# mattiaskvist/yolo-v1

Hardware: AMD Instinct MI355X
Metric: images/sec at 448x448, forward (YOLOv1Backbone + FC head) (higher is better)
Workload: dtype bf16; 1 GPU; BASELINE.json configs[1]: batch=64/GPU 448x448 forward-only, YOLOv1Backbone + FC head, 1xMI355X per rank; global_batch=64, per_gpu_batch=64, weights=random init (torch default, seed 0), parallelism=single

## Files before the change

### include/yolo_hip.h

```cpp
#ifndef YOLO_HIP_H
#define YOLO_HIP_H

#include <stddef.h>
#include <stdint.h>

#ifdef __cplusplus
extern "C" {
#endif

#define YOLO_HIP_ABI_VERSION 2

#define YOLO_E_ARG (-1)
#define YOLO_E_UNSUPPORTED (-2)

typedef void *yolo_stream_t;

int yolo_hip_abi_version(void);
const char *yolo_hip_last_error(void);
int yolo_debug_stamps(void *buf, int k_iter);
int yolo_stream_create(int low, yolo_stream_t *out);


int yolo_decode(const float *pred, int N, int S, int B, int C, double conf_thr,
                double *rec, int32_t *counts, yolo_stream_t stream);

int yolo_decode_gt(const float *tgt, int N, int S, int B, int C,
                   double *rec, int32_t *counts, yolo_stream_t stream);

#define YOLO_NMS_INFERENCE 0
#define YOLO_NMS_METRICS 1

int yolo_nms(const double *rec, const int32_t *counts, int N, int max_per_img, double thr, int variant,
             int32_t *keep, int32_t *keep_counts, yolo_stream_t stream);

int yolo_pairwise_iou(const double *a, int na, const double *b, int nb, int variant,
                      double *out, yolo_stream_t stream);

int yolo_loss_fwd_bwd(const float *pred, const float *tgt, int N, int S, int B, int C,
                      float lambda_coord, float lambda_noobj,
                      float *out, float *dpred, double *work, yolo_stream_t stream);

int yolo_loss_iou(const float *boxes1, const float *boxes2, long n, float *out, yolo_stream_t stream);


typedef struct yolo_igemm_desc {
    int32_t N, Ho, Wo;
    int64_t in_img_stride;
    int32_t in_row_stride;
    int32_t in_px_stride;
    int32_t in_off;
    int32_t stride;
    int32_t KH, KW;
    int32_t tap_len;
    int32_t Cout;
    int64_t out_img_stride;
    int32_t out_row_stride, out_px_stride, out_off;
    int32_t epilogue;
    float slope;
    int32_t out_fp32;
    int32_t split_k;
    int64_t aux_img_stride;
    int32_t aux_row_stride, aux_px_stride, aux_off;
    int32_t pool2;
    int32_t w_blocked;
    int32_t tile_order;
    int32_t tile_hint;
    int64_t px_begin, px_end;
    int32_t skew_phases;
    int32_t skew_step;
    void *bn_stats;
    int32_t tile_px;
    int32_t split_slabs;
} yolo_igemm_desc;

#define YOLO_EPI_NONE 0
#define YOLO_EPI_BIAS 1
#define YOLO_EPI_BIAS_LRELU 2
#define YOLO_EPI_MUL_DLRELU 3

#define YOLO_EPI_BIAS_ADD_LRELU 4

int yolo_igemm(const yolo_igemm_desc *d, const void *in_bf16, const void *w_bf16 ,
               const float *bias, const void *aux_bf16, void *out, yolo_stream_t stream);
int yolo_igemm_finish(const yolo_igemm_desc *d, const float *acc, const float *bias, const void *aux_bf16,
                      void *out_bf16, yolo_stream_t stream);

typedef struct yolo_wgrad_desc {
    int64_t P;
    int32_t dy_px_stride, x_px_stride;
    int32_t Cout, Cin;
    int32_t KH, KW, pad;
    int64_t x_row_stride;
    int32_t split;
    int32_t accumulate;
    int32_t variant;
    int32_t geo_W, geo_H, geo_img_slots, geo_row_slots, geo_px_slots, geo_slot0;
    double *dw_sumsq;
    float *slabs;
    int64_t slab_floats;
} yolo_wgrad_desc;

int yolo_wgrad_slab_floats(const yolo_wgrad_desc *d, long *floats);
int yolo_wgrad(const yolo_wgrad_desc *d, const void *x_bf16, const void *dy_bf16,
               float *dw_packed, float *db, yolo_stream_t stream);

typedef struct yolo_pool_desc {
    int32_t N, H, W, C;
    int32_t in_halo, out_halo;
} yolo_pool_desc;
int yolo_maxpool3s2_fwd(const yolo_pool_desc *d, const void *x_bf16, void *y_bf16, yolo_stream_t stream);
int yolo_maxpool3s2_bwd(const yolo_pool_desc *d, const void *x_bf16, const void *dy_bf16, void *dx_bf16, int dx_halo,
                        yolo_stream_t stream);
int yolo_maxpool2_fwd(const yolo_pool_desc *d, const void *x_bf16, void *y_bf16, yolo_stream_t stream);
int yolo_maxpool2_bwd_lrelu(const yolo_pool_desc *d, const void *yfull_bf16, const void *dpool_bf16,
                            float slope, void *dz_bf16, yolo_stream_t stream);
int yolo_maxpool2_bwd_codes(const yolo_pool_desc *d, const void *ypool_bf16, const void *codes_u16, const void *dpool_bf16,
                            float slope, void *dz_bf16, yolo_stream_t stream);


int yolo_nchw_f32_to_nhwc_bf16(const float *x, int N, int C, int H, int W, void *y, int Cpad,
                               int halo_lo, int halo_hi, yolo_stream_t stream);
int yolo_nhwc_bf16_to_nchw_f32(const void *x, int N, int C, int H, int W, int halo, float *y, yolo_stream_t stream);
int yolo_nhwc_bf16_to_nchw_bf16(const void *x, int N, int C, int H, int W, int halo, void *y, yolo_stream_t stream);

int yolo_pack_conv_weight(const float *w_oihw, int Cout, int Cin, int KH, int KW, int Cinp, int KWp,
                          void *w_fwd_bf16, void *w_dgrad_bf16, yolo_stream_t stream);
int yolo_pack_fc_weight(const float *w, int O, int C, int HW, void *w_fwd_bf16, void *w_t_bf16, yolo_stream_t stream);
int yolo_pack_fc_weight_blocked(const float *w, int O, long K, void *w_panels_bf16, yolo_stream_t stream);
int yolo_pack_fc_weight_blocked_hwc(const float *w, int O, int C, int HW, void *w_panels_bf16, yolo_stream_t stream);
int yolo_unpack_conv_wgrad(const float *dw_packed, int Cout, int Cin, int KH, int KW, int Cinp, int KWp,
                           float *dw_oihw, int accumulate, yolo_stream_t stream);
int yolo_conv_stem7_fwd(const void *x_nhwc4_bf16, const void *w_packed_bf16, const float *bias, int N, int Ho, int Wo,
                        long x_img_stride, int x_row_stride, float slope, int pool2, void *out_bf16,
                        long out_img_stride, int out_row_stride, int out_off, void *out_full_bf16,
                        long full_img_stride, int full_row_stride, int full_off, yolo_stream_t stream);
int yolo_conv_stem7_fwd_f32(const float *x_nchw_f32, const void *w_packed_bf16, const float *bias, int N, int H, int W, float slope,
                            int pool2, void *out_bf16, long out_img_stride, int out_row_stride, int out_off, void *out_full_bf16,
                            long full_img_stride, int full_row_stride, int full_off, yolo_stream_t stream);
int yolo_wgrad_stem7(const void *x_nhwc4_bf16, const void *dy_bf16, int N, int Ho, int Wo, long x_img_stride,
                     int x_row_stride, long dy_img_stride, int dy_row_stride, int dy_off, float *dw_oihw,
                     float *db, float *scratch, long scratch_elems, yolo_stream_t stream);
int yolo_wgrad_stem7_pooled(const void *x_nhwc4_bf16, const void *y_full_bf16, int N, int Ho, int Wo, long x_img_stride,
                            int x_row_stride, long y_img_stride, int y_row_stride, int y_off, const void *dpool_bf16,
                            long dp_img_stride, int dp_row_stride, int dp_off, float slope, float *dw_oihw, float *db,
                            float *scratch, long scratch_elems, yolo_stream_t stream);
int yolo_wgrad_stem7_codes(const void *x_nhwc4_bf16, const void *y_pooled_bf16, const void *codes_u16, int N, int Ho, int Wo,
                           long x_img_stride, int x_row_stride, const void *dpool_bf16, long dp_img_stride, int dp_row_stride,
                           int dp_off, float slope, float *dw_oihw, float *db, float *scratch, long scratch_elems,
                           yolo_stream_t stream);
#define YOLO_PACK_MAX 32
typedef struct yolo_conv_pack_item {
    const float *w;
    void *w_fwd_bf16;
    void *w_dgrad_bf16;
    int Cout, Cin, KH, KW;
} yolo_conv_pack_item;
typedef struct yolo_conv_unpack_item {
    const float *dw_packed;
    float *dw_oihw;
    int Cout, Cin, KH, KW;
} yolo_conv_unpack_item;
int yolo_pack_conv_weights_multi(const yolo_conv_pack_item *items, int count, yolo_stream_t stream);
int yolo_unpack_conv_wgrads_multi(const yolo_conv_unpack_item *items, int count, yolo_stream_t stream);
int yolo_im2col_rows(const void *x_bf16, long x_img_stride, int x_row_stride, int x_px_stride, int stride,
                     int KH, int seg, int N, int Ho, int Wo, int out_halo, void *xcol_bf16, yolo_stream_t stream);
int yolo_transpose_f32_to_bf16(const float *x, int R, int Ccols, void *y_bf16, int ld, yolo_stream_t stream);
int yolo_transpose_bf16(const void *x_bf16, int R, int Ccols, int ldx, void *y_bf16, int ldy, yolo_stream_t stream);
int yolo_fc_dgrad_to_nhwc(const float *dxT, int N, int C, int H, int W, int halo, const void *y_act_bf16,
                          float slope, void *g_bf16, yolo_stream_t stream);
int yolo_cast_f32_to_bf16(const float *x, long n, void *y_bf16, yolo_stream_t stream);
int yolo_cast_bf16_to_f32(const void *x_bf16, long n, float *y, yolo_stream_t stream);
int yolo_bias_lrelu_rows(const float *x, const float *bias, int R, int Ccols, float slope,
                         void *y_bf16, float *y_f32, yolo_stream_t stream);
int yolo_bias_lrelu_rows_slabs(const float *x, int slabs, const float *bias, int R, int Ccols, float slope,
                               void *y_bf16, float *y_f32, yolo_stream_t stream);

int yolo_scale_rows_to_bf16(const float *x, const unsigned char *mask, float scale, const void *act_bf16, float slope,
                            int R, int Cc, int ld, void *y_bf16, yolo_stream_t stream);
int yolo_dropout_bf16(const void *x_bf16, const unsigned char *mask, float scale, long n, void *y_bf16, yolo_stream_t stream);

int yolo_sumsq_f32(const float *g, long n, double *acc, yolo_stream_t stream);
int yolo_adam_step(float *p, const float *g, float *exp_avg, float *exp_avg_sq, long n, float lr, float beta1,
                   float beta2, float eps, float weight_decay, long step, const double *norm_sq,
                   float max_norm, void *p_bf16, yolo_stream_t stream);
#define YOLO_MT_MAX 48
typedef struct yolo_adam_tensor {
    float *p;
    const float *g;
    float *m, *v;
    void *p_bf16;
    long n;
} yolo_adam_tensor;
int yolo_sumsq_f32_multi(const float *const *g, const long *n, int count, double *acc, yolo_stream_t stream);
int yolo_sumsq_fixed_slots(const long *n, int count, long *slots);
int yolo_sumsq_f32_fixed(const float *g, long n, double *scratch, long scratch_slots, double *acc, yolo_stream_t stream);
int yolo_sumsq_f32_multi_fixed(const float *const *g, const long *n, int count, double *scratch, long scratch_slots, double *acc,
                               yolo_stream_t stream);
int yolo_adam_step_multi(const yolo_adam_tensor *t, int count, float lr, float beta1, float beta2, float eps,
                         float weight_decay, long step, const double *norm_sq, float max_norm, const float *skip_flag,
                         yolo_stream_t stream);
int yolo_adam_step_multi_bg(const yolo_adam_tensor *t, int count, float lr, float beta1, float beta2, float eps,
                            float weight_decay, long step, const double *norm_sq, float max_norm, const float *skip_flag,
                            int workgroups, yolo_stream_t stream);

typedef struct yolo_sgd_tensor {
    float *p;
    const float *g;
    float *buf;
    void *p_bf16;
    long n;
} yolo_sgd_tensor;
int yolo_sgd_step(float *p, const float *g, float *buf, long n, float lr, float momentum, float dampening, float weight_decay,
                  int nesterov, int first_step, const double *norm_sq, float max_norm, void *p_bf16, const float *skip_flag,
                  yolo_stream_t stream);
int yolo_sgd_step_multi(const yolo_sgd_tensor *t, int count, float lr, float momentum, float dampening, float weight_decay,
                        int nesterov, int first_step, const double *norm_sq, float max_norm, const float *skip_flag,
                        yolo_stream_t stream);
int yolo_sgd_step_multi_bg(const yolo_sgd_tensor *t, int count, float lr, float momentum, float dampening, float weight_decay,
                           int nesterov, int first_step, const double *norm_sq, float max_norm, const float *skip_flag,
                           int workgroups, yolo_stream_t stream);

int yolo_clip_scale_f32(float *g, long n, const double *norm_sq, float max_norm, yolo_stream_t stream);

#define YOLO_BN_ACC_REPLICAS 16
int yolo_batchnorm_train_fwd(void *z_bf16, int N, int H, int W, int C, int halo, const float *gamma, const float *beta,
                             double eps, double momentum, float *running_mean, float *running_var,
                             const void *residual_bf16, int residual_halo, int relu, double *acc2c,
                             float *scale_shift, void *out_bf16, int out_halo, float *save_mean_invstd,
                             int stats_ready, yolo_stream_t stream);
int yolo_batchnorm_bwd(void *dy_bf16, int dy_halo, const void *y_bf16, int y_halo, const void *z_bf16, int z_halo,
                       int N, int H, int W, int C, const float *gamma, const float *mean_invstd, void *dz_bf16,
                       long dz_img_stride, long dz_row_stride, long dz_px_stride, long dz_off, int store_masked_dy,
                       int relu_from_z, float *dgamma, float *dbeta, double *acc2c, float *coef3c, yolo_stream_t stream);

int yolo_map_match(const double *rec, const int32_t *keep, const int32_t *keep_counts, int N, int max_per_img,
                   const double *gt_rec, const int32_t *gt_counts, int max_gt, const double *thresholds, int T,
                   double extra_threshold, double small_area, double medium_area, unsigned long long *tp_bits,
                   int32_t *gt_bucket, yolo_stream_t stream);

int yolo_preprocess_u8(const unsigned char *src_u8, int N, int Hs, int Ws, int Ho, int Wo, const int32_t *hbounds,
                       const int32_t *hcoef, int hk, const int32_t *vbounds, const int32_t *vcoef, int vk,
                       unsigned char *tmp_u8, const float *mean3, const float *std3, void *out_nhwc4_bf16, int halo,
                       float *out_nchw, yolo_stream_t stream);

typedef struct yolo_augment_desc {
    int64_t src_off;
    int64_t tmp_off;
    int32_t Hs, Ws;
    int32_t top, left, ch, cw;
    const int32_t *htab;
    const int32_t *vtab;
    int32_t hk, vk;
    int32_t n_ops;
    int32_t ops[3];
    float brightness;
    float saturation;
    int32_t hue_shift;
    int32_t reserved;
} yolo_augment_desc;
#define YOLO_AUG_BRIGHTNESS 0
#define YOLO_AUG_SATURATION 1
#define YOLO_AUG_HUE 2

int yolo_augment_u8(const unsigned char *src_u8, int64_t src_bytes, const yolo_augment_desc *descs_host,
                    const yolo_augment_desc *descs_dev, int N, int Ho, int Wo, unsigned char *tmp_u8, int64_t tmp_bytes,
                    const float *mean3, const float *std3, void *out_nhwc4_bf16, int halo, float *out_nchw,
                    unsigned char *out_u8, yolo_stream_t stream);

#ifdef __cplusplus
}
#endif
#endif
```

### yolo-v1_amd/csrc/igemm.hip

```cpp
#include "igemm_common.h"

namespace yolo {

template <int TCO, int TPX, int BK, int WCO, int WPX, int NST, int MF = MFMA_32x32x16>
struct IgemmCfg {
    static constexpr int NW = WCO * WPX;
    static constexpr int NTHR = NW * 64;
    static constexpr bool UNEVEN = MF == MFMA_16x16x32_STAGGER_U;
    static constexpr int A_BYTES = TCO * BK * 2;
    static constexpr int B_BYTES = (TPX * BK * 2 + 1024 * NW - 1) / (1024 * NW) * (1024 * NW);
    static constexpr int STAGE_BYTES = A_BYTES + B_BYTES;
    static constexpr int EP = TCO + 4;
    static constexpr int NTILES = TPX / 16;
    static constexpr int NT0 = (NTILES + 1) / 2, NT1 = NTILES / 2;
    static constexpr int PPX = UNEVEN ? NT0 * 16 : TPX / WPX;
    static constexpr int EPI_BYTES = PPX * EP * 4;
    static constexpr int TABLE_BYTES = TPX * 32;
    static constexpr int RED_BYTES = WCO * WPX * 64 * 16 * 4;
    static constexpr int MAIN_BYTES = (NST * STAGE_BYTES > EPI_BYTES + RED_BYTES) ? NST * STAGE_BYTES : EPI_BYTES + RED_BYTES;
    static constexpr int LDS_BYTES = TABLE_BYTES + MAIN_BYTES;
    static constexpr int A_INSTR = A_BYTES / 1024 / NW;
    static constexpr int B_INSTR = B_BYTES / 1024 / NW;
    static constexpr int LOADS = A_INSTR + B_INSTR;
    static constexpr int FR = MF != MFMA_32x32x16 ? 16 : 32;
    static constexpr int KS = MF != MFMA_32x32x16 ? 32 : 16;
    static constexpr int MT = TCO / WCO / FR, NT = UNEVEN ? NT0 : TPX / WPX / FR;
    static_assert(A_BYTES % (1024 * NW) == 0 && B_BYTES % (1024 * NW) == 0, "stage must split evenly over the waves");
    static_assert(!UNEVEN || (WPX == 2 && TPX % 16 == 0), "uneven split: two pixel groups of 16-pixel columns");
    static_assert(UNEVEN || TPX * BK * 2 == B_BYTES, "only the uneven configuration pads its B stage");
    static_assert(TPX <= NTHR, "one table entry per thread");
};

template <int TCO, int TPX, int BK, int WCO, int WPX, int NST, int MF, int VAR>
__global__ void __launch_bounds__(WCO * WPX * 64, (TCO == 64 && TPX == 128 && BK == 32 && VAR == 0 ? 5 : 2)) igemm_kernel(const IgemmParams p)
{
    using Cfg = IgemmCfg<TCO, TPX, BK, WCO, WPX, NST, MF>;
    constexpr bool STATS = VAR == 1, CODES = VAR == 2;
    constexpr bool M16 = MF != MFMA_32x32x16;
    constexpr bool UNEVEN = Cfg::UNEVEN;
    constexpr bool STG = MF == MFMA_16x16x32_STAGGER || UNEVEN;
    constexpr int FR = Cfg::FR;
    constexpr int MT = Cfg::MT, NT = Cfg::NT, NW = Cfg::NW, NTHR = Cfg::NTHR;
    extern __shared__ __attribute__((aligned(16))) char smem[];
    long *tab = reinterpret_cast<long *>(smem);
    char *stage_base = smem + Cfg::TABLE_BYTES;

    const int tid = threadIdx.x;
    const int lane = tid & 63;
    const int wave = __builtin_amdgcn_readfirstlane(tid >> 6);
    const int wco = UNEVEN ? wave % WCO : wave / WPX, wpx = UNEVEN ? wave / WCO : wave % WPX;
    const int px_lo = UNEVEN ? wpx * Cfg::NT0 * 16 : wpx * (TPX / WPX);

    if (NW == 8 && p.skew_phases > 1 && gridDim.x * gridDim.y > 256 && blockIdx.y == 0 && blockIdx.x < 256) {
        const int ph = (blockIdx.x >> 3) % p.skew_phases;
        if (ph) {
            const long t0 = __builtin_amdgcn_s_memtime(), wait = ph * p.skew_cycles;
            while ((long)__builtin_amdgcn_s_memtime() - t0 < wait) __builtin_amdgcn_s_sleep(16);
        }
    }

    const int nwg = p.n_co_tiles * p.n_px_tiles;
    int bid = blockIdx.x;
    {
        const int q = nwg >> 3, r = nwg & 7, xcd = bid & 7, k = bid >> 3;
        bid = (xcd < r ? xcd * (q + 1) : r * (q + 1) + (xcd - r) * q) + k;
    }
    const int co_tile = p.px_fastest ? bid / p.n_px_tiles : bid % p.n_co_tiles;
    const int px_tile = p.px_fastest ? bid % p.n_px_tiles : bid / p.n_co_tiles;
    const int co0 = co_tile * TCO;
    const int tpv = p.tpx_valid;
    const long px0 = p.px_begin + (long)px_tile * tpv;

    if (tid < TPX) {
        int n, oy, ox;
        bool valid;
        if (p.pool) {
            const int per_img = p.pool_tiles_x * p.pool_tiles_y;
            n = px_tile / per_img;
            const int t = px_tile - n * per_img;
            const int ty = t / p.pool_tiles_x, tx = t - ty * p.pool_tiles_x;
            oy = ty * (TPX / p.pool_tw) + tid / p.pool_tw;
            ox = tx * p.pool_tw + tid % p.pool_tw;
            valid = oy < p.HoWo / p.Wo && ox < p.Wo;
            if (!valid) { oy = 0; ox = 0; }
        } else {
            long m = px0 + tid;
            valid = m < p.M && tid < tpv;
            if (!valid) m = p.M - 1;
            n = (int)(m / p.HoWo);
            const int rem = (int)(m - (long)n * p.HoWo);
            oy = rem / p.Wo;
            ox = rem - oy * p.Wo;
        }
        tab[4 * tid] = (long)n * p.in_img_stride + (long)(oy * p.stride) * p.in_row_stride + (long)(ox * p.stride) * p.in_px_stride + p.in_off;
        const int qy = p.pool ? oy >> 1 : oy, qx = p.pool ? ox >> 1 : ox;
        tab[4 * tid + 1] = valid ? ((long)n * p.out_img_stride + (long)qy * p.out_row_stride + (long)qx * p.out_px_stride + p.out_off) : -1;
        tab[4 * tid + 2] = (long)n * p.aux_img_stride + (long)oy * p.aux_row_stride + (long)ox * p.aux_px_stride + p.aux_off;
    }
    __syncthreads();

    const bf16_t *a_src[Cfg::A_INSTR];
    const bf16_t *b_src[Cfg::B_INSTR];
    int a_dst[Cfg::A_INSTR], b_dst[Cfg::B_INSTR];
    {
        constexpr int CPR = BK / 8, RPB = 16 / CPR;
#pragma unroll
        for (int i = 0; i < Cfg::A_INSTR; ++i) {
            const int q = i * NW + wave;
            const int pos = q * 64 + lane;
            const int R = pos >> 4, s = (pos & 15) ^ swz_key<BK, M16>(R);
            const int r = R * RPB + s / CPR, chunk = s % CPR;
            int co = co0 + r;
            if (co >= p.Cout) co = p.Cout - 1;
            a_src[i] = p.w_blocked ? p.w + ((long)co_tile * p.nk * TCO + r) * BK + chunk * 8 : p.w + (long)co * p.Ktot + chunk * 8;
            a_dst[i] = q * 1024;
        }
#pragma unroll
        for (int i = 0; i < Cfg::B_INSTR; ++i) {
            const int q = i * NW + wave;
            const int pos = q * 64 + lane;
            const int R = pos >> 4, s = (pos & 15) ^ swz_key<BK, M16>(R);
            const int r = R * RPB + s / CPR, chunk = s % CPR;
            b_src[i] = r < TPX ? p.in + tab[4 * r] + chunk * 8 : p.in + tab[0];
            b_dst[i] = Cfg::A_BYTES + q * 1024;
        }
    }

    const bool interleave = gridDim.y > 1 && p.KH * p.KW == 1;
    const int kstep = interleave ? (int)gridDim.y : 1;
    int kbeg, kend;
    if (interleave) {
        const int mine = (p.nk - (int)blockIdx.y + kstep - 1) / kstep;
        kbeg = 0;
        kend = mine > 0 ? mine : 0;
    } else {
        kbeg = blockIdx.y * p.nk_per_split;
        kend = min(p.nk, kbeg + p.nk_per_split);
    }
    const int cpt = p.tap_len / BK;
    int tap = interleave ? 0 : kbeg / cpt;
    int c0 = interleave ? (int)blockIdx.y * BK : (kbeg - tap * cpt) * BK;
    int ky = tap / p.KW, kx = tap - ky * p.KW;

    auto stage = [&](int buf, int kiter_local) {
        char *sb = stage_base + buf * Cfg::STAGE_BYTES;
        const int kiter = interleave ? (int)blockIdx.y + kiter_local * kstep : kiter_local;
        const long a_off = (long)kiter * (p.w_blocked ? TCO * BK : BK);
        const long b_off = interleave ? (long)kiter * BK : (long)ky * p.in_row_stride + (long)kx * p.in_px_stride + c0;
        if (p.w_blocked) {
#pragma unroll
            for (int i = 0; i < Cfg::A_INSTR; ++i) GLDS16_NT(a_src[i] + a_off, sb + a_dst[i]);
        } else {
#pragma unroll
            for (int i = 0; i < Cfg::A_INSTR; ++i) GLDS16(a_src[i] + a_off, sb + a_dst[i]);
        }
#pragma unroll
        for (int i = 0; i < Cfg::B_INSTR; ++i) GLDS16(b_src[i] + b_off, sb + b_dst[i]);
        c0 += BK;
        if (c0 == p.tap_len) {
            c0 = 0;
            if (++kx == p.KW) { kx = 0; ++ky; }
        }
    };

    int a_rd[MT], b_rd[NT];
#pragma unroll
    for (int i = 0; i < MT; ++i) a_rd[i] = lds_off<BK, M16>(wco * (TCO / WCO) + i * FR + (lane & (FR - 1)), M16 ? (lane >> 4) : (lane >> 5));
#pragma unroll
    for (int i = 0; i < NT; ++i) {
        int row = px_lo + i * FR + (lane & (FR - 1));
        if (UNEVEN && row >= TPX) row = TPX - 1;
        b_rd[i] = Cfg::A_BYTES + lds_off<BK, M16>(row, M16 ? (lane >> 4) : (lane >> 5));
    }

    typedef typename std::conditional<M16, f32x4, f32x16>::type acc_t;
    acc_t acc[MT][NT];
#pragma unroll
    for (int i = 0; i < MT; ++i)
#pragma unroll
        for (int j = 0; j < NT; ++j)
#pragma unroll
            for (int r = 0; r < (M16 ? 4 : 16); ++r) acc[i][j][r] = 0.0f;

    constexpr int KSTEPS = BK / Cfg::KS;
    constexpr int KSH = M16 ? 6 : 5;
    auto read_frags = [&](int buf, bf16x8(&af)[KSTEPS][MT], bf16x8(&bfr)[KSTEPS][NT], auto ntc) {
        constexpr int NTG = decltype(ntc)::value;
        const char *sb = stage_base + buf * Cfg::STAGE_BYTES;
#pragma unroll
        for (int ks = 0; ks < KSTEPS; ++ks) {
#pragma unroll
            for (int i = 0; i < MT; ++i) af[ks][i] = *reinterpret_cast<const bf16x8 *>(sb + (a_rd[i] ^ (ks << KSH)));
#pragma unroll
            for (int j = 0; j < NTG; ++j) bfr[ks][j] = *reinterpret_cast<const bf16x8 *>(sb + (b_rd[j] ^ (ks << KSH)));
        }
    };
    auto mfmas = [&](bf16x8(&af)[KSTEPS][MT], bf16x8(&bfr)[KSTEPS][NT], auto ntc) {
        constexpr int NTG = decltype(ntc)::value;
#pragma unroll
        for (int ks = 0; ks < KSTEPS; ++ks)
#pragma unroll
            for (int i = 0; i < MT; ++i)
#pragma unroll
                for (int j = 0; j < NTG; ++j) {
                    if constexpr (M16) acc[i][j] = __builtin_amdgcn_mfma_f32_16x16x32_bf16(af[ks][i], bfr[ks][j], acc[i][j], 0, 0, 0);
                    else acc[i][j] = __builtin_amdgcn_mfma_f32_32x32x16_bf16(af[ks][i], bfr[ks][j], acc[i][j], 0, 0, 0);
                }
    };

    if constexpr (STG) {
        static_assert(!STG || (NST >= 3 && NW == 8), "stagger needs 8 waves and a ring of >= 3 stages");
        constexpr std::integral_constant<int, NT> ntA{};
        constexpr std::integral_constant<int, UNEVEN ? Cfg::NT1 : NT> ntB{};
        constexpr int D = NST - 1;
        const bool grpB = wave >= NW / 2;
        const int nkk = kend - kbeg;
#pragma unroll
        for (int s0 = 0; s0 < D; ++s0)
            if (s0 < nkk) stage(s0, kbeg + s0);
        auto wait_stage = [&](int newer) {
            if (newer >= D - 1) wait_vmcnt<(D - 1) * Cfg::LOADS>();
            else if (newer == 1 && D - 1 > 1) wait_vmcnt<Cfg::LOADS>();
            else wait_vmcnt<0>();
        };
        wait_stage(nkk - 1 < D - 1 ? nkk - 1 : D - 1);
        __builtin_amdgcn_s_barrier();
        __builtin_amdgcn_sched_barrier(0);
        bf16x8 af[KSTEPS][MT], bfr[KSTEPS][NT];
        int rd_buf = 0;
#ifdef IGEMM_STAMPS
        long stamp[8] = {0, 0, 0, 0, 0, 0, 0, 0};
#define STAMP(i) do { if (p.dbg && it == p.dbg_it) { __builtin_amdgcn_sched_barrier(0); stamp[i] = __builtin_amdgcn_s_memtime(); __builtin_amdgcn_sched_barrier(0); } } while (0)
#else
#define STAMP(i) do { } while (0)
#endif
        if (!grpB) {
            int ld_buf = D % NST;
            for (int it = 0; it < nkk; ++it) {
                STAMP(0);
                read_frags(rd_buf, af, bfr, ntA);
                STAMP(1);
                if (it + D < nkk) stage(ld_buf, kbeg + it + D);
                STAMP(2);
                asm volatile("s_waitcnt lgkmcnt(0)" ::: "memory");
                STAMP(3);
                __builtin_amdgcn_sched_barrier(0);
                __builtin_amdgcn_s_barrier();
                __builtin_amdgcn_sched_barrier(0);
                STAMP(4);
                __builtin_amdgcn_s_setprio(1);
                mfmas(af, bfr, ntA);
                __builtin_amdgcn_s_setprio(0);
                STAMP(5);
                { const int left = nkk - 2 - it; wait_stage(left < 0 ? 0 : left); }
                STAMP(6);
                __builtin_amdgcn_sched_barrier(0);
                __builtin_amdgcn_s_barrier();
                __builtin_amdgcn_sched_barrier(0);
                STAMP(7);
                rd_buf = rd_buf + 1 == NST ? 0 : rd_buf + 1;
                ld_buf = ld_buf + 1 == NST ? 0 : ld_buf + 1;
            }
            __builtin_amdgcn_s_barrier();
        } else {
            __builtin_amdgcn_s_barrier();
            __builtin_amdgcn_sched_barrier(0);
            int ld_buf = D % NST;
            for (int it = 0; it < nkk; ++it) {
                STAMP(0);
                read_frags(rd_buf, af, bfr, ntB);
                STAMP(1);
                if (it + D < nkk) stage(ld_buf, kbeg + it + D);
                STAMP(2);
                asm volatile("s_waitcnt lgkmcnt(0)" ::: "memory");
                { const int left = nkk - 2 - it; wait_stage(left < 0 ? 0 : left); }
                STAMP(3);
                __builtin_amdgcn_sched_barrier(0);
                __builtin_amdgcn_s_barrier();
                __builtin_amdgcn_sched_barrier(0);
                STAMP(4);
                STAMP(5);
                __builtin_amdgcn_s_setprio(1);
                mfmas(af, bfr, ntB);
                __builtin_amdgcn_s_setprio(0);
                STAMP(6);
                __builtin_amdgcn_sched_barrier(0);
                __builtin_amdgcn_s_barrier();
                __builtin_amdgcn_sched_barrier(0);
                STAMP(7);
                rd_buf = rd_buf + 1 == NST ? 0 : rd_buf + 1;
                ld_buf = ld_buf + 1 == NST ? 0 : ld_buf + 1;
            }
        }
#ifdef IGEMM_STAMPS
        if (p.dbg && lane == 0 && blockIdx.x < 512) {
#pragma unroll
            for (int i = 0; i < 8; ++i) p.dbg[((long)blockIdx.x * 8 + wave) * 8 + i] = stamp[i];
        }
#endif
#undef STAMP
    } else {
    constexpr int D = NST - 1;
#pragma unroll
    for (int s0 = 0; s0 < D; ++s0)
        if (kbeg + s0 < kend) stage(s0, kbeg + s0);
    int cur = 0, nxt = D % NST;
    for (int it = kbeg; it < kend; ++it) {
        if (D >= 2 && it + 1 < kend) wait_vmcnt<(D >= 2 ? (D - 1) * Cfg::LOADS : 0)>();
        else wait_vmcnt<0>();
        asm volatile("s_waitcnt lgkmcnt(0)" ::: "memory");
        __builtin_amdgcn_s_barrier();
        if (it + D < kend) stage(nxt, it + D);
        bf16x8 af[KSTEPS][MT], bfr[KSTEPS][NT];
        const char *sb = stage_base + cur * Cfg::STAGE_BYTES;
#pragma unroll
        for (int ks = 0; ks < KSTEPS; ++ks) {
#pragma unroll
            for (int i = 0; i < MT; ++i) af[0][i] = *reinterpret_cast<const bf16x8 *>(sb + (a_rd[i] ^ (ks << KSH)));
#pragma unroll
            for (int j = 0; j < NT; ++j) bfr[0][j] = *reinterpret_cast<const bf16x8 *>(sb + (b_rd[j] ^ (ks << KSH)));
#pragma unroll
            for (int i = 0; i < MT; ++i)
#pragma unroll
                for (int j = 0; j < NT; ++j) {
                    if constexpr (M16) acc[i][j] = __builtin_amdgcn_mfma_f32_16x16x32_bf16(af[0][i], bfr[0][j], acc[i][j], 0, 0, 0);
                    else acc[i][j] = __builtin_amdgcn_mfma_f32_32x32x16_bf16(af[0][i], bfr[0][j], acc[i][j], 0, 0, 0);
                }
        }
        cur = (cur + 1 == NST) ? 0 : cur + 1;
        nxt = (nxt + 1 == NST) ? 0 : nxt + 1;
    }
    }
    __syncthreads();

    float *ep = reinterpret_cast<float *>(stage_base);
    constexpr int PPX = Cfg::PPX;
    constexpr int CCH = TCO / 8;
    constexpr int PX_PER_STEP = NTHR / CCH;
    const int cc = tid % CCH;
    const int co = co0 + cc * 8;
    const bool has_bias = p.epilogue == YOLO_EPI_BIAS || p.epilogue == YOLO_EPI_BIAS_LRELU || p.epilogue == YOLO_EPI_BIAS_ADD_LRELU;
    float bias8[8];
#pragma unroll
    for (int k = 0; k < 8; ++k) bias8[k] = has_bias && (co + k < p.Cout) ? p.bias[co + k] : 0.0f;
    const bool split = gridDim.y > 1 && p.slab_stride == 0;
    void *const outp = p.slab_stride ? (void *)(reinterpret_cast<float *>(p.out) + (long)blockIdx.y * p.slab_stride) : p.out;
    float *red = reinterpret_cast<float *>(stage_base + Cfg::EPI_BYTES) + tid * 16;
    if constexpr (STATS) {
#pragma unroll
        for (int k = 0; k < 16; ++k) red[k] = 0.0f;
    }

    constexpr int E_CCH = TCO / 8, E_PXS = NTHR / E_CCH, E_PPX = Cfg::PPX;
    constexpr int NIT = (E_PPX + E_PXS - 1) / E_PXS;
    constexpr bool CAN_PREFETCH = NIT <= 4 && !UNEVEN && !STATS && TCO * TPX <= 128 * 128;
    const bool aux_fast = CAN_PREFETCH && (p.epilogue == YOLO_EPI_BIAS_ADD_LRELU || p.epilogue == YOLO_EPI_MUL_DLRELU) && gridDim.y == 1 && !p.pool &&
                          !p.out_fp32 && co0 + (tid % E_CCH) * 8 + 8 <= p.Cout;
    uint4 axv[CAN_PREFETCH ? NIT : 1];
    long axo[CAN_PREFETCH ? NIT : 1];
    auto aux_fetch = [&](int q) {
#pragma unroll
        for (int it = 0; it < NIT; ++it) {
            const int lp = tid / E_CCH + it * E_PXS;
            const int px = q * E_PPX + (lp < E_PPX ? lp : 0);
            axo[it] = lp < E_PPX ? tab[4 * px + 1] : -1;
            axv[it] = axo[it] >= 0 ? *reinterpret_cast<const uint4 *>(p.aux + tab[4 * px + 2] + co0 + (tid % E_CCH) * 8) : uint4{0u, 0u, 0u, 0u};
        }
    };

    for (int q = 0; q < WPX; ++q) {
        if (q > 0) __syncthreads();
        if constexpr (CAN_PREFETCH) {
            if (aux_fast) aux_fetch(q);
        }
        if (wpx == q) {
#pragma unroll
            for (int i = 0; i < MT; ++i)
#pragma unroll
                for (int j = 0; j < NT; ++j) {
                    if constexpr (M16) {
                        const int lp = j * 16 + (lane & 15);
                        const int cob = wco * (TCO / WCO) + i * 16 + 4 * (lane >> 4);
                        f32x4 v = {acc[i][j][0], acc[i][j][1], acc[i][j][2], acc[i][j][3]};
                        *reinterpret_cast<f32x4 *>(ep + lp * Cfg::EP + cob) = v;
                    } else {
                        const int lp = j * 32 + (lane & 31);
                        const int cob = wco * (TCO / WCO) + i * 32 + 4 * (lane >> 5);
#pragma unroll
                        for (int g = 0; g < 4; ++g) {
                            f32x4 v = {acc[i][j][4 * g], acc[i][j][4 * g + 1], acc[i][j][4 * g + 2], acc[i][j][4 * g + 3]};
                            *reinterpret_cast<f32x4 *>(ep + lp * Cfg::EP + cob + 8 * g) = v;
                        }
                    }
                }
        }
        __syncthreads();
        const int pbase = q * PPX;
        const int ppx_q = UNEVEN && q == 1 ? Cfg::NT1 * 16 : PPX;

        if (split) {
            float *o = reinterpret_cast<float *>(p.out);
            for (int e = tid; e < ppx_q * TCO; e += NTHR) {
                const int lp = e / TCO, c = e - lp * TCO;
                const long ob = tab[4 * (pbase + lp) + 1];
                if (ob >= 0 && co0 + c < p.Cout) atomicAdd(o + ob + co0 + c, ep[lp * Cfg::EP + c]);
            }
            continue;
        }
        if (p.pool) {
            const int tw = p.pool_tw, hw = tw >> 1;
            for (int w = tid / CCH; w < PPX / 4; w += PX_PER_STEP) {
                const int l00 = (w / hw) * 2 * tw + (w % hw) * 2;
                const long ob = tab[4 * (pbase + l00) + 1];
                if (ob < 0 || co >= p.Cout) continue;
                float v[8];
                if (CODES && p.pool == 3) {
                    unsigned code = 0;
#pragma unroll
                    for (int k = 0; k < 8; ++k) {
                        const float *zp = ep + l00 * Cfg::EP + cc * 8 + k;
                        float m = 0.0f;
                        unsigned am = 0;
#pragma unroll
                        for (int w4 = 0; w4 < 4; ++w4) {
                            float t = zp[((w4 >> 1) * tw + (w4 & 1)) * Cfg::EP] + bias8[k];
                            t = (p.epilogue == YOLO_EPI_BIAS_LRELU && t < 0.0f) ? t * p.slope : t;
                            t = __uint_as_float((unsigned)f32_to_bf16(t) << 16);
                            if (w4 == 0 || t > m) { m = t; am = w4; }
                        }
                        v[k] = m;
                        code |= am << (2 * k);
                        __builtin_amdgcn_sched_barrier(0);
                    }
                    reinterpret_cast<unsigned short *>(const_cast<bf16_t *>(p.aux))[(ob + co) >> 3] = (unsigned short)code;
                } else {
#pragma unroll
                    for (int k = 0; k < 8; ++k) {
                        const float a = ep[l00 * Cfg::EP + cc * 8 + k], b = ep[(l00 + 1) * Cfg::EP + cc * 8 + k];
                        const float c = ep[(l00 + tw) * Cfg::EP + cc * 8 + k], d = ep[(l00 + tw + 1) * Cfg::EP + cc * 8 + k];
                        float m = fmaxf(fmaxf(a, b), fmaxf(c, d)) + bias8[k];
                        v[k] = (p.epilogue == YOLO_EPI_BIAS_LRELU && m < 0.0f) ? m * p.slope : m;
                    }
                }
                uint4 pk;
                pk.x = (unsigned)f32_to_bf16(v[0]) | ((unsigned)f32_to_bf16(v[1]) << 16);
                pk.y = (unsigned)f32_to_bf16(v[2]) | ((unsigned)f32_to_bf16(v[3]) << 16);
                pk.z = (unsigned)f32_to_bf16(v[4]) | ((unsigned)f32_to_bf16(v[5]) << 16);
                pk.w = (unsigned)f32_to_bf16(v[6]) | ((unsigned)f32_to_bf16(v[7]) << 16);
                *reinterpret_cast<uint4 *>(reinterpret_cast<bf16_t *>(p.out) + ob + co) = pk;
            }
            if (p.pool == 2) {
                bf16_t *full = const_cast<bf16_t *>(p.aux);
                for (int lp = tid / CCH; lp < PPX; lp += PX_PER_STEP) {
                    const int px = pbase + lp;
                    if (tab[4 * px + 1] < 0) continue;
                    if (co >= p.Cout) continue;
                    float v[8];
#pragma unroll
                    for (int k = 0; k < 8; ++k) {
                        const float m = ep[lp * Cfg::EP + cc * 8 + k] + bias8[k];
                        v[k] = (p.epilogue == YOLO_EPI_BIAS_LRELU && m < 0.0f) ? m * p.slope : m;
                    }
                    uint4 pk;
                    pk.x = (unsigned)f32_to_bf16(v[0]) | ((unsigned)f32_to_bf16(v[1]) << 16);
                    pk.y = (unsigned)f32_to_bf16(v[2]) | ((unsigned)f32_to_bf16(v[3]) << 16);
                    pk.z = (unsigned)f32_to_bf16(v[4]) | ((unsigned)f32_to_bf16(v[5]) << 16);
                    pk.w = (unsigned)f32_to_bf16(v[6]) | ((unsigned)f32_to_bf16(v[7]) << 16);
                    *reinterpret_cast<uint4 *>(full + tab[4 * px + 2] + co) = pk;
                }
            }
            continue;
        }
        if constexpr (CAN_PREFETCH) {
            if (aux_fast) {
#pragma unroll
                for (int it0 = 0; it0 < NIT; ++it0) {
                    const uint4 av = axv[it0];
                    const long ao = axo[it0];
                    if (ao < 0) continue;
                    const int lp = tid / CCH + it0 * PX_PER_STEP;
                    const f32x4 lo = *reinterpret_cast<const f32x4 *>(ep + lp * Cfg::EP + cc * 8);
                    const f32x4 hi = *reinterpret_cast<const f32x4 *>(ep + lp * Cfg::EP + cc * 8 + 4);
                    float v[8] = {lo[0], lo[1], lo[2], lo[3], hi[0], hi[1], hi[2], hi[3]};
                    const unsigned yy[4] = {av.x, av.y, av.z, av.w};
#pragma unroll
                    for (int k = 0; k < 8; ++k) {
                        const float a = __uint_as_float((k & 1) ? (yy[k >> 1] & 0xffff0000u) : (yy[k >> 1] << 16));
                        if (p.epilogue == YOLO_EPI_BIAS_ADD_LRELU) {
                            v[k] += bias8[k] + a;
                            v[k] = v[k] > 0.0f ? v[k] : v[k] * p.slope;
                        } else {
                            v[k] = a > 0.0f ? v[k] : v[k] * p.slope;
                        }
                    }
                    uint4 pk;
                    pk.x = (unsigned)f32_to_bf16(v[0]) | ((unsigned)f32_to_bf16(v[1]) << 16);
                    pk.y = (unsigned)f32_to_bf16(v[2]) | ((unsigned)f32_to_bf16(v[3]) << 16);
                    pk.z = (unsigned)f32_to_bf16(v[4]) | ((unsigned)f32_to_bf16(v[5]) << 16);
                    pk.w = (unsigned)f32_to_bf16(v[6]) | ((unsigned)f32_to_bf16(v[7]) << 16);
                    *reinterpret_cast<uint4 *>(reinterpret_cast<bf16_t *>(p.out) + ao + co) = pk;
                }
                continue;
            }
        }
#pragma unroll 2
        for (int lp = tid / CCH; lp < ppx_q; lp += PX_PER_STEP) {
            const int px = pbase + lp;
            const long ob = tab[4 * px + 1];
            if (ob < 0 || co >= p.Cout) continue;
            float v[8];
            const f32x4 lo = *reinterpret_cast<const f32x4 *>(ep + lp * Cfg::EP + cc * 8);
            const f32x4 hi = *reinterpret_cast<const f32x4 *>(ep + lp * Cfg::EP + cc * 8 + 4);
            v[0] = lo[0]; v[1] = lo[1]; v[2] = lo[2]; v[3] = lo[3];
            v[4] = hi[0]; v[5] = hi[1]; v[6] = hi[2]; v[7] = hi[3];
            if (has_bias) {
#pragma unroll
                for (int k = 0; k < 8; ++k) v[k] += bias8[k];
            }
            if (p.epilogue == YOLO_EPI_BIAS_ADD_LRELU) {
                const uint4 y = *reinterpret_cast<const uint4 *>(p.aux + tab[4 * px + 2] + co);
                const unsigned yy[4] = {y.x, y.y, y.z, y.w};
#pragma unroll
                for (int k = 0; k < 8; ++k) {
                    v[k] += __uint_as_float((k & 1) ? (yy[k >> 1] & 0xffff0000u) : (yy[k >> 1] << 16));
                    v[k] = v[k] > 0.0f ? v[k] : v[k] * p.slope;
                }
            } else if (p.epilogue == YOLO_EPI_BIAS_LRELU) {
#pragma unroll
                for (int k = 0; k < 8; ++k) v[k] = v[k] > 0.0f ? v[k] : v[k] * p.slope;
            } else if (p.epilogue == YOLO_EPI_MUL_DLRELU) {
                const uint4 y = *reinterpret_cast<const uint4 *>(p.aux + tab[4 * px + 2] + co);
                const unsigned yy[4] = {y.x, y.y, y.z, y.w};
#pragma unroll
                for (int k = 0; k < 8; ++k) {
                    const float a = __uint_as_float((k & 1) ? (yy[k >> 1] & 0xffff0000u) : (yy[k >> 1] << 16));
                    v[k] = a > 0.0f ? v[k] : v[k] * p.slope;
                }
            }
            if (p.out_fp32) {
                float *o = reinterpret_cast<float *>(outp) + ob + co;
                if (co + 8 <= p.Cout && ((ob + co) & 3) == 0) {
                    *reinterpret_cast<f32x4 *>(o) = f32x4{v[0], v[1], v[2], v[3]};
                    *reinterpret_cast<f32x4 *>(o + 4) = f32x4{v[4], v[5], v[6], v[7]};
                } else {
#pragma unroll
                    for (int k = 0; k < 8; ++k)
                        if (co + k < p.Cout) o[k] = v[k];
                }
            } else {
                bf16_t *o = reinterpret_cast<bf16_t *>(p.out) + ob + co;
                uint4 pk;
                pk.x = (unsigned)f32_to_bf16(v[0]) | ((unsigned)f32_to_bf16(v[1]) << 16);
                pk.y = (unsigned)f32_to_bf16(v[2]) | ((unsigned)f32_to_bf16(v[3]) << 16);
                pk.z = (unsigned)f32_to_bf16(v[4]) | ((unsigned)f32_to_bf16(v[5]) << 16);
                pk.w = (unsigned)f32_to_bf16(v[6]) | ((unsigned)f32_to_bf16(v[7]) << 16);
                *reinterpret_cast<uint4 *>(o) = pk;
                if constexpr (STATS) {
                    const unsigned w4[4] = {pk.x, pk.y, pk.z, pk.w};
#pragma unroll
                    for (int k = 0; k < 8; ++k) {
                        const float r = __uint_as_float((k & 1) ? (w4[k >> 1] & 0xffff0000u) : (w4[k >> 1] << 16));
                        red[k] += r;
                        red[8 + k] += r * r;
                    }
                }
            }
        }
    }
    if constexpr (STATS) {
        __syncthreads();
        const float *all = reinterpret_cast<const float *>(stage_base + Cfg::EPI_BYTES);
        for (int c = tid; c < TCO; c += NTHR) {
            const int c8 = c >> 3, k = c & 7;
            float a = 0.0f, b = 0.0f;
            for (int j = 0; j < NTHR / CCH; ++j) { a += all[(j * CCH + c8) * 16 + k]; b += all[(j * CCH + c8) * 16 + 8 + k]; }
            if (co0 + c < p.Cout) {
                double *rep = p.stats + (size_t)(blockIdx.x % YOLO_BN_ACC_REPLICAS) * 2 * p.Cout;
                atomicAdd(rep + co0 + c, (double)a);
                atomicAdd(rep + p.Cout + co0 + c, (double)b);
            }
        }
    }
}

template <int TCO, int TPX, int BK, int WCO, int WPX, int NST, int MF, int VAR>
static int launch_impl(const IgemmParams &p, int splits, hipStream_t s)
{
    using Cfg = IgemmCfg<TCO, TPX, BK, WCO, WPX, NST, MF>;
    static bool attr_done[64] = {};
    int dev = 0;
    if (hipGetDevice(&dev) != hipSuccess || dev < 0 || dev >= 64) dev = 0;
    if (!attr_done[dev]) {
        hipError_t e = hipFuncSetAttribute(reinterpret_cast<const void *>(&igemm_kernel<TCO, TPX, BK, WCO, WPX, NST, MF, VAR>), hipFuncAttributeMaxDynamicSharedMemorySize, Cfg::LDS_BYTES);
        if (e != hipSuccess) return fail((int)e, "yolo_igemm: hipFuncSetAttribute(%d B LDS): %s", Cfg::LDS_BYTES, hipGetErrorString(e));
        attr_done[dev] = true;
    }
    IgemmParams q = p;
    q.n_co_tiles = (p.Cout + TCO - 1) / TCO;
    if (p.pool) {
        q.tpx_valid = TPX;
        q.pool_tiles_x = (p.Wo + p.pool_tw - 1) / p.pool_tw;
        q.pool_tiles_y = (p.HoWo / p.Wo + TPX / p.pool_tw - 1) / (TPX / p.pool_tw);
        q.n_px_tiles = (int)(p.M / p.HoWo) * q.pool_tiles_x * q.pool_tiles_y;
    } else {
        if (q.tpx_valid <= 0 || q.tpx_valid > TPX) q.tpx_valid = TPX;
        q.n_px_tiles = (int)((p.M - p.px_begin + q.tpx_valid - 1) / q.tpx_valid);
    }
    q.nk = (int)(p.Ktot / BK);
    if (p.px_fastest < 0) q.px_fastest = 0;
    q.nk_per_split = (q.nk + splits - 1) / splits;
    const int real_splits = p.slab_stride ? splits : (q.nk + q.nk_per_split - 1) / q.nk_per_split;
    hipLaunchKernelGGL((igemm_kernel<TCO, TPX, BK, WCO, WPX, NST, MF, VAR>), dim3(q.n_co_tiles * q.n_px_tiles, real_splits), dim3(Cfg::NTHR), Cfg::LDS_BYTES, s, q);
    return check_launch("yolo_igemm");
}

template <int TCO, int TPX, int BK, int WCO, int WPX, int NST, int MF = MFMA_32x32x16>
static int launch(const IgemmParams &p, int splits, hipStream_t s)
{
    return p.stats ? launch_impl<TCO, TPX, BK, WCO, WPX, NST, MF, 1>(p, splits, s) : launch_impl<TCO, TPX, BK, WCO, WPX, NST, MF, 0>(p, splits, s);
}

__global__ void __launch_bounds__(256) igemm_finish_kernel(const float *__restrict__ acc, const float *__restrict__ bias, const bf16_t *__restrict__ aux,
                                                           bf16_t *__restrict__ out, long M, int slabs, int HoWo, int Wo, int Cout, int epilogue, float slope,
                                                           long out_img, int out_row, int out_px, int out_off, long aux_img, int aux_row, int aux_px, int aux_off)
{
    const int C8 = Cout >> 3;
    const long idx = (long)blockIdx.x * blockDim.x + threadIdx.x;
    if (idx >= M * C8) return;
    const int c = (int)(idx % C8) * 8;
    const long m = idx / C8;
    const int n = (int)(m / HoWo);
    const int rem = (int)(m - (long)n * HoWo);
    const int oy = rem / Wo, ox = rem - oy * Wo;
    const float4 a = *reinterpret_cast<const float4 *>(acc + m * Cout + c), b = *reinterpret_cast<const float4 *>(acc + m * Cout + c + 4);
    float v[8] = {a.x, a.y, a.z, a.w, b.x, b.y, b.z, b.w};
    for (int sl = 1; sl < slabs; ++sl) {
        const float *as = acc + (long)sl * M * Cout + m * Cout + c;
        const float4 a2 = *reinterpret_cast<const float4 *>(as), b2 = *reinterpret_cast<const float4 *>(as + 4);
        v[0] += a2.x; v[1] += a2.y; v[2] += a2.z; v[3] += a2.w;
        v[4] += b2.x; v[5] += b2.y; v[6] += b2.z; v[7] += b2.w;
    }
    if (epilogue == YOLO_EPI_BIAS || epilogue == YOLO_EPI_BIAS_LRELU) {
#pragma unroll
        for (int k = 0; k < 8; ++k) v[k] += bias[c + k];
    }
    if (epilogue == YOLO_EPI_BIAS_LRELU) {
#pragma unroll
        for (int k = 0; k < 8; ++k) v[k] = v[k] > 0.0f ? v[k] : v[k] * slope;
    } else if (epilogue == YOLO_EPI_MUL_DLRELU) {
        const uint4 y = *reinterpret_cast<const uint4 *>(aux + (long)n * aux_img + (long)oy * aux_row + (long)ox * aux_px + aux_off + c);
        const unsigned yy[4] = {y.x, y.y, y.z, y.w};
#pragma unroll
        for (int k = 0; k < 8; ++k) {
            const float t = __uint_as_float((k & 1) ? (yy[k >> 1] & 0xffff0000u) : (yy[k >> 1] << 16));
            v[k] = t > 0.0f ? v[k] : v[k] * slope;
        }
    }
    uint4 o;
    o.x = (unsigned)f32_to_bf16(v[0]) | ((unsigned)f32_to_bf16(v[1]) << 16);
    o.y = (unsigned)f32_to_bf16(v[2]) | ((unsigned)f32_to_bf16(v[3]) << 16);
    o.z = (unsigned)f32_to_bf16(v[4]) | ((unsigned)f32_to_bf16(v[5]) << 16);
    o.w = (unsigned)f32_to_bf16(v[6]) | ((unsigned)f32_to_bf16(v[7]) << 16);
    *reinterpret_cast<uint4 *>(out + (long)n * out_img + (long)oy * out_row + (long)ox * out_px + out_off + c) = o;
}

}

using namespace yolo;

static long *g_dbg = nullptr;
static int g_dbg_it = 0;

namespace yolo {
void debug_stamp_target(long **buf, int *it)
{
    *buf = g_dbg;
    *it = g_dbg_it;
}
}

YOLO_API int yolo_debug_stamps(void *buf, int k_iter)
{
    g_dbg = (long *)buf;
    g_dbg_it = k_iter;
#ifdef IGEMM_STAMPS
    return 0;
#else
    return buf ? fail(YOLO_E_UNSUPPORTED, "yolo_debug_stamps: this library was built without -DIGEMM_STAMPS (make diag)") : 0;
#endif
}

YOLO_API int yolo_igemm(const yolo_igemm_desc *d, const void *in, const void *w, const float *bias, const void *aux, void *out, yolo_stream_t stream)
{
    if (!d || !in || !w || !out) return fail(YOLO_E_ARG, "yolo_igemm: null pointer");
    if (d->N <= 0 || d->Ho <= 0 || d->Wo <= 0 || d->KH <= 0 || d->KW <= 0 || d->tap_len <= 0 || d->Cout <= 0 || d->stride <= 0)
        return fail(YOLO_E_ARG, "yolo_igemm: bad descriptor");
    if ((d->epilogue == YOLO_EPI_BIAS || d->epilogue == YOLO_EPI_BIAS_LRELU || d->epilogue == YOLO_EPI_BIAS_ADD_LRELU) && !bias) return fail(YOLO_E_ARG, "yolo_igemm: epilogue needs bias");
    if ((d->epilogue == YOLO_EPI_MUL_DLRELU || d->epilogue == YOLO_EPI_BIAS_ADD_LRELU) && !aux) return fail(YOLO_E_ARG, "yolo_igemm: epilogue needs aux");
    if (d->epilogue < 0 || d->epilogue > YOLO_EPI_BIAS_ADD_LRELU) return fail(YOLO_E_ARG, "yolo_igemm: epilogue %d", d->epilogue);
    const int splits = d->split_k > 1 ? d->split_k : 1;
    if (splits > 1 && (!d->out_fp32 || d->epilogue != YOLO_EPI_NONE)) return fail(YOLO_E_ARG, "yolo_igemm: split_k needs fp32 output and EPI_NONE");
    if (d->split_slabs && splits > 1 && (d->out_off != 0 || (d->Wo > 1 && d->out_px_stride != d->Cout) || (d->Ho > 1 && d->out_row_stride != d->Wo * d->Cout)
                                         || (d->N > 1 && d->out_img_stride != (int64_t)d->Ho * d->Wo * d->Cout)))
        return fail(YOLO_E_ARG, "yolo_igemm: split_slabs needs the dense [N*Ho*Wo][Cout] output addressing");
    if (d->tile_px < 0) return fail(YOLO_E_ARG, "yolo_igemm: tile_px %d", d->tile_px);
    if (!d->out_fp32 && ((d->Cout & 7) || (d->out_off & 7) || (d->out_px_stride & 7) || (d->out_row_stride & 7) || (d->out_img_stride & 7)))
        return fail(YOLO_E_UNSUPPORTED, "yolo_igemm: bf16 output needs Cout and output strides in multiples of 8");
    if ((d->tap_len & 31) || (d->in_off & 7) || (d->in_px_stride & 3) || (d->in_row_stride & 7) || (d->in_img_stride & 7))
        return fail(YOLO_E_UNSUPPORTED, "yolo_igemm: tap_len=%d must be a multiple of 32 and input strides 16-B aligned", d->tap_len);

    IgemmParams p{};
    p.in = (const bf16_t *)in; p.w = (const bf16_t *)w; p.bias = bias; p.aux = (const bf16_t *)aux; p.out = out;
    p.M = (long)d->N * d->Ho * d->Wo; p.HoWo = d->Ho * d->Wo; p.Wo = d->Wo;
    if (d->px_begin < 0 || d->px_end < 0 || d->px_begin > p.M || d->px_end > p.M || (d->px_end && d->px_end <= d->px_begin))
        return fail(YOLO_E_ARG, "yolo_igemm: bad pixel range [%ld, %ld) of %ld", (long)d->px_begin, (long)d->px_end, (long)p.M);
    if ((d->px_begin || d->px_end) && d->pool2) return fail(YOLO_E_UNSUPPORTED, "yolo_igemm: pixel ranges are not available with pool2");
    p.px_begin = d->px_begin;
    p.tpx_valid = d->tile_px;
    p.slab_stride = (d->split_slabs && splits > 1) ? (long)d->N * d->Ho * d->Wo * d->Cout : 0;
    if (d->px_end) p.M = d->px_end;
    p.in_img_stride = d->in_img_stride; p.in_row_stride = d->in_row_stride; p.in_px_stride = d->in_px_stride; p.in_off = d->in_off; p.stride = d->stride;
    p.KH = d->KH; p.KW = d->KW; p.tap_len = d->tap_len; p.Cout = d->Cout;
    p.Ktot = (long)d->KH * d->KW * d->tap_len;
    p.out_img_stride = d->out_img_stride; p.out_row_stride = d->out_row_stride; p.out_px_stride = d->out_px_stride; p.out_off = d->out_off;
    p.aux_img_stride = d->aux_img_stride; p.aux_row_stride = d->aux_row_stride; p.aux_px_stride = d->aux_px_stride; p.aux_off = d->aux_off;
    p.epilogue = d->epilogue; p.slope = d->slope; p.out_fp32 = d->out_fp32;
    hipStream_t s = STRM(stream);

    const bool bk64 = (d->tap_len % 64) == 0;
    const bool small_co = d->Cout <= 64 || (d->Cout % 128 != 0 && d->Cout % 64 == 0 && d->Cout < 512);
    const long npx = p.M - p.px_begin;
    const long tiles128 = ((npx + 127) / 128) * ((d->Cout + 127) / 128);
    const int force = d->tile_hint;
    p.w_blocked = d->w_blocked;
    p.px_fastest = d->tile_order == 1 ? 0 : (d->tile_order == 2 ? 1 : -1);
    if (d->skew_phases < 0 || d->skew_phases > 64 || d->skew_step < 0 || d->skew_step > (1 << 22)) return fail(YOLO_E_ARG, "yolo_igemm: skew_phases %d / skew_step %d", d->skew_phases, d->skew_step);
    p.skew_phases = d->skew_phases;
    p.skew_cycles = d->skew_step;
    p.stats = (double *)d->bn_stats;
    p.dbg = g_dbg;
    p.dbg_it = g_dbg_it;
    if (p.stats && (d->out_fp32 || splits > 1 || d->pool2 || d->px_begin || d->px_end))
        return fail(YOLO_E_UNSUPPORTED, "yolo_igemm: bn_stats needs a plain bf16 launch (no split_k, pool2, pixel range)");
    p.pool = (d->pool2 == 2 || d->pool2 == 3) ? d->pool2 : (d->pool2 ? 1 : 0);
    if (p.pool == 2 && !aux) return fail(YOLO_E_ARG, "yolo_igemm: pool2 = 2 writes the un-pooled activation through aux (pointer + aux_* strides)");
    if (p.pool == 3 && (!aux || (d->Cout & 7) || (d->out_img_stride & 7) || (d->out_row_stride & 7) || (d->out_px_stride & 7) || (d->out_off & 7)))
        return fail(YOLO_E_ARG, "yolo_igemm: pool2 = 3 writes the arg-max codes through aux (one uint16 per 8 channels at (pooled element address) / 8): "
                                "Cout and the out_* strides must be multiples of 8");
    p.pool_tw = 16;
    if (p.pool && d->tile_px) return fail(YOLO_E_UNSUPPORTED, "yolo_igemm: tile_px is not available with pool2");
    if (p.pool && (splits > 1 || d->out_fp32 || (d->Ho & 1) || (d->Wo & 1) || (d->epilogue != YOLO_EPI_BIAS && d->epilogue != YOLO_EPI_BIAS_LRELU)))
        return fail(YOLO_E_UNSUPPORTED, "yolo_igemm: pool2 needs even Ho/Wo, bf16 output, a bias epilogue and no split-K");
    if (force == 20 || force == 21) return igemm_persist_launch(p, force, splits, s);
    if (p.pool == 3 && !(force >= 15 && force <= 18)) {
        if (!bk64 || d->w_blocked || p.stats) return fail(YOLO_E_UNSUPPORTED, "yolo_igemm: pool2 = 3 needs tap_len %% 64 == 0 (or tile_hint 16 / 18), plain weights, no bn_stats");
        if (small_co) return launch_impl<64, 128, 64, 2, 2, 2, MFMA_16x16x32, 2>(p, splits, s);
        return launch_impl<128, 128, 64, 2, 2, 2, MFMA_16x16x32, 2>(p, splits, s);
    }
    if (d->w_blocked) {
        if (!bk64) return fail(YOLO_E_UNSUPPORTED, "yolo_igemm: blocked weights need tap_len %% 64 == 0");
        return npx <= 64 ? launch<128, 64, 64, 2, 2, 3, MFMA_16x16x32>(p, splits, s) : launch<128, 128, 64, 2, 2, 2, MFMA_16x16x32>(p, splits, s);
    }
    if (force == 12) return launch<256, 256, 32, 2, 4, 4, MFMA_16x16x32_STAGGER>(p, splits, s);
    if (force == 14) {
        if (d->pool2) return fail(YOLO_E_UNSUPPORTED, "yolo_igemm: tile_hint 14 has no pooled epilogue");
        return launch<256, 208, 32, 4, 2, 4, MFMA_16x16x32_STAGGER_U>(p, splits, s);
    }
    if (force >= 15 && force <= 18) return igemm_pipe_launch(p, force, splits, s);
    if (force == 22) return conv_c64_launch(p, s);
    if (force == 19) return igemm_stream_launch(p, splits, s);
    if (force == 13) return launch<256, 128, 32, 4, 2, 4, MFMA_16x16x32_STAGGER>(p, splits, s);
    if (force == 10) return launch<64, 128, 32, 2, 2, 2>(p, splits, s);
    if (!bk64) {
        if (force == 7) return launch<64, 128, 32, 2, 2, 3>(p, splits, s);
        if (force == 9) return launch<64, 128, 32, 2, 2, 4>(p, splits, s);
        if (force == 10) return launch<64, 128, 32, 2, 2, 2>(p, splits, s);
        if (small_co) return launch<64, 128, 32, 2, 2, 3>(p, splits, s);
        return launch<128, 128, 32, 2, 2, 2>(p, splits, s);
    }
    if (force == 8) return launch<64, 128, 64, 2, 2, 3, MFMA_16x16x32>(p, splits, s);
    if (p.pool) {
        if (small_co) return launch<64, 128, 64, 2, 2, 2, MFMA_16x16x32>(p, splits, s);
        return launch<128, 128, 64, 2, 2, 2, MFMA_16x16x32>(p, splits, s);
    }
    if (force == 1) return launch<128, 128, 64, 2, 2, 2>(p, splits, s);
    if (force == 2) return launch<256, 128, 64, 4, 2, 3>(p, splits, s);
    if (force == 3) return launch<128, 64, 64, 2, 2, 2>(p, splits, s);
    if (force == 4) return launch<64, 128, 64, 2, 2, 2>(p, splits, s);
    if (force == 5) return launch<128, 128, 64, 2, 2, 2, MFMA_16x16x32>(p, splits, s);
    if (force == 6) return launch<256, 128, 64, 4, 2, 3, MFMA_16x16x32>(p, splits, s);
    if (force == 11) return launch<256, 128, 64, 4, 2, 3, MFMA_16x16x32_STAGGER>(p, splits, s);
    if (npx <= 64) {
        if (small_co) return launch<64, 64, 64, 2, 2, 2, MFMA_16x16x32>(p, splits, s);
        return splits > 1 ? launch<128, 64, 64, 2, 2, 3, MFMA_16x16x32>(p, splits, s) : launch<128, 64, 64, 2, 2, 2, MFMA_16x16x32>(p, splits, s);
    }
    if (small_co) return launch<64, 128, 64, 2, 2, 2, MFMA_16x16x32>(p, splits, s);
    if (tiles128 * splits < 320 && d->Cout >= 128) return launch<128, 64, 64, 2, 2, 2, MFMA_16x16x32>(p, splits, s);
    return launch<128, 128, 64, 2, 2, 2, MFMA_16x16x32>(p, splits, s);
}

YOLO_API int yolo_igemm_finish(const yolo_igemm_desc *d, const float *acc, const float *bias, const void *aux, void *out, yolo_stream_t stream)
{
    if (!d || !acc || !out) return fail(YOLO_E_ARG, "yolo_igemm_finish: null pointer");
    if (d->epilogue != YOLO_EPI_NONE && d->epilogue != YOLO_EPI_BIAS && d->epilogue != YOLO_EPI_BIAS_LRELU && d->epilogue != YOLO_EPI_MUL_DLRELU)
        return fail(YOLO_E_UNSUPPORTED, "yolo_igemm_finish: epilogue %d", d->epilogue);
    if ((d->epilogue == YOLO_EPI_BIAS || d->epilogue == YOLO_EPI_BIAS_LRELU) && !bias) return fail(YOLO_E_ARG, "yolo_igemm_finish: epilogue needs bias");
    if (d->epilogue == YOLO_EPI_MUL_DLRELU && !aux) return fail(YOLO_E_ARG, "yolo_igemm_finish: epilogue needs aux");
    if (d->out_fp32 || d->pool2 || (d->Cout & 7) || (d->out_off & 7) || (d->out_px_stride & 7) || (d->out_row_stride & 7) || (d->out_img_stride & 7))
        return fail(YOLO_E_UNSUPPORTED, "yolo_igemm_finish: bf16 output with Cout and strides in multiples of 8, no pool2");
    const long M = (long)d->N * d->Ho * d->Wo;
    const long total = M * (d->Cout / 8);
    hipLaunchKernelGGL(igemm_finish_kernel, dim3((unsigned)((total + 255) / 256)), dim3(256), 0, STRM(stream), acc, bias, (const bf16_t *)aux, (bf16_t *)out, M,
                       (d->split_slabs && d->split_k > 1) ? d->split_k : 1, d->Ho * d->Wo, d->Wo, d->Cout, d->epilogue, d->slope, (long)d->out_img_stride, d->out_row_stride, d->out_px_stride, d->out_off,
                       (long)d->aux_img_stride, d->aux_row_stride, d->aux_px_stride, d->aux_off);
    return check_launch("yolo_igemm_finish");
}
```

### yolo-v1_amd/csrc/igemm_common.h

```cpp
#pragma once
#include "common.h"
#include <type_traits>

namespace yolo {

typedef __attribute__((ext_vector_type(8))) __bf16 bf16x8;
typedef __attribute__((ext_vector_type(16))) float f32x16;
typedef __attribute__((ext_vector_type(4))) float f32x4;

enum { MFMA_32x32x16 = 0, MFMA_16x16x32 = 1, MFMA_16x16x32_STAGGER = 2, MFMA_16x16x32_STAGGER_U = 3 };

struct IgemmParams {
    const bf16_t *in;
    const bf16_t *w;
    const float *bias;
    const bf16_t *aux;
    void *out;
    long M;
    int HoWo, Wo;
    long in_img_stride;
    int in_row_stride, in_px_stride, in_off, stride;
    int KH, KW, tap_len, Cout;
    long Ktot;
    long out_img_stride;
    int out_row_stride, out_px_stride, out_off;
    long aux_img_stride;
    int aux_row_stride, aux_px_stride, aux_off;
    int epilogue;
    float slope;
    int out_fp32;
    int pool, pool_tw, pool_tiles_x, pool_tiles_y;
    int w_blocked;
    int nk;
    int nk_per_split;
    int n_co_tiles, n_px_tiles;
    long px_begin;
    int tpx_valid;
    long slab_stride;
    int px_fastest;
    int skew_phases;
    long skew_cycles;
    long *dbg;
    int dbg_it;
    double *stats;
    unsigned div_hw_magic, div_hw_shift, div_w_magic, div_w_shift, div_hw2_magic, div_hw2_shift;
    unsigned *tile_ctr;
};

#define GLDS16(gptr, lptr) \
    __builtin_amdgcn_global_load_lds((const __attribute__((address_space(1))) void *)(gptr), (__attribute__((address_space(3))) void *)(lptr), 16, 0, 0)

#define GLDS16_NT(gptr, lptr) \
    __builtin_amdgcn_global_load_lds((const __attribute__((address_space(1))) void *)(gptr), (__attribute__((address_space(3))) void *)(lptr), 16, 0, 2)

template <int BK, bool M16>
__device__ __forceinline__ int swz_key(int R)
{
    if constexpr (BK == 32 && M16) return (-R) & 3;
    else return R & 15;
}

template <int BK, bool M16>
__device__ __forceinline__ int lds_off(int r, int chunk)
{
    constexpr int CPR = BK / 8;
    constexpr int RPB = 16 / CPR;
    const int R = r / RPB;
    const int s = (r % RPB) * CPR + chunk;
    return R * 256 + ((s ^ swz_key<BK, M16>(R)) << 4);
}

template <int N>
__device__ __forceinline__ void wait_vmcnt()
{
    asm volatile("s_waitcnt vmcnt(%0)" ::"n"(N) : "memory");
}

int igemm_pipe_launch(const IgemmParams &p, int hint, int splits, hipStream_t s);
int igemm_persist_launch(const IgemmParams &p, int hint, int splits, hipStream_t s);
int igemm_stream_launch(const IgemmParams &p, int splits, hipStream_t s);
int conv_c64_launch(const IgemmParams &p, hipStream_t s);

}
```

### yolo-v1_amd/csrc/igemm_persist.hip

```cpp
#include "igemm_common.h"
#include <atomic>
#include <mutex>

namespace yolo {

template <int NTILES_>
struct PersistCfg {
    static constexpr int TCO = 256, NTILES = NTILES_, NST = 4, BK = 32;
    static constexpr int TPX = 16 * NTILES;
    static constexpr int WCO = 4, NW = 8, NTHR = 512;
    static constexpr int NT0 = 7, NT1 = NTILES - 7;
    static constexpr int A_BYTES = TCO * BK * 2;
    static constexpr int B_BYTES = 256 * BK * 2;
    static constexpr int STAGE_BYTES = A_BYTES + B_BYTES;
    static constexpr int A_PIECES = A_BYTES / 1024 / NW, B_PIECES = B_BYTES / 1024 / NW;
    static constexpr int LOADS = A_PIECES + B_PIECES;
    static constexpr int TABLE_BYTES = 256 * 16;
    static constexpr int STASH_BYTES = NW * 64 * 4;
    static constexpr int MAIL_BYTES = 64;
    static constexpr int LDS_BYTES = 2 * TABLE_BYTES + STASH_BYTES + MAIL_BYTES + NST * STAGE_BYTES;
    static constexpr int D = NST - 1;
    static_assert(NT1 >= 1 && NT1 <= NT0, "pixel group B holds 1 .. 7 columns");
};

__device__ __forceinline__ unsigned fast_div(unsigned n, unsigned magic, unsigned shift)
{
    return magic ? (__umulhi(n, magic) >> shift) : n;
}

__device__ __forceinline__ int fresh_lane()
{
    int l;
    asm volatile("v_mbcnt_lo_u32_b32 %0, -1, 0\n\tv_mbcnt_hi_u32_b32 %0, -1, %0" : "=v"(l));
    return l;
}

__device__ __forceinline__ f32x4 quad_max4(f32x4 v)
{
    float a0, a1, a2, a3;
    asm volatile("s_nop 1\n\t"
                 "v_max_f32_dpp %0, %4, %4 quad_perm:[1,0,3,2] row_mask:0xf bank_mask:0xf\n\t"
                 "v_max_f32_dpp %1, %5, %5 quad_perm:[1,0,3,2] row_mask:0xf bank_mask:0xf\n\t"
                 "v_max_f32_dpp %2, %6, %6 quad_perm:[1,0,3,2] row_mask:0xf bank_mask:0xf\n\t"
                 "v_max_f32_dpp %3, %7, %7 quad_perm:[1,0,3,2] row_mask:0xf bank_mask:0xf\n\t"
                 "v_max_f32_dpp %0, %0, %0 quad_perm:[2,3,0,1] row_mask:0xf bank_mask:0xf\n\t"
                 "v_max_f32_dpp %1, %1, %1 quad_perm:[2,3,0,1] row_mask:0xf bank_mask:0xf\n\t"
                 "v_max_f32_dpp %2, %2, %2 quad_perm:[2,3,0,1] row_mask:0xf bank_mask:0xf\n\t"
                 "v_max_f32_dpp %3, %3, %3 quad_perm:[2,3,0,1] row_mask:0xf bank_mask:0xf"
                 : "=&v"(a0), "=&v"(a1), "=&v"(a2), "=&v"(a3)
                 : "v"(v[0]), "v"(v[1]), "v"(v[2]), "v"(v[3]));
    return f32x4{a0, a1, a2, a3};
}

__device__ __forceinline__ void quad_min4(unsigned (&k)[4])
{
    asm volatile("s_nop 1\n\t"
                 "v_min_u32_dpp %0, %0, %0 quad_perm:[1,0,3,2] row_mask:0xf bank_mask:0xf\n\t"
                 "v_min_u32_dpp %1, %1, %1 quad_perm:[1,0,3,2] row_mask:0xf bank_mask:0xf\n\t"
                 "v_min_u32_dpp %2, %2, %2 quad_perm:[1,0,3,2] row_mask:0xf bank_mask:0xf\n\t"
                 "v_min_u32_dpp %3, %3, %3 quad_perm:[1,0,3,2] row_mask:0xf bank_mask:0xf\n\t"
                 "v_min_u32_dpp %0, %0, %0 quad_perm:[2,3,0,1] row_mask:0xf bank_mask:0xf\n\t"
                 "v_min_u32_dpp %1, %1, %1 quad_perm:[2,3,0,1] row_mask:0xf bank_mask:0xf\n\t"
                 "v_min_u32_dpp %2, %2, %2 quad_perm:[2,3,0,1] row_mask:0xf bank_mask:0xf\n\t"
                 "v_min_u32_dpp %3, %3, %3 quad_perm:[2,3,0,1] row_mask:0xf bank_mask:0xf"
                 : "+v"(k[0]), "+v"(k[1]), "+v"(k[2]), "+v"(k[3]));
}

__device__ __forceinline__ void store1(const void *base, unsigned voff, unsigned byte)
{
    asm volatile("global_store_byte %0, %1, %2\n\ts_nop 1" ::"v"(voff), "v"(byte), "s"(base) : "memory");
}

__device__ __forceinline__ unsigned pack_bf16x2(float lo, float hi)
{
    unsigned r;
    asm("v_cvt_pk_bf16_f32 %0, %1, %2" : "=v"(r) : "v"(lo), "v"(hi));
    return r;
}

template <int IMM>
__device__ __forceinline__ void store8(const void *base, unsigned voff, unsigned lo, unsigned hi)
{
    typedef __attribute__((ext_vector_type(2))) unsigned u32x2;
    const u32x2 d = {lo, hi};
    asm volatile("global_store_dwordx2 %0, %1, %2 offset:%3\n\ts_nop 1" ::"v"(voff), "v"(d), "s"(base), "n"(IMM) : "memory");
}

template <int IMM>
__device__ __forceinline__ void store16(const void *base, unsigned voff, unsigned a, unsigned b, unsigned c, unsigned d)
{
    typedef __attribute__((ext_vector_type(4))) unsigned u32x4;
    const u32x4 v = {a, b, c, d};
    asm volatile("global_store_dwordx4 %0, %1, %2 offset:%3\n\ts_nop 1" ::"v"(voff), "v"(v), "s"(base), "n"(IMM) : "memory");
}

__device__ __forceinline__ void row_swap4(f32x4 &x, f32x4 &y)
{
    float x0 = x[0], x1 = x[1], x2 = x[2], x3 = x[3], y0 = y[0], y1 = y[1], y2 = y[2], y3 = y[3];
    asm volatile("s_nop 1\n\t"
                 "v_permlane16_swap_b32 %0, %4\n\t"
                 "v_permlane16_swap_b32 %1, %5\n\t"
                 "v_permlane16_swap_b32 %2, %6\n\t"
                 "v_permlane16_swap_b32 %3, %7\n\t"
                 "s_nop 1"
                 : "+v"(x0), "+v"(x1), "+v"(x2), "+v"(x3), "+v"(y0), "+v"(y1), "+v"(y2), "+v"(y3));
    x = f32x4{x0, x1, x2, x3};
    y = f32x4{y0, y1, y2, y3};
}

template <int NTILES, bool POOL, int DGRAD, bool CODES = false, bool SLAB = false, int MT = 4>
__global__ void __launch_bounds__(512, 2) igemm_persist_kernel(const IgemmParams p)
{
    using C = PersistCfg<NTILES>;
    constexpr int TPX = C::TPX, BK = C::BK, NW = C::NW, WCO = C::WCO, NT0 = C::NT0, NT1 = C::NT1, NST = C::NST;
    constexpr int A_BYTES = C::A_BYTES, STAGE_BYTES = C::STAGE_BYTES, LOADS = C::LOADS, D = C::D;
    constexpr int WCH = MT * 16;
    constexpr int TCO = WCO * WCH;
    extern __shared__ __attribute__((aligned(16))) char smem[];
    unsigned *tab = reinterpret_cast<unsigned *>(smem);
    float *stash = reinterpret_cast<float *>(smem + 2 * C::TABLE_BYTES);
    int *mail = reinterpret_cast<int *>(smem + 2 * C::TABLE_BYTES + C::STASH_BYTES);
    char *stage_base = smem + 2 * C::TABLE_BYTES + C::STASH_BYTES + C::MAIL_BYTES;

    const int tid = threadIdx.x;
    const int lane = tid & 63;
    const int wave = __builtin_amdgcn_readfirstlane(tid >> 6);
    const int wco = wave % WCO, grp = wave / WCO;
    const int px_lo = grp * NT0 * 16;

#ifdef IGEMM_STAMPS
    long tstamp[8] = {0, 0, 0, 0, 0, 0, 0, 0};
    tstamp[0] = __builtin_amdgcn_s_memtime();
#define PSTAMP(i) do { __builtin_amdgcn_sched_barrier(0); tstamp[i] = __builtin_amdgcn_s_memtime(); __builtin_amdgcn_sched_barrier(0); } while (0)
#else
#define PSTAMP(i) do { } while (0)
#endif
    const int S = SLAB ? p.pool_tiles_x : 1;
    const int T = p.n_co_tiles * p.n_px_tiles * S;
    const int G = gridDim.x;
    const int tpv = p.tpx_valid;
    const int xl = (int)blockIdx.x & 7;
    const int cnt_x = (T >> 3) + (xl < (T & 7) ? 1 : 0);
    const int nwg_x = (G - xl + 7) >> 3;
    unsigned *const tile_ctr = p.tile_ctr + xl;

    auto tile_of = [&](int j, int &co0, unsigned &px0, int &ks) {
        const int q = T >> 3, r = T & 7;
        int bid = (xl < r ? xl * (q + 1) : r * (q + 1) + (xl - r) * q) + j;
        ks = 0;
        if constexpr (SLAB) {
            ks = bid % S;
            bid /= S;
        }
        const int co_tile = p.px_fastest ? bid / p.n_px_tiles : bid % p.n_co_tiles;
        const int px_tile = p.px_fastest ? bid % p.n_px_tiles : bid / p.n_co_tiles;
        co0 = co_tile * TCO;
        px0 = (unsigned)px_tile * (unsigned)tpv;
    };

    auto build_table = [&](int buf, unsigned px0) {
        const int tid = wave * 64 + fresh_lane();
        if (tid < TPX) {
            unsigned m;
            if constexpr (POOL) {
                const unsigned W = (unsigned)(tid >> 4) * 4 + (unsigned)((tid >> 2) & 3), e = (unsigned)tid & 3;
                const unsigned hw = (unsigned)p.Wo >> 1;
                const unsigned wy = fast_div(W, p.div_hw2_magic, p.div_hw2_shift), wx = W - wy * hw;
                m = px0 + (2 * wy + (e >> 1)) * (unsigned)p.Wo + 2 * wx + (e & 1);
            } else {
                m = px0 + (unsigned)tid;
            }
            if (m >= (unsigned)p.M) m = (unsigned)p.M - 1;
            const unsigned n = fast_div(m, p.div_hw_magic, p.div_hw_shift);
            const unsigned rem = m - n * (unsigned)p.HoWo;
            const unsigned oy = fast_div(rem, p.div_w_magic, p.div_w_shift), ox = rem - oy * (unsigned)p.Wo;
            const long in_e = (long)n * p.in_img_stride + (long)(oy * p.stride) * p.in_row_stride + (long)(ox * p.stride) * p.in_px_stride + p.in_off;
            const unsigned qy = POOL ? oy >> 1 : oy, qx = POOL ? ox >> 1 : ox;
            const long out_e = (long)n * p.out_img_stride + (long)qy * p.out_row_stride + (long)qx * p.out_px_stride + p.out_off;
            const long aux_e = (long)n * p.aux_img_stride + (long)oy * p.aux_row_stride + (long)ox * p.aux_px_stride + p.aux_off;
            uint4 ent;
            ent.x = (unsigned)(in_e * 2);
            ent.y = (unsigned)(out_e * (SLAB ? 4 : 2));
            ent.z = (unsigned)(aux_e * 2);
            ent.w = 0;
            *reinterpret_cast<uint4 *>(tab + (buf * 256 + tid) * 4) = ent;
        }
    };

    unsigned a_voff[C::A_PIECES], b_voff[C::B_PIECES];
#pragma unroll
    for (int i = 0; i < C::A_PIECES; ++i) {
        const int pos = (i * NW + wave) * 64 + lane;
        const int R = pos >> 4, s = (pos & 15) ^ swz_key<BK, true>(R);
        int r = R * 4 + s / 4;
        const int chunk = s % 4;
        if (r >= p.Cout) r = p.Cout - 1;
        a_voff[i] = (unsigned)(((long)r * p.Ktot + chunk * 8) * 2);
    }
    auto load_b_voff = [&](int buf) {
        const int lane = fresh_lane();
#pragma unroll
        for (int i = 0; i < C::B_PIECES; ++i) {
            const int pos = (i * NW + wave) * 64 + lane;
            const int R = pos >> 4, s = (pos & 15) ^ swz_key<BK, true>(R);
            const int r = R * 4 + s / 4;
            b_voff[i] = tab[(buf * 256 + (r < TPX ? r : 0)) * 4] + (unsigned)((s % 4) * 16);
        }
    };

    const int nk = SLAB ? p.nk_per_split : p.nk;
    const int cpt = p.tap_len / BK;
    unsigned a_soff = 0;
    int c0 = 0, ky = 0, kx = 0;

    auto stage = [&](int buf) {
        char *sb = stage_base + buf * STAGE_BYTES + wave * 1024;
        const unsigned b_soff = (unsigned)((ky * p.in_row_stride + kx * p.in_px_stride + c0) * 2);
        const char *wb = reinterpret_cast<const char *>(p.w) + a_soff;
        const char *xb = reinterpret_cast<const char *>(p.in) + b_soff;
#pragma unroll
        for (int i = 0; i < C::A_PIECES; ++i)
            __builtin_amdgcn_global_load_lds((const __attribute__((address_space(1))) void *)(wb + (unsigned long)a_voff[i]),
                                             (__attribute__((address_space(3))) void *)(sb + i * NW * 1024), 16, 0, 0);
#ifdef PERSIST_NO_B
        constexpr int NB = 0;
        (void)xb;
#elif defined(PERSIST_HALF_B)
        const int NB = (kx == 1) ? C::B_PIECES : 0;
#else
        constexpr int NB = C::B_PIECES;
#endif
#pragma unroll
        for (int i = 0; i < NB; ++i)
            __builtin_amdgcn_global_load_lds((const __attribute__((address_space(1))) void *)(xb + (unsigned long)b_voff[i]),
                                             (__attribute__((address_space(3))) void *)(sb + A_BYTES + i * NW * 1024), 16, 0, 0);
        a_soff += BK * 2;
        c0 += BK;
        const int w0 = c0 == p.tap_len;
        c0 = w0 ? 0 : c0;
        kx += w0;
        const int w1 = kx == p.KW;
        kx = w1 ? 0 : kx;
        ky += w1;
    };
    auto stage_reset = [&](int co0, int ks) {
        const int kbeg = ks * nk;
        a_soff = (unsigned)((long)co0 * p.Ktot * 2) + (unsigned)kbeg * (BK * 2);
        const int tap = kbeg / cpt;
        c0 = (kbeg - tap * cpt) * BK;
        ky = tap / p.KW;
        kx = tap - ky * p.KW;
    };

    const int a_rd0 = lds_off<BK, true>(wco * WCH + (lane & 15), lane >> 4);
    const int b_rd0 = A_BYTES + lds_off<BK, true>(px_lo + (lane & 15), lane >> 4);

    f32x4 acc[MT][NT0];

    unsigned drawn = 0;
    auto draw = [&]() {
        if (wave == 0) {
            const unsigned l = fresh_lane();
            if (l == 0) {
                unsigned d = 1u;
                asm volatile("s_nop 4\n\tglobal_atomic_add %0, %1, %0, %2 sc0" : "+v"(d) : "v"(l), "s"(tile_ctr) : "memory");
                drawn = d;
            }
        }
    };
    auto publish = [&](int slot) {
        if (wave == 0) {
            if (fresh_lane() == 0) mail[slot] = nwg_x + (int)drawn;
            asm volatile("s_waitcnt lgkmcnt(0)" ::: "memory");
        }
    };

    int j_cur = (int)blockIdx.x >> 3;
    draw();
    int co0_cur, ks_cur;
    unsigned px0_cur;
    tile_of(j_cur, co0_cur, px0_cur, ks_cur);
    build_table(0, px0_cur);
    const bool has_bias = p.epilogue == YOLO_EPI_BIAS || p.epilogue == YOLO_EPI_BIAS_LRELU || p.epilogue == YOLO_EPI_BIAS_ADD_LRELU;
    auto load_stash = [&](int co0) {
        const int lane = fresh_lane();
        const int ch = co0 + wco * WCH + lane;
        stash[wave * 64 + lane] = (has_bias && lane < WCH && ch < p.Cout) ? p.bias[ch] : 0.0f;
    };
    load_stash(co0_cur);
    __syncthreads();
    load_b_voff(0);
    stage_reset(co0_cur, ks_cur);
#pragma unroll
    for (int s0 = 0; s0 < D; ++s0) stage(s0);
    wait_vmcnt<(D - 1) * LOADS>();
    publish(0);
    __builtin_amdgcn_s_barrier();
    __builtin_amdgcn_sched_barrier(0);
    int j_next = __builtin_amdgcn_readfirstlane(mail[0]);
    PSTAMP(1);

    auto run = [&](auto ntc) {
        constexpr int NTG = decltype(ntc)::value;
        bf16x8 a0[MT], b0[NT0], a1[MT], b1[NT0];
        auto rd = [&](int buf, bf16x8(&af)[MT], bf16x8(&bfr)[NT0]) {
            const char *sb = stage_base + buf * STAGE_BYTES;
#pragma unroll
            for (int i = 0; i < MT; ++i) af[i] = *reinterpret_cast<const bf16x8 *>(sb + a_rd0 + i * 1024);
#pragma unroll
            for (int j = 0; j < NTG; ++j) bfr[j] = *reinterpret_cast<const bf16x8 *>(sb + b_rd0 + j * 1024);
        };
        auto mm = [&](auto zc, bf16x8(&af)[MT], bf16x8(&bfr)[NT0]) {
            constexpr bool Z = decltype(zc)::value;
#pragma unroll
            for (int i = 0; i < MT; ++i)
#pragma unroll
                for (int j = 0; j < NTG; ++j)
                    acc[i][j] = __builtin_amdgcn_mfma_f32_16x16x32_bf16(af[i], bfr[j], Z ? f32x4{0.0f, 0.0f, 0.0f, 0.0f} : acc[i][j], 0, 0, 0);
        };
        using ZeroC = std::integral_constant<bool, true>;
        using AccC = std::integral_constant<bool, false>;
        constexpr int NRD = MT + NTG, NMF = MT * NTG;
        auto body = [&](auto zc, int rbuf, int lbuf, bf16x8(&ca)[MT], bf16x8(&cb)[NT0], bf16x8(&na)[MT], bf16x8(&nb)[NT0]) {
            __builtin_amdgcn_s_barrier();
            __builtin_amdgcn_sched_barrier(0);
            rd(rbuf, na, nb);
            stage(lbuf);
            mm(zc, ca, cb);
#pragma unroll
            for (int k = 0; k < NRD; ++k) {
                __builtin_amdgcn_sched_group_barrier(0x008, 1, 0);
                __builtin_amdgcn_sched_group_barrier(0x100, 1, 0);
            }
            constexpr int PER = (NMF - NRD) / (LOADS + 1);
#pragma unroll
            for (int k = 0; k < LOADS; ++k) {
                __builtin_amdgcn_sched_group_barrier(0x008, PER, 0);
                __builtin_amdgcn_sched_group_barrier(0x020, 1, 0);
            }
            __builtin_amdgcn_sched_group_barrier(0x008, NMF - NRD - LOADS * PER, 0);
            __builtin_amdgcn_sched_barrier(0);
        };
        auto last_step = [&](int lbuf, bf16x8(&ca)[MT], bf16x8(&cb)[NT0]) {
            wait_vmcnt<(D - 2) * LOADS>();
            __builtin_amdgcn_s_barrier();
            __builtin_amdgcn_sched_barrier(0);
            stage(lbuf);
            mm(AccC{}, ca, cb);
            constexpr int PER = NMF / (LOADS + 1);
#pragma unroll
            for (int k = 0; k < LOADS; ++k) {
                __builtin_amdgcn_sched_group_barrier(0x008, PER, 0);
                __builtin_amdgcn_sched_group_barrier(0x020, 1, 0);
            }
            __builtin_amdgcn_sched_group_barrier(0x008, NMF - LOADS * PER, 0);
            __builtin_amdgcn_sched_barrier(0);
        };
        auto step = [&](int rbuf, int lbuf, bf16x8(&ca)[MT], bf16x8(&cb)[NT0], bf16x8(&na)[MT], bf16x8(&nb)[NT0]) {
            wait_vmcnt<(D - 2) * LOADS>();
            body(AccC{}, rbuf, lbuf, ca, cb, na, nb);
        };
        auto step_x = [&](auto zc, int nst, int rbuf, int lbuf, bf16x8(&ca)[MT], bf16x8(&cb)[NT0], bf16x8(&na)[MT], bf16x8(&nb)[NT0]) {
            if (nst == 0) wait_vmcnt<(D - 2) * LOADS>();
            else if (SLAB) wait_vmcnt<(D - 2) * LOADS + MT * NTG>();
            else if (POOL ? !CODES : nst <= 2) wait_vmcnt<(D - 2) * LOADS + NTG>();
            else wait_vmcnt<(D - 2) * LOADS + 2 * NTG>();
            body(zc, rbuf, lbuf, ca, cb, na, nb);
        };
        auto epilogue = [&](int tb, int co0, int nvi, int ks) {
            asm volatile("s_nop 15\n\ts_nop 15" ::: "memory");
            const int lane = fresh_lane();
            const int g4 = (lane >> 4) * 4;
            const unsigned *tb_ = tab + tb * 1024;
            const float *st = stash + wave * 64;
            const float slope = p.slope;
            if constexpr (SLAB) {
                const float *slab = reinterpret_cast<const float *>(p.out) + (long)ks * p.slab_stride;
                const unsigned chb = (unsigned)((co0 + wco * WCH + g4) * 4);
#pragma unroll
                for (int j = 0; j < NTG; ++j) {
                    const unsigned ob = tb_[(px_lo + j * 16 + (lane & 15)) * 4 + 1] + chb;
#pragma unroll
                    for (int i = 0; i < MT; ++i) {
                        const unsigned w0 = __float_as_uint(acc[i][j][0]), w1 = __float_as_uint(acc[i][j][1]), w2 = __float_as_uint(acc[i][j][2]), w3 = __float_as_uint(acc[i][j][3]);
                        if (i == 0) store16<0>(slab, ob, w0, w1, w2, w3);
                        else if (i == 1) store16<64>(slab, ob, w0, w1, w2, w3);
                        else if (i == 2) store16<128>(slab, ob, w0, w1, w2, w3);
                        else store16<192>(slab, ob, w0, w1, w2, w3);
                    }
                }
                (void)nvi; (void)st; (void)slope;
            } else if constexpr (POOL) {
                const int e = lane & 3;
                if constexpr (CODES) {
                    f32x4 bsa[MT];
#pragma unroll
                    for (int i = 0; i < MT; ++i) bsa[i] = *reinterpret_cast<const f32x4 *>(st + i * 16 + g4);
                    const unsigned chb = (unsigned)((co0 + wco * WCH + e * 16 + g4) * 2);
                    const unsigned cdb = (unsigned)((co0 + wco * WCH + e * 16) >> 2) + (unsigned)(lane >> 4);
                    const bool lrelu = p.epilogue == YOLO_EPI_BIAS_LRELU;
#pragma unroll
                    for (int j = 0; j < NTG; ++j) {
                        const unsigned obp = tb_[(px_lo + j * 16 + (lane & 15)) * 4 + 1];
                        f32x4 sel = f32x4{0.0f, 0.0f, 0.0f, 0.0f};
                        unsigned code = 0;
#pragma unroll
                        for (int i = 0; i < MT; ++i) {
                            f32x4 t;
#pragma unroll
                            for (int r = 0; r < 4; r += 2) {
                                float t0 = acc[i][j][r] + bsa[i][r], t1 = acc[i][j][r + 1] + bsa[i][r + 1];
                                t0 = (lrelu && t0 < 0.0f) ? t0 * slope : t0;
                                t1 = (lrelu && t1 < 0.0f) ? t1 * slope : t1;
                                const unsigned pk = pack_bf16x2(t0, t1);
                                t[r] = __uint_as_float(pk << 16);
                                t[r + 1] = __uint_as_float(pk & 0xffff0000u);
                            }
                            const f32x4 m = quad_max4(t);
                            unsigned key[4];
#pragma unroll
                            for (int r = 0; r < 4; ++r) key[r] = (t[r] == m[r]) ? (unsigned)e : 4u;
                            quad_min4(key);
                            const unsigned c4 = key[0] | (key[1] << 2) | (key[2] << 4) | (key[3] << 6);
                            code = (e == i) ? c4 : code;
#pragma unroll
                            for (int r = 0; r < 4; ++r) sel[r] = (e == i) ? m[r] : sel[r];
                        }
                        const unsigned lo = pack_bf16x2(sel[0], sel[1]), hi = pack_bf16x2(sel[2], sel[3]);
                        if (e < nvi) {
                            store8<0>(p.out, obp + chb, lo, hi);
                            store1(p.aux, (obp >> 3) + cdb, code);
                        }
                    }
                } else {
                const f32x4 bs = *reinterpret_cast<const f32x4 *>(st + e * 16 + g4);
                const unsigned chb = (unsigned)((co0 + wco * WCH + e * 16 + g4) * 2);
#pragma unroll
                for (int j = 0; j < NTG; ++j) {
                    const unsigned ob = tb_[(px_lo + j * 16 + (lane & 15)) * 4 + 1] + chb;
                    f32x4 sel = f32x4{0.0f, 0.0f, 0.0f, 0.0f};
#pragma unroll
                    for (int i = 0; i < MT; ++i) {
                        const f32x4 m = quad_max4(acc[i][j]);
#pragma unroll
                        for (int r = 0; r < 4; ++r) sel[r] = (e == i) ? m[r] : sel[r];
                    }
                    float v[4];
#pragma unroll
                    for (int r = 0; r < 4; ++r) {
                        const float t = sel[r] + bs[r];
                        v[r] = (p.epilogue == YOLO_EPI_BIAS_LRELU && t < 0.0f) ? t * slope : t;
                    }
                    const unsigned lo = pack_bf16x2(v[0], v[1]), hi = pack_bf16x2(v[2], v[3]);
                    if (e < nvi) store8<0>(p.out, ob, lo, hi);
                }
                }
            } else {
                const int g = lane >> 4;
                const int cl = (g & 1) * 16 + (g >> 1) * 8;
                f32x4 bs[2][2];
#pragma unroll
                for (int pr = 0; pr < 2; ++pr) {
                    bs[pr][0] = *reinterpret_cast<const f32x4 *>(st + pr * 32 + cl);
                    bs[pr][1] = *reinterpret_cast<const f32x4 *>(st + pr * 32 + cl + 4);
                }
                const unsigned chb = (unsigned)((co0 + wco * WCH + cl) * 2);
                const int my_tile = g & 1;
                const bool lrelu = p.epilogue == YOLO_EPI_BIAS_LRELU;
#pragma unroll
                for (int j = 0; j < NTG; ++j) {
                    const unsigned slot4 = (unsigned)(px_lo + j * 16 + (lane & 15)) * 4;
                    const unsigned ob = tb_[slot4 + 1] + chb;
                    uint4 ax[2];
                    if constexpr (DGRAD) {
                        const char *ap = reinterpret_cast<const char *>(p.aux) + (unsigned long)(tb_[slot4 + 2] + chb);
                        ax[0] = *reinterpret_cast<const uint4 *>(ap);
                        ax[1] = *reinterpret_cast<const uint4 *>(ap + 64);
                    }
#pragma unroll
                    for (int pr = 0; pr < 2; ++pr) {
                        f32x4 x = acc[2 * pr][j], y = acc[2 * pr + 1][j];
                        row_swap4(x, y);
                        float v[8] = {x[0], x[1], x[2], x[3], y[0], y[1], y[2], y[3]};
                        if constexpr (DGRAD == 1) {
                            const unsigned yy[4] = {ax[pr].x, ax[pr].y, ax[pr].z, ax[pr].w};
#pragma unroll
                            for (int k = 0; k < 8; ++k) {
                                const float a = __uint_as_float((k & 1) ? (yy[k >> 1] & 0xffff0000u) : (yy[k >> 1] << 16));
                                v[k] = a > 0.0f ? v[k] : v[k] * slope;
                            }
                        } else if constexpr (DGRAD == 2) {
                            const unsigned yy[4] = {ax[pr].x, ax[pr].y, ax[pr].z, ax[pr].w};
#pragma unroll
                            for (int k = 0; k < 8; ++k) {
                                float t = v[k] + bs[pr][k >> 2][k & 3];
                                t += __uint_as_float((k & 1) ? (yy[k >> 1] & 0xffff0000u) : (yy[k >> 1] << 16));
                                v[k] = t > 0.0f ? t : t * slope;
                            }
                        } else {
#pragma unroll
                            for (int k = 0; k < 8; ++k) {
                                const float t = v[k] + bs[pr][k >> 2][k & 3];
                                v[k] = lrelu ? fmaxf(t, t * slope) : t;
                            }
                        }
                        const unsigned w0 = pack_bf16x2(v[0], v[1]), w1 = pack_bf16x2(v[2], v[3]), w2 = pack_bf16x2(v[4], v[5]), w3 = pack_bf16x2(v[6], v[7]);
                        if (2 * pr + my_tile < nvi) {
                            if (pr == 0) store16<0>(p.out, ob, w0, w1, w2, w3);
                            else store16<64>(p.out, ob, w0, w1, w2, w3);
                        }
                    }
                }
            }
            __builtin_amdgcn_sched_barrier(0);
        };

        rd(0, a0, b0);
        int rbuf = 1, lbuf = D;
        auto adv = [&]() {
            rbuf = rbuf + 1 == NST ? 0 : rbuf + 1;
            lbuf = lbuf + 1 == NST ? 0 : lbuf + 1;
        };
        int nst = 0;
        bool has_next;
        int n_lim = cnt_x;
        for (int ti = 0; ti < n_lim;) {
            has_next = (unsigned)j_next < (unsigned)cnt_x;
            int co0_next, ks_next;
            unsigned px0_next;
            tile_of(has_next ? j_next : j_cur, co0_next, px0_next, ks_next);
            step_x(ZeroC{}, nst, rbuf, lbuf, a0, b0, a1, b1);
            adv();
            draw();
            build_table((ti + 1) & 1, px0_next);
            asm volatile("s_waitcnt lgkmcnt(0)" ::: "memory");
            step_x(AccC{}, nst, rbuf, lbuf, a1, b1, a0, b0);
            adv();
            for (int it = 2; it + 4 < nk; it += 2) {
                step(rbuf, lbuf, a0, b0, a1, b1);
                adv();
                step(rbuf, lbuf, a1, b1, a0, b0);
                adv();
            }
            step(rbuf, lbuf, a0, b0, a1, b1);
            adv();
            publish((ti + 1) & 1);
            load_b_voff((ti + 1) & 1);
            stage_reset(co0_next, ks_next);
            step(rbuf, lbuf, a1, b1, a0, b0);
            adv();
            step(rbuf, lbuf, a0, b0, a1, b1);
            adv();
            last_step(lbuf, a1, b1);
            adv();
#ifdef IGEMM_STAMPS
            if (ti == 0) PSTAMP(2);
            if (ti == 1) PSTAMP(4);
            if (!has_next) PSTAMP(6);
#endif
            nst = __builtin_amdgcn_readfirstlane(min(MT, max(0, (p.Cout - co0_cur - wco * WCH) >> 4)));
            epilogue(ti & 1, co0_cur, nst, ks_cur);
            ks_cur = ks_next;
#ifdef IGEMM_STAMPS
            if (ti == 0) PSTAMP(3);
            if (ti == 1) PSTAMP(5);
#endif
            rd(rbuf == 0 ? NST - 1 : rbuf - 1, a0, b0);
            if (co0_next != co0_cur) load_stash(co0_next);
            co0_cur = co0_next;
            j_cur = j_next;
            j_next = __builtin_amdgcn_readfirstlane(mail[(ti + 1) & 1]);
            ++ti;
            if (!has_next) n_lim = ti;
        }
        wait_vmcnt<0>();
        if (threadIdx.x == 0) {
            const unsigned gone = atomicAdd(p.tile_ctr + 8 + xl, 1u);
            if (gone == (unsigned)nwg_x - 1u) {
                atomicExch(p.tile_ctr + xl, 0u);
                atomicExch(p.tile_ctr + 8 + xl, 0u);
            }
        }
    };
    if (grp == 0) run(std::integral_constant<int, NT0>{});
    else run(std::integral_constant<int, NT1>{});
#ifdef IGEMM_STAMPS
    if (p.dbg && lane == 0 && blockIdx.x < 512) {
        tstamp[7] = __builtin_amdgcn_s_memtime();
#pragma unroll
        for (int i = 0; i < 8; ++i) p.dbg[((long)blockIdx.x * 8 + wave) * 8 + i] = tstamp[i];
    }
#endif
#undef PSTAMP
}

static void magic_u31(unsigned d, unsigned &magic, unsigned &shift)
{
    if (d <= 1) { magic = 0; shift = 0; return; }
    unsigned l = 0;
    while ((1ull << l) < d) ++l;
    const unsigned long long num = 1ull << (31 + l);
    magic = (unsigned)((num + d - 1) / d);
    shift = l - 1;
}

static unsigned *persist_counters(int dev)
{
    constexpr unsigned RING = 1024;
    static unsigned *ring[64] = {};
    static std::atomic<unsigned> next[64];
    static std::mutex mu;
    if (!ring[dev]) {
        std::lock_guard<std::mutex> g(mu);
        if (!ring[dev]) {
            unsigned *r = nullptr;
            if (hipMalloc(&r, RING * 16 * sizeof(unsigned)) != hipSuccess) return nullptr;
            if (hipMemset(r, 0, RING * 16 * sizeof(unsigned)) != hipSuccess || hipDeviceSynchronize() != hipSuccess) return nullptr;
            ring[dev] = r;
        }
    }
    return ring[dev] + 16u * (next[dev].fetch_add(1u, std::memory_order_relaxed) % RING);
}

template <int NTILES, bool POOL, int DGRAD, bool CODES = false, bool SLAB = false, int MT = 4>
static int persist_launch(const IgemmParams &p, int splits, hipStream_t s)
{
    using C = PersistCfg<NTILES>;
    static bool attr_done[64] = {};
    static int cus[64] = {};
    int dev = 0;
    if (hipGetDevice(&dev) != hipSuccess || dev < 0 || dev >= 64) dev = 0;
    if (!attr_done[dev]) {
        hipError_t e = hipFuncSetAttribute(reinterpret_cast<const void *>(&igemm_persist_kernel<NTILES, POOL, DGRAD, CODES, SLAB, MT>), hipFuncAttributeMaxDynamicSharedMemorySize, C::LDS_BYTES);
        if (e != hipSuccess) return fail((int)e, "yolo_igemm: hipFuncSetAttribute(%d B LDS): %s", C::LDS_BYTES, hipGetErrorString(e));
        int n = 0;
        if (hipDeviceGetAttribute(&n, hipDeviceAttributeMultiprocessorCount, dev) != hipSuccess || n <= 0) n = 256;
        cus[dev] = n;
        attr_done[dev] = true;
    }
    IgemmParams q = p;
    q.n_co_tiles = (p.Cout + 64 * MT - 1) / (64 * MT);
    if (POOL) q.tpx_valid = C::TPX;
    if (q.tpx_valid <= 0 || q.tpx_valid > C::TPX) q.tpx_valid = C::TPX;
    q.n_px_tiles = (int)((p.M + q.tpx_valid - 1) / q.tpx_valid);
    q.nk = (int)(p.Ktot / C::BK);
    if (p.px_fastest < 0) q.px_fastest = 0;
    magic_u31((unsigned)p.HoWo, q.div_hw_magic, q.div_hw_shift);
    magic_u31((unsigned)p.Wo, q.div_w_magic, q.div_w_shift);
    magic_u31((unsigned)p.Wo / 2, q.div_hw2_magic, q.div_hw2_shift);
    q.nk_per_split = q.nk / (SLAB ? splits : 1);
    const long tiles = (long)q.n_co_tiles * q.n_px_tiles * (SLAB ? splits : 1);
    const int G = (int)std::min<long>(tiles, cus[dev]);
    q.pool_tiles_x = SLAB ? splits : 1;
    q.tile_ctr = persist_counters(dev);
    if (!q.tile_ctr) return fail(2, "yolo_igemm: cannot allocate the tile counters");
    hipLaunchKernelGGL((igemm_persist_kernel<NTILES, POOL, DGRAD, CODES, SLAB, MT>), dim3(G), dim3(C::NTHR), C::LDS_BYTES, s, q);
    return check_launch("yolo_igemm (persistent)");
}

int igemm_persist_launch(const IgemmParams &p, int hint, int splits, hipStream_t s)
{
    const bool slab = splits > 1;
    if (p.stats || p.w_blocked || p.px_begin || (slab ? (!p.slab_stride || !p.out_fp32 || p.epilogue != YOLO_EPI_NONE || p.pool) : (p.slab_stride || p.out_fp32)))
        return fail(YOLO_E_UNSUPPORTED, "yolo_igemm: tile_hint %d is a bf16 launch, or split-K into fp32 slabs (split_slabs = 1, epilogue NONE); no bn_stats, blocked weights, pixel range", hint);
    if (p.tap_len % 32) return fail(YOLO_E_UNSUPPORTED, "yolo_igemm: tile_hint %d needs tap_len %% 32 == 0", hint);
    const long nk_all = p.Ktot / 32;
    if (nk_all % splits) return fail(YOLO_E_UNSUPPORTED, "yolo_igemm: tile_hint %d splits K into equal ranges", hint);
    const long nk = nk_all / splits;
    if (nk % 2 || nk < 6) return fail(YOLO_E_UNSUPPORTED, "yolo_igemm: tile_hint %d needs an even number (>= 6) of 32-deep K steps per range", hint);
    if (p.epilogue < YOLO_EPI_NONE || p.epilogue > YOLO_EPI_BIAS_ADD_LRELU) return fail(YOLO_E_UNSUPPORTED, "yolo_igemm: tile_hint %d has no epilogue %d", hint, p.epilogue);
    if (!(p.slope >= 0.0f && p.slope <= 1.0f)) return fail(YOLO_E_UNSUPPORTED, "yolo_igemm: tile_hint %d needs 0 <= slope <= 1", hint);
    if (p.Cout > 256 && p.Cout % 256) return fail(YOLO_E_UNSUPPORTED, "yolo_igemm: tile_hint %d needs Cout <= 256 or Cout %% 256 == 0", hint);
    if (p.Cout % 16) return fail(YOLO_E_UNSUPPORTED, "yolo_igemm: tile_hint %d needs Cout %% 16 == 0", hint);
    if (p.M >= (1L << 31)) return fail(YOLO_E_UNSUPPORTED, "yolo_igemm: tile_hint %d indexes fewer than 2^31 output pixels", hint);
    const long n_img = p.M / p.HoWo + 1;
    const long in_bytes = (n_img * p.in_img_stride + (long)p.KH * p.in_row_stride) * 2, w_bytes = (long)p.Cout * p.Ktot * 2;
    const long out_bytes = (n_img * p.out_img_stride + p.out_off) * (slab ? 4 : 2), aux_bytes = p.aux ? (n_img * p.aux_img_stride + p.aux_off) * 2 : 0;
    if (in_bytes >= (1L << 32) || w_bytes >= (1L << 32) || out_bytes >= (1L << 32) || aux_bytes >= (1L << 32))
        return fail(YOLO_E_UNSUPPORTED, "yolo_igemm: tile_hint %d addresses operands below 4 GB", hint);
    if ((p.out_off | p.out_px_stride | p.out_row_stride) & 3 || (p.out_img_stride & 3))
        return fail(YOLO_E_UNSUPPORTED, "yolo_igemm: tile_hint %d stores 8-byte pieces: output strides in multiples of 4 elements", hint);
    if ((p.epilogue == YOLO_EPI_MUL_DLRELU || p.epilogue == YOLO_EPI_BIAS_ADD_LRELU) && ((p.aux_off | p.aux_px_stride | p.aux_row_stride) & 3 || (p.aux_img_stride & 3)))
        return fail(YOLO_E_UNSUPPORTED, "yolo_igemm: tile_hint %d reads aux in 8-byte pieces", hint);
    if (p.pool) {
        if (hint != 21 || (p.pool != 1 && p.pool != 3) || !(p.Wo == 112 || p.Wo == 56 || p.Wo == 28) || (p.HoWo / p.Wo) % 2 || p.M % 224
            || (p.epilogue != YOLO_EPI_BIAS && p.epilogue != YOLO_EPI_BIAS_LRELU))
            return fail(YOLO_E_UNSUPPORTED, "yolo_igemm: the pooled epilogue of tile_hint 21 needs pool2 = 1 or 3, rows of 112, 56 or 28 pixels and whole 224-pixel tiles");
        if (p.pool == 3 && ((p.out_off | p.out_px_stride | p.out_row_stride) & 7 || (p.out_img_stride & 7) || (p.Cout & 7)))
            return fail(YOLO_E_UNSUPPORTED, "yolo_igemm: pool2 = 3 needs Cout and the output strides in multiples of 8");
        if (p.Cout > 128 && p.Cout <= 192)
            return p.pool == 3 ? persist_launch<14, true, 0, true, false, 3>(p, 1, s) : persist_launch<14, true, 0, false, false, 3>(p, 1, s);
        return p.pool == 3 ? persist_launch<14, true, 0, true>(p, 1, s) : persist_launch<14, true, 0>(p, 1, s);
    }
    if (slab && p.Cout % 256) return fail(YOLO_E_UNSUPPORTED, "yolo_igemm: tile_hint %d splits K only for Cout %% 256 == 0", hint);
    if (slab) return hint == 20 ? persist_launch<13, false, 0, false, true>(p, splits, s) : persist_launch<14, false, 0, false, true>(p, splits, s);
    const int dg = p.epilogue == YOLO_EPI_MUL_DLRELU ? 1 : (p.epilogue == YOLO_EPI_BIAS_ADD_LRELU ? 2 : 0);
    switch (hint) {
    case 20: return dg == 1 ? persist_launch<13, false, 1>(p, 1, s) : (dg == 2 ? persist_launch<13, false, 2>(p, 1, s) : persist_launch<13, false, 0>(p, 1, s));
    case 21: return dg == 1 ? persist_launch<14, false, 1>(p, 1, s) : (dg == 2 ? persist_launch<14, false, 2>(p, 1, s) : persist_launch<14, false, 0>(p, 1, s));
    }
    return fail(YOLO_E_ARG, "yolo_igemm: tile_hint %d is not a persistent configuration", hint);
}

}
```

### yolo-v1_amd/yolo/_hip.py

```python

from __future__ import annotations

import ctypes
import os

import torch

_HERE = os.path.dirname(os.path.abspath(__file__))
LIB_PATH = os.environ.get("YOLO_HIP_LIB") or os.path.join(_HERE, "libyolo_hip.so")
_LIB = None

ABI_VERSION = 2
BN_ACC_REPLICAS = 16
c_int, c_long, c_float, c_double, c_void_p = ctypes.c_int, ctypes.c_long, ctypes.c_float, ctypes.c_double, ctypes.c_void_p


class IgemmDesc(ctypes.Structure):

    _fields_ = [
        ("N", ctypes.c_int32), ("Ho", ctypes.c_int32), ("Wo", ctypes.c_int32),
        ("in_img_stride", ctypes.c_int64),
        ("in_row_stride", ctypes.c_int32), ("in_px_stride", ctypes.c_int32), ("in_off", ctypes.c_int32),
        ("stride", ctypes.c_int32), ("KH", ctypes.c_int32), ("KW", ctypes.c_int32),
        ("tap_len", ctypes.c_int32), ("Cout", ctypes.c_int32),
        ("out_img_stride", ctypes.c_int64),
        ("out_row_stride", ctypes.c_int32), ("out_px_stride", ctypes.c_int32), ("out_off", ctypes.c_int32),
        ("epilogue", ctypes.c_int32), ("slope", ctypes.c_float), ("out_fp32", ctypes.c_int32), ("split_k", ctypes.c_int32),
        ("aux_img_stride", ctypes.c_int64),
        ("aux_row_stride", ctypes.c_int32), ("aux_px_stride", ctypes.c_int32), ("aux_off", ctypes.c_int32),
        ("pool2", ctypes.c_int32),
        ("w_blocked", ctypes.c_int32),
        ("tile_order", ctypes.c_int32),
        ("tile_hint", ctypes.c_int32),
        ("px_begin", ctypes.c_int64), ("px_end", ctypes.c_int64),
        ("skew_phases", ctypes.c_int32), ("skew_step", ctypes.c_int32),
        ("bn_stats", ctypes.c_void_p),
        ("tile_px", ctypes.c_int32), ("split_slabs", ctypes.c_int32),
    ]


class WgradDesc(ctypes.Structure):

    _fields_ = [
        ("P", ctypes.c_int64),
        ("dy_px_stride", ctypes.c_int32), ("x_px_stride", ctypes.c_int32),
        ("Cout", ctypes.c_int32), ("Cin", ctypes.c_int32),
        ("KH", ctypes.c_int32), ("KW", ctypes.c_int32), ("pad", ctypes.c_int32),
        ("x_row_stride", ctypes.c_int64),
        ("split", ctypes.c_int32), ("accumulate", ctypes.c_int32), ("variant", ctypes.c_int32),
        ("geo_W", ctypes.c_int32), ("geo_H", ctypes.c_int32), ("geo_img_slots", ctypes.c_int32), ("geo_row_slots", ctypes.c_int32),
        ("geo_px_slots", ctypes.c_int32), ("geo_slot0", ctypes.c_int32),
        ("dw_sumsq", ctypes.c_void_p),
        ("slabs", ctypes.c_void_p), ("slab_floats", ctypes.c_int64),
    ]


class PoolDesc(ctypes.Structure):

    _fields_ = [("N", ctypes.c_int32), ("H", ctypes.c_int32), ("W", ctypes.c_int32), ("C", ctypes.c_int32),
                ("in_halo", ctypes.c_int32), ("out_halo", ctypes.c_int32)]


class AdamTensor(ctypes.Structure):

    _fields_ = [("p", c_void_p), ("g", c_void_p), ("m", c_void_p), ("v", c_void_p), ("p_bf16", c_void_p), ("n", ctypes.c_long)]


class SgdTensor(ctypes.Structure):

    _fields_ = [("p", c_void_p), ("g", c_void_p), ("buf", c_void_p), ("p_bf16", c_void_p), ("n", ctypes.c_long)]


class ConvPackItem(ctypes.Structure):

    _fields_ = [("w", c_void_p), ("wf", c_void_p), ("wd", c_void_p), ("Cout", c_int), ("Cin", c_int), ("KH", c_int), ("KW", c_int)]


class ConvUnpackItem(ctypes.Structure):

    _fields_ = [("dwp", c_void_p), ("dw", c_void_p), ("Cout", c_int), ("Cin", c_int), ("KH", c_int), ("KW", c_int)]


class AugmentDesc(ctypes.Structure):

    _fields_ = [("src_off", ctypes.c_int64), ("tmp_off", ctypes.c_int64),
                ("Hs", ctypes.c_int32), ("Ws", ctypes.c_int32),
                ("top", ctypes.c_int32), ("left", ctypes.c_int32), ("ch", ctypes.c_int32), ("cw", ctypes.c_int32),
                ("htab", c_void_p), ("vtab", c_void_p),
                ("hk", ctypes.c_int32), ("vk", ctypes.c_int32),
                ("n_ops", ctypes.c_int32), ("ops", ctypes.c_int32 * 3),
                ("brightness", ctypes.c_float), ("saturation", ctypes.c_float), ("hue_shift", ctypes.c_int32), ("reserved", ctypes.c_int32)]


AUG_BRIGHTNESS, AUG_SATURATION, AUG_HUE = 0, 1, 2
EPI_NONE, EPI_BIAS, EPI_BIAS_LRELU, EPI_MUL_DLRELU, EPI_BIAS_ADD_LRELU = 0, 1, 2, 3, 4
NMS_INFERENCE, NMS_METRICS = 0, 1

_SIGS = {
    "yolo_hip_abi_version": [],
    "yolo_debug_stamps": [c_void_p, c_int],
    "yolo_stream_create": [c_int, ctypes.POINTER(c_void_p)],
    "yolo_decode": [c_void_p, c_int, c_int, c_int, c_int, c_double, c_void_p, c_void_p, c_void_p],
    "yolo_decode_gt": [c_void_p, c_int, c_int, c_int, c_int, c_void_p, c_void_p, c_void_p],
    "yolo_nms": [c_void_p, c_void_p, c_int, c_int, c_double, c_int, c_void_p, c_void_p, c_void_p],
    "yolo_batchnorm_train_fwd": [c_void_p, c_int, c_int, c_int, c_int, c_int, c_void_p, c_void_p, c_double, c_double, c_void_p, c_void_p, c_void_p, c_int,
                                 c_int, c_void_p, c_void_p, c_void_p, c_int, c_void_p, c_int, c_void_p],
    "yolo_batchnorm_bwd": [c_void_p, c_int, c_void_p, c_int, c_void_p, c_int, c_int, c_int, c_int, c_int, c_void_p, c_void_p, c_void_p, ctypes.c_long, ctypes.c_long,
                           ctypes.c_long, ctypes.c_long, c_int, c_int, c_void_p, c_void_p, c_void_p, c_void_p, c_void_p],
    "yolo_map_match": [c_void_p, c_void_p, c_void_p, c_int, c_int, c_void_p, c_void_p, c_int, ctypes.POINTER(c_double), c_int, c_double, c_double, c_double,
                       c_void_p, c_void_p, c_void_p],
    "yolo_pairwise_iou": [c_void_p, c_int, c_void_p, c_int, c_int, c_void_p, c_void_p],
    "yolo_loss_fwd_bwd": [c_void_p, c_void_p, c_int, c_int, c_int, c_int, c_float, c_float, c_void_p, c_void_p, c_void_p, c_void_p],
    "yolo_loss_iou": [c_void_p, c_void_p, c_long, c_void_p, c_void_p],
    "yolo_igemm": [ctypes.POINTER(IgemmDesc), c_void_p, c_void_p, c_void_p, c_void_p, c_void_p, c_void_p],
    "yolo_igemm_finish": [ctypes.POINTER(IgemmDesc), c_void_p, c_void_p, c_void_p, c_void_p, c_void_p],
    "yolo_wgrad": [ctypes.POINTER(WgradDesc), c_void_p, c_void_p, c_void_p, c_void_p, c_void_p],
    "yolo_wgrad_slab_floats": [ctypes.POINTER(WgradDesc), ctypes.POINTER(ctypes.c_long)],
    "yolo_conv_stem7_fwd": [c_void_p, c_void_p, c_void_p, c_int, c_int, c_int, c_long, c_int, c_float, c_int, c_void_p, c_long, c_int, c_int, c_void_p, c_long,
                            c_int, c_int, c_void_p],
    "yolo_conv_stem7_fwd_f32": [c_void_p, c_void_p, c_void_p, c_int, c_int, c_int, c_float, c_int, c_void_p, c_long, c_int, c_int, c_void_p, c_long, c_int, c_int,
                                c_void_p],
    "yolo_wgrad_stem7": [c_void_p, c_void_p, c_int, c_int, c_int, c_long, c_int, c_long, c_int, c_int, c_void_p, c_void_p, c_void_p, c_long, c_void_p],
    "yolo_wgrad_stem7_pooled": [c_void_p, c_void_p, c_int, c_int, c_int, c_long, c_int, c_long, c_int, c_int, c_void_p, c_long, c_int, c_int, c_float, c_void_p,
                                c_void_p, c_void_p, c_long, c_void_p],
    "yolo_wgrad_stem7_codes": [c_void_p, c_void_p, c_void_p, c_int, c_int, c_int, c_long, c_int, c_void_p, c_long, c_int, c_int, c_float, c_void_p, c_void_p, c_void_p,
                               c_long, c_void_p],
    "yolo_maxpool3s2_fwd": [ctypes.POINTER(PoolDesc), c_void_p, c_void_p, c_void_p],
    "yolo_maxpool3s2_bwd": [ctypes.POINTER(PoolDesc), c_void_p, c_void_p, c_void_p, c_int, c_void_p],
    "yolo_maxpool2_fwd": [ctypes.POINTER(PoolDesc), c_void_p, c_void_p, c_void_p],
    "yolo_maxpool2_bwd_lrelu": [ctypes.POINTER(PoolDesc), c_void_p, c_void_p, c_float, c_void_p, c_void_p],
    "yolo_maxpool2_bwd_codes": [ctypes.POINTER(PoolDesc), c_void_p, c_void_p, c_void_p, c_float, c_void_p, c_void_p],
    "yolo_nchw_f32_to_nhwc_bf16": [c_void_p, c_int, c_int, c_int, c_int, c_void_p, c_int, c_int, c_int, c_void_p],
    "yolo_nhwc_bf16_to_nchw_f32": [c_void_p, c_int, c_int, c_int, c_int, c_int, c_void_p, c_void_p],
    "yolo_nhwc_bf16_to_nchw_bf16": [c_void_p, c_int, c_int, c_int, c_int, c_int, c_void_p, c_void_p],
    "yolo_scale_rows_to_bf16": [c_void_p, c_void_p, c_float, c_void_p, c_float, c_int, c_int, c_int, c_void_p, c_void_p],
    "yolo_dropout_bf16": [c_void_p, c_void_p, c_float, c_long, c_void_p, c_void_p],
    "yolo_pack_conv_weight": [c_void_p, c_int, c_int, c_int, c_int, c_int, c_int, c_void_p, c_void_p, c_void_p],
    "yolo_pack_fc_weight": [c_void_p, c_int, c_int, c_int, c_void_p, c_void_p, c_void_p],
    "yolo_pack_fc_weight_blocked": [c_void_p, c_int, c_long, c_void_p, c_void_p],
    "yolo_pack_fc_weight_blocked_hwc": [c_void_p, c_int, c_int, c_int, c_void_p, c_void_p],
    "yolo_unpack_conv_wgrad": [c_void_p, c_int, c_int, c_int, c_int, c_int, c_int, c_void_p, c_int, c_void_p],
    "yolo_im2col_rows": [c_void_p, c_long, c_int, c_int, c_int, c_int, c_int, c_int, c_int, c_int, c_int, c_void_p, c_void_p],
    "yolo_transpose_f32_to_bf16": [c_void_p, c_int, c_int, c_void_p, c_int, c_void_p],
    "yolo_transpose_bf16": [c_void_p, c_int, c_int, c_int, c_void_p, c_int, c_void_p],
    "yolo_fc_dgrad_to_nhwc": [c_void_p, c_int, c_int, c_int, c_int, c_int, c_void_p, c_float, c_void_p, c_void_p],
    "yolo_cast_f32_to_bf16": [c_void_p, c_long, c_void_p, c_void_p],
    "yolo_cast_bf16_to_f32": [c_void_p, c_long, c_void_p, c_void_p],
    "yolo_preprocess_u8": [c_void_p, c_int, c_int, c_int, c_int, c_int, c_void_p, c_void_p, c_int, c_void_p, c_void_p, c_int, c_void_p,
                           ctypes.POINTER(c_float), ctypes.POINTER(c_float), c_void_p, c_int, c_void_p, c_void_p],
    "yolo_augment_u8": [c_void_p, ctypes.c_int64, ctypes.POINTER(AugmentDesc), c_void_p, c_int, c_int, c_int, c_void_p, ctypes.c_int64,
                        ctypes.POINTER(c_float), ctypes.POINTER(c_float), c_void_p, c_int, c_void_p, c_void_p, c_void_p],
    "yolo_sumsq_f32": [c_void_p, c_long, c_void_p, c_void_p],
    "yolo_adam_step": [c_void_p, c_void_p, c_void_p, c_void_p, c_long, c_float, c_float, c_float, c_float, c_float, c_long, c_void_p, c_float, c_void_p, c_void_p],
    "yolo_clip_scale_f32": [c_void_p, c_long, c_void_p, c_float, c_void_p],
    "yolo_pack_conv_weights_multi": [ctypes.POINTER(ConvPackItem), c_int, c_void_p],
    "yolo_unpack_conv_wgrads_multi": [ctypes.POINTER(ConvUnpackItem), c_int, c_void_p],
    "yolo_sumsq_f32_multi": [c_void_p, c_void_p, c_int, c_void_p, c_void_p],
    "yolo_sumsq_fixed_slots": [ctypes.POINTER(c_long), c_int, ctypes.POINTER(c_long)],
    "yolo_sumsq_f32_fixed": [c_void_p, c_long, c_void_p, c_long, c_void_p, c_void_p],
    "yolo_sumsq_f32_multi_fixed": [c_void_p, c_void_p, c_int, c_void_p, c_long, c_void_p, c_void_p],
    "yolo_adam_step_multi": [ctypes.POINTER(AdamTensor), c_int, c_float, c_float, c_float, c_float, c_float, c_long, c_void_p, c_float, c_void_p, c_void_p],
    "yolo_adam_step_multi_bg": [ctypes.POINTER(AdamTensor), c_int, c_float, c_float, c_float, c_float, c_float, c_long, c_void_p, c_float, c_void_p, c_int, c_void_p],
    "yolo_sgd_step": [c_void_p, c_void_p, c_void_p, c_long, c_float, c_float, c_float, c_float, c_int, c_int, c_void_p, c_float, c_void_p, c_void_p, c_void_p],
    "yolo_sgd_step_multi": [ctypes.POINTER(SgdTensor), c_int, c_float, c_float, c_float, c_float, c_int, c_int, c_void_p, c_float, c_void_p, c_void_p],
    "yolo_sgd_step_multi_bg": [ctypes.POINTER(SgdTensor), c_int, c_float, c_float, c_float, c_float, c_int, c_int, c_void_p, c_float, c_void_p, c_int, c_void_p],
    "yolo_bias_lrelu_rows": [c_void_p, c_void_p, c_int, c_int, c_float, c_void_p, c_void_p, c_void_p],
    "yolo_bias_lrelu_rows_slabs": [c_void_p, c_int, c_void_p, c_int, c_int, c_float, c_void_p, c_void_p, c_void_p],
}


def available() -> bool:
    return os.path.exists(LIB_PATH)


def lib():
    global _LIB
    if _LIB is None:
        if not os.path.exists(LIB_PATH):
            raise RuntimeError(
                f"{LIB_PATH} not found: the gfx950 HIP library is not built (run `make -C yolo-v1_amd/csrc` or "
                "`python -c 'import __graft_entry__ as g; g.build()'`).  This package has no CPU/eager fallback for GPU tensors.")
        L = ctypes.CDLL(LIB_PATH)
        L.yolo_hip_abi_version.argtypes, L.yolo_hip_abi_version.restype = [], c_int
        if L.yolo_hip_abi_version() != ABI_VERSION:
            raise RuntimeError(f"{LIB_PATH} has ABI version {L.yolo_hip_abi_version()}, this package binds version {ABI_VERSION}: rebuild it "
                               "(`make -C yolo-v1_amd/csrc`)")
        for name, args in _SIGS.items():
            fn = getattr(L, name)
            fn.argtypes = args
            fn.restype = c_int
        L.yolo_hip_last_error.argtypes = []
        L.yolo_hip_last_error.restype = ctypes.c_char_p
        _LIB = L
    return _LIB


E_ARG, E_UNSUPPORTED = -1, -2


class HipUnsupported(RuntimeError):
    """the library refused a shape / configuration (YOLO_E_UNSUPPORTED) -- nothing was launched"""


def check(rc: int, what: str = "") -> None:
    if rc != 0:
        msg = lib().yolo_hip_last_error().decode(errors="replace")
        raise (HipUnsupported if rc == E_UNSUPPORTED else RuntimeError)(f"libyolo_hip {what} failed (code {rc}): {msg}")


def ptr(t) -> c_void_p:
    return c_void_p(None) if t is None else c_void_p(t.data_ptr())


def stream() -> c_void_p:
    return c_void_p(torch.cuda.current_stream().cuda_stream)


def side_stream(device, low: bool = True) -> "torch.cuda.Stream":
    with torch.cuda.device(device):
        h = c_void_p()
        check(lib().yolo_stream_create(1 if low else 0, ctypes.byref(h)), "yolo_stream_create")
        return torch.cuda.ExternalStream(h.value, device=device)


def require_cuda(*tensors) -> None:
    dev = None
    for t in tensors:
        if t is None:
            continue
        if not t.is_cuda:
            raise RuntimeError("libyolo_hip kernels need device tensors (got a CPU tensor)")
        if dev is None:
            dev = t.device
        elif t.device != dev:
            raise RuntimeError(f"libyolo_hip kernels need all tensors on one device (got {dev} and {t.device})")


def device_guard(fn):
    import functools

    @functools.wraps(fn)
    def wrapper(*args, **kw):
        dev = None
        for a in (*args, *kw.values()):
            if isinstance(a, torch.Tensor) and a.is_cuda:
                if dev is None:
                    dev = a.device
                elif a.device != dev:
                    raise RuntimeError(f"{fn.__name__}: tensors on different devices ({dev} and {a.device})")
        if dev is None or dev.index == torch.cuda.current_device():
            return fn(*args, **kw)
        with torch.cuda.device(dev):
            return fn(*args, **kw)

    return wrapper
```

### yolo-v1_amd/yolo/config.py

```python

from __future__ import annotations

from dataclasses import dataclass, fields


@dataclass
class EngineConfig:
    TIMERS: list | None = None
    IGEMM_LAUNCHES: int = 0
    TUNE_LOG: list | None = None
    AUTOTUNE: bool = False
    TILE_HINT: int = 0
    TILE_PX: int = 0
    PLAN_TABLE: bool = True
    BORROW_PLANS: bool = True
    SMALL_SPLIT: bool = True
    PERSIST: bool = True
    BN_STATS_IN_CONV: bool = True
    STEM_KERNEL: bool = True
    STEM_POOL_BWD_FUSED: bool = True
    STRIDE2_CLASSES: bool = True
    STEM_F32_INPUT: bool = True
    FLATTEN_FREE: bool = True
    POOL_CODES: bool = True
    FUSE_POOL: bool = True
    FC_NORM_IN_WGRAD: int = 1 << 26
    WGRAD_STREAM: bool = True
    SIDE_LOW: bool = True
    WGRAD_SLABS: bool = False
    WGRAD_PIPE: bool = True
    WGRAD_CHOICE: object = None
    PLAN_TIMES: object = None
    TUNE_REPS: int = 1
    FC_WGRAD_SIDE: bool = True
    DETERMINISTIC: bool = False
    WGRAD_WIDE: bool = True


def _from_env(cfg: EngineConfig) -> EngineConfig:
    import os
    for f in fields(EngineConfig):
        v = os.environ.get("YOLO_AMD_" + f.name)
        if v is None:
            continue
        if f.type not in ("bool", "int"):
            raise ValueError(f"YOLO_AMD_{f.name}: only the bool / int switches can be set from the environment")
        setattr(cfg, f.name, bool(int(v)) if f.type == "bool" else int(v))
    return cfg


CONFIG = _from_env(EngineConfig())
SWITCHES = frozenset(f.name for f in fields(EngineConfig))
```

### yolo-v1_amd/yolo/executor.py

```python

from __future__ import annotations

import ctypes
from dataclasses import dataclass

import torch
import torch.nn as nn

from . import _hip
from ._hip import (EPI_BIAS, EPI_BIAS_LRELU, EPI_MUL_DLRELU, EPI_NONE, ConvPackItem, ConvUnpackItem, IgemmDesc, PoolDesc, WgradDesc, check, ptr)
from .config import CONFIG as CFG
from .plans import igemm_call
from .runtime import RT, Act, _attach_wgrad_slabs, _EventSlot, _igemm, _on_side_stream, _round_up, _timed

@dataclass
class Layer:
    kind: str
    name: str = ""
    Cout: int = 0
    Cin: int = 0
    K: int = 1
    stride: int = 1
    pad: int = 0
    lrelu: bool = False
    dropout: float = 0.0
    drop_mod: object = None
    weight: nn.Parameter | None = None
    bias: nn.Parameter | None = None
    first: bool = False
    Hin: int = 0
    Win: int = 0
    Hout: int = 0
    Wout: int = 0


class Plan:

    SLOPE = 0.1

    def __init__(self, layers: list[Layer], in_channels: int, input_is_image: bool, S: int | None = None):
        self.layers = layers
        self.in_channels = in_channels
        self.input_is_image = input_is_image
        self.params: list[nn.Parameter] = []
        for L in layers:
            if L.kind in ("conv", "fc"):
                self.params += [L.weight, L.bias]
        self._pf: dict[int, tuple] = {}
        self._pd: dict[int, tuple] = {}
        self._pfb: dict[int, tuple] = {}
        self._pd2: dict[int, tuple] = {}
        self._ws: dict[tuple, list] = {}
        self.grad_norm_sq: dict = {}
        self.debug_keep = False
        self.last = None
        self.arena = None
        self.arena_views: dict[int, tuple] = {}
        self.on_grad_ready = None
        self.on_backward_done = None
        self.on_stream_wait = None
        self.cfg = None
        self.params_ready = _EventSlot()
        self.owner = None

    @property
    def c(self):
        return self.cfg if self.cfg is not None else CFG

    def attach_grad_arena(self, device) -> torch.Tensor:
        order = [li for li in reversed(range(len(self.layers))) if self.layers[li].kind in ("conv", "fc")]
        off = 0
        wv, bv = {}, {}
        for li in order:
            n = self.layers[li].weight.numel()
            wv[li] = (off, off + n, _round_up(off + n, 64))
            off = _round_up(off + n, 64)
        self._arena_w_end = off
        for li in order:
            n = self.layers[li].bias.numel()
            bv[li] = (off, off + n)
            off = _round_up(off + n, 64)
        self.arena = torch.zeros(off, dtype=torch.float32, device=device)
        self.arena_views = {li: (self.arena[wv[li][0]:wv[li][1]].view_as(self.layers[li].weight),
                                 self.arena[bv[li][0]:bv[li][1]].view_as(self.layers[li].bias), wv[li][0], wv[li][2])
                            for li in order}
        return self.arena

    @staticmethod
    def _side_stream(dev) -> "torch.cuda.Stream":
        key = torch.device(dev).index
        if key not in RT._SIDE_STREAMS:
            RT._SIDE_STREAMS[key] = RT.STREAMS.side(dev, CFG.SIDE_LOW)
        return RT._SIDE_STREAMS[key]

    def _layer_done(self, li: int):
        if self.arena is not None and self.on_grad_ready is not None:
            _, _, a, b = self.arena_views[li]
            self.on_grad_ready(a, b)

    @staticmethod
    def from_modules(mods, in_channels: int, input_is_image: bool) -> "Plan":
        layers: list[Layer] = []
        i = 0
        mods = list(mods)
        while i < len(mods):
            m = mods[i]
            nxt = mods[i + 1] if i + 1 < len(mods) else None
            if isinstance(m, nn.Conv2d):
                k, s, p = m.kernel_size[0], m.stride[0], m.padding[0]
                if m.kernel_size[0] != m.kernel_size[1] or m.groups != 1 or m.dilation != (1, 1) or m.bias is None:
                    raise ValueError(f"unsupported conv {m}")
                act = isinstance(nxt, nn.LeakyReLU)
                if act and abs(nxt.negative_slope - Plan.SLOPE) > 1e-12:
                    raise ValueError("only LeakyReLU(0.1) is fused")
                first = (m.in_channels == 3 and k == 7 and s == 2 and p == 3)
                if not first and not ((k == 3 and p == 1) or (k == 1 and p == 0)) or (not first and s not in (1, 2)):
                    raise ValueError(f"unsupported conv geometry {m}")
                if not first and (m.in_channels % 32 or m.out_channels % 8):
                    raise ValueError(f"unsupported channel counts {m}")
                layers.append(Layer("conv", Cout=m.out_channels, Cin=m.in_channels, K=k, stride=s, pad=p, lrelu=act,
                                    weight=m.weight, bias=m.bias, first=first))
                i += 2 if act else 1
            elif isinstance(m, nn.MaxPool2d):
                ks = m.kernel_size if isinstance(m.kernel_size, int) else m.kernel_size[0]
                st = m.stride if isinstance(m.stride, int) else m.stride[0]
                if ks != 2 or st != 2:
                    raise ValueError("only MaxPool2d(2,2)")
                layers.append(Layer("pool"))
                i += 1
            elif isinstance(m, nn.Flatten):
                layers.append(Layer("flatten"))
                i += 1
            elif isinstance(m, nn.Linear):
                if m.in_features % 64 or m.bias is None:
                    raise ValueError(f"unsupported Linear {m}: in_features must be a multiple of 64")
                act = isinstance(nxt, nn.LeakyReLU)
                j = i + (2 if act else 1)
                drop, drop_mod = 0.0, None
                if j < len(mods) and isinstance(mods[j], nn.Dropout):
                    drop, drop_mod = mods[j].p, mods[j]
                    j += 1
                layers.append(Layer("fc", Cout=m.out_features, Cin=m.in_features, lrelu=act, dropout=drop, drop_mod=drop_mod, weight=m.weight, bias=m.bias))
                i = j
            else:
                raise ValueError(f"unsupported module in plan: {m}")
        return Plan(layers, in_channels, input_is_image)

    @staticmethod
    def _wkey(w):
        return (w._version, w.data_ptr())

    def _multi_ok(self, L: Layer) -> bool:
        return L.kind == "conv" and not L.first and L.Cout % 64 == 0 and L.Cin % 64 == 0 and L.K * L.K <= 9

    def _src(self, L: Layer):
        wsrc = L.weight.detach()
        if wsrc.dtype != torch.float32 or not wsrc.is_contiguous():
            wsrc = wsrc.float().contiguous()
        return wsrc

    def _pack_all(self, need_dgrad: bool):
        items, keep, done = [], [], []
        for li, L in enumerate(self.layers):
            if not self._multi_ok(L):
                continue
            key = self._wkey(L.weight)
            f, d = self._pf.get(li), self._pd.get(li)
            want_f = f is None or f[0] != key
            want_d = need_dgrad and li > 0 and (d is None or d[0] != key)
            if not (want_f or want_d):
                continue
            dev = L.weight.device
            wsrc = self._src(L)
            keep.append(wsrc)
            wf = wd = None
            if want_f:
                wf = f[1] if f is not None else torch.empty((L.Cout, L.K, L.K, L.Cin), dtype=torch.bfloat16, device=dev)
            if want_d:
                wd = d[1] if d is not None else torch.empty((L.Cin, L.K, L.K, L.Cout), dtype=torch.bfloat16, device=dev)
            items.append(ConvPackItem(wsrc.data_ptr(), wf.data_ptr() if wf is not None else None, wd.data_ptr() if wd is not None else None,
                                      L.Cout, L.Cin, L.K, L.K))
            done.append((li, key, wf, wd))
        if items:
            tab = (ConvPackItem * len(items))(*items)
            check(RT.lib().yolo_pack_conv_weights_multi(tab, len(items), RT.stream()), "pack_conv_weights_multi")
            for li, key, wf, wd in done:
                if wf is not None:
                    self._pf[li] = (key, wf)
                if wd is not None:
                    self._pd[li] = (key, wd)

    def _pack(self, li: int, need_dgrad: bool):
        L = self.layers[li]
        key = self._wkey(L.weight)
        f, d = self._pf.get(li), self._pd.get(li)
        ok_f = f is not None and f[0] == key
        ok_d = d is not None and d[0] == key
        if ok_f and (ok_d or not need_dgrad):
            return f[1], (d[1] if ok_d else None)
        dev = L.weight.device
        wsrc = self._src(L)
        wf = f[1] if f is not None else None
        wd = d[1] if d is not None else None
        if L.kind == "conv":
            if L.first:
                if wf is None:
                    wf = torch.empty((L.Cout, 7, 8, 4), dtype=torch.bfloat16, device=dev)
                check(RT.lib().yolo_pack_conv_weight(ptr(wsrc), L.Cout, 3, 7, 7, 4, 8, ptr(wf), None, RT.stream()), "pack_conv_weight")
                self._pf[li] = (key, wf)
                return wf, None
            if wf is None:
                wf = torch.empty((L.Cout, L.K, L.K, L.Cin), dtype=torch.bfloat16, device=dev)
            if need_dgrad and wd is None:
                wd = torch.empty((L.Cin, L.K, L.K, L.Cout), dtype=torch.bfloat16, device=dev)
            check(RT.lib().yolo_pack_conv_weight(ptr(wsrc), L.Cout, L.Cin, L.K, L.K, L.Cin, L.K, None if ok_f else ptr(wf),
                                              ptr(wd) if (need_dgrad and not ok_d) else None, RT.stream()), "pack_conv_weight")
        else:
            if not ok_f:
                if wf is None:
                    wf = torch.empty((L.Cout, L.Cin), dtype=torch.bfloat16, device=dev)
                check(RT.lib().yolo_cast_f32_to_bf16(ptr(wsrc), wsrc.numel(), ptr(wf), RT.stream()), "cast fc weight")
            if need_dgrad and not ok_d:
                ld = _round_up(L.Cout, 32)
                if wd is None:
                    wd = torch.zeros((L.Cin, ld), dtype=torch.bfloat16, device=dev)
                check(RT.lib().yolo_transpose_f32_to_bf16(ptr(wsrc), L.Cout, L.Cin, ptr(wd), ld, RT.stream()), "transpose")
        self._pf[li] = (key, wf)
        if need_dgrad:
            self._pd[li] = (key, wd)
            return wf, wd
        return wf, (wd if ok_d else None)

    def _stride2_panels(self, li: int, wdg: torch.Tensor) -> dict:
        L = self.layers[li]
        key = self._wkey(L.weight)
        hit = self._pd2.get(li)
        if hit is not None and hit[0] == key:
            return hit[1]
        sel = {0: slice(1, 2), 1: slice(0, 3, 2)}
        panels = {}
        for py in (0, 1):
            for px in (0, 1):
                panels[(py, px)] = wdg[:, sel[py], sel[px], :].contiguous()
        self._pd2[li] = (key, panels)
        return panels

    def _pack_fc_blocked(self, li: int, hwc=None):
        L = self.layers[li]
        key = (self._wkey(L.weight), hwc)
        hit = self._pfb.get(li)
        if hit is not None and hit[0] == key:
            return hit[1]
        wsrc = self._src(L)
        wb = hit[1] if hit is not None else torch.empty((_round_up(L.Cout, 128) * L.Cin,), dtype=torch.bfloat16, device=L.weight.device)
        if hwc is not None:
            check(RT.lib().yolo_pack_fc_weight_blocked_hwc(ptr(wsrc), L.Cout, hwc[0], hwc[1], ptr(wb), RT.stream()), "pack_fc_blocked_hwc")
        else:
            check(RT.lib().yolo_pack_fc_weight_blocked(ptr(wsrc), L.Cout, L.Cin, ptr(wb), RT.stream()), "pack_fc_blocked")
        self._pfb[li] = (key, wb)
        return wb

    def fc_biases(self):
        return [L.bias for L in self.layers if L.kind == "fc" and L.bias is not None and L.bias.is_cuda]

    def bf16_shadows(self):
        out = []
        for li, L in enumerate(self.layers):
            if L.kind != "fc" or not L.weight.is_cuda:
                continue
            wf, _ = self._pack(li, False)

            def fresh(p, li=li, wf=wf):
                self._pf[li] = (self._wkey(p), wf)
            out.append((L.weight, wf, fresh))
        return out

    def _workspace(self, N: int, x_shape, device, train: bool):
        key = (N, tuple(x_shape[1:]), str(device), train)
        pool = self._ws.setdefault(key, [])
        if pool:
            ws = pool.pop()
            self._apply_geom(ws)
            return key, ws
        ws = {"acts": [], "grads": {}, "misc": {}, "geom": {}}
        C, H, W = x_shape[1], x_shape[2], x_shape[3]
        if self.layers and self.layers[0].kind == "conv" and self.layers[0].first:
            a = Act(N, H, W, 4, 3, device)
        else:
            a = Act(N, H, W, C, 1, device)
        ws["in"] = a
        cur = a
        flat = None
        for li, L in enumerate(self.layers):
            if L.kind == "conv":
                L.Hin, L.Win = cur.H, cur.W
                L.Hout = (cur.H + 2 * L.pad - L.K) // L.stride + 1
                L.Wout = (cur.W + 2 * L.pad - L.K) // L.stride + 1
                dense = (not train and self.c.FLATTEN_FREE and li + 2 < len(self.layers) and self.layers[li + 1].kind == "flatten"
                         and self.layers[li + 2].kind == "fc" and L.Cout % 8 == 0 and (L.Cout * L.Hout * L.Wout) % 64 == 0)
                cur = Act(N, L.Hout, L.Wout, L.Cout, 0 if dense else 1, device)
            elif L.kind == "pool":
                L.Hin, L.Win = cur.H, cur.W
                cur = Act(N, cur.H // 2, cur.W // 2, cur.C, 1, device)
            elif L.kind == "flatten":
                flat = torch.empty((N, cur.C * cur.H * cur.W), dtype=torch.bfloat16, device=device)
                cur = flat
            elif L.kind == "fc":
                feat = flat.shape[1] if (flat is not None and cur is flat) else None
                if feat is not None and feat != L.Cin:
                    raise RuntimeError(f"mat1 and mat2 shapes cannot be multiplied ({N}x{feat} and {L.Cin}x{L.Cout}): input of "
                                       f"{tuple(x_shape[2:])} pixels does not match the Linear layer behind nn.Flatten")
                cur = None
            ws["acts"].append(cur)
            ws["geom"][li] = (L.Hin, L.Win, L.Hout, L.Wout)
        return key, ws

    def _apply_geom(self, ws):
        for li, g in ws["geom"].items():
            L = self.layers[li]
            L.Hin, L.Win, L.Hout, L.Wout = g

    def _release(self, key, ws):
        self._ws.setdefault(key, []).append(ws)

    def _conv_desc(self, L: Layer, a_in: Act, a_out: Act) -> IgemmDesc:
        d = IgemmDesc()
        d.N, d.Ho, d.Wo = a_in.N, L.Hout, L.Wout
        d.in_img_stride, d.in_row_stride, d.in_px_stride = a_in.img_stride, a_in.row_stride, a_in.px_stride
        d.stride = L.stride
        if L.first:
            d.in_off = 0
            d.KH, d.KW, d.tap_len = 7, 1, 32
        else:
            d.in_off = a_in.interior_off(L.pad)
            d.KH, d.KW, d.tap_len = L.K, L.K, L.Cin
        d.Cout = L.Cout
        d.out_img_stride, d.out_row_stride, d.out_px_stride = a_out.img_stride, a_out.row_stride, a_out.px_stride
        d.out_off = a_out.interior_off()
        d.epilogue = EPI_BIAS_LRELU if L.lrelu else EPI_BIAS
        d.slope = self.SLOPE
        d.out_fp32 = 0
        d.split_k = 1
        d.tile_hint, d.tile_px = self.c.TILE_HINT, self.c.TILE_PX
        return d

    @staticmethod
    def _pool_fusable(L: Layer) -> bool:
        if L.Cout % 8:
            return False
        if L.Hout % 8 == 0 and L.Wout % 16 == 0:
            return True
        nk = L.K * L.K * L.Cin // 32
        return (not L.first and L.Cin % 32 == 0 and nk % 2 == 0 and nk >= 4 and L.Wout in (112, 56, 28) and L.Hout % 2 == 0
                and (L.Hout * L.Wout) % 112 == 0)

    def _few_tiles(self, L: Layer, N: int) -> bool:
        tiles = ((N * L.Hout * L.Wout + 223) // 224) * ((L.Cout + 255) // 256)
        return bool(self.c.SMALL_SPLIT and not L.first and tiles < 64 and L.K * L.K * L.Cin >= 2304 and L.Cin % 64 == 0)

    @_hip.device_guard
    def forward(self, x: torch.Tensor, train: bool, drop_training: bool, u8_size=None):
        from .augment import U8Batch
        L_ = RT.lib()
        st = RT.stream()
        N = x.shape[0]
        dev = x.device
        stem_f32 = False
        if isinstance(x, U8Batch):
            key, ws = self._workspace(N, x.shape, dev, train)
            self._pack_all(train)
            a = ws["in"]
            if not (a.C == 4 and a.halo == 3):
                raise ValueError("uint8 input needs a plan that starts with the 7x7/s2 stem")
            x.into_act(a)
        elif u8_size is not None:
            x = x.detach()
            from . import preprocess as _pp
            key, ws = self._workspace(N, (N, 3, u8_size[0], u8_size[1]), dev, train)
            self._pack_all(train)
            a = ws["in"]
            if not (a.C == 4 and a.halo == 3):
                raise ValueError("uint8 input needs a plan that starts with the 7x7/s2 stem")
            _pp.preprocess_u8_into(x, u8_size, a)
        else:
            x = x.detach()
            if x.dim() != 4 or x.shape[1] != self.in_channels:
                raise RuntimeError(f"expected input of shape (N, {self.in_channels}, H, W), got {tuple(x.shape)}")
            if x.dtype != torch.float32 or not x.is_contiguous():
                x = x.float().contiguous()
            key, ws = self._workspace(N, x.shape, dev, train)
            self._pack_all(train)
            a = ws["in"]
            L0 = self.layers[0]
            stem_f32 = (not train and self.c.STEM_F32_INPUT and self.c.STEM_KERNEL and a.C == 4 and a.halo == 3 and L0.kind == "conv" and L0.first and L0.Cout == 64
                        and L0.Hout % 8 == 0 and L0.Wout % 16 == 0 and 2 * L0.Hout == x.shape[2] and 2 * L0.Wout == x.shape[3]
                        and ws["acts"][0].C == 64 and L0.bias.dtype == torch.float32)
            if stem_f32:
                pass
            elif a.C == 4 and a.halo == 3:
                check(L_.yolo_nchw_f32_to_nhwc_bf16(ptr(x), N, x.shape[1], x.shape[2], x.shape[3], a.p, 4, 3, 3, st), "nchw->nhwc4")
            else:
                check(L_.yolo_nchw_f32_to_nhwc_bf16(ptr(x), N, x.shape[1], x.shape[2], x.shape[3], a.p, a.C, 1, 1, st), "nchw->nhwc")
        cur = a
        fc_saved = {}
        out = None
        skip_pool = False
        self.grad_norm_sq.clear()
        hwc = None
        codes_mode = train and self.c.POOL_CODES and self.debug_keep is not True
        ws["codes"] = set()
        for li, L in enumerate(self.layers):
            nxt = ws["acts"][li]
            if L.kind == "conv":
                wf, _ = self._pack(li, train)
                fuse = (not train and self.c.FUSE_POOL and li + 1 < len(self.layers) and self.layers[li + 1].kind == "pool"
                        and self._pool_fusable(L) and not self._few_tiles(L, N))
                if fuse:
                    nxt = ws["acts"][li + 1]
                d = self._conv_desc(L, cur, nxt)
                d.pool2 = 1 if fuse else 0
                b = L.bias.detach()
                if L.first and self.c.STEM_KERNEL and L.Cout == 64 and L.Hout % 8 == 0 and L.Wout % 16 == 0 and nxt.C == 64 and b.dtype == torch.float32:
                    dual = (train and self.c.FUSE_POOL and li + 1 < len(self.layers) and self.layers[li + 1].kind == "pool")
                    full = nxt if dual else None
                    dst = ws["acts"][li + 1] if dual else nxt
                    codes = self._codes(ws, li, dst) if (dual and codes_mode) else None
                    with _timed(f"conv{li}" + ("+pool" if (fuse or dual) else ""), "stem", 2.0 * N * L.Hout * L.Wout * L.Cout * L.Cin * L.K * L.K):
                        if stem_f32 and li == 0:
                            check(L_.yolo_conv_stem7_fwd_f32(ptr(x), ptr(wf), ptr(b), N, x.shape[2], x.shape[3], self.SLOPE if L.lrelu else 1.0,
                                                             1 if fuse else 0, dst.p, dst.img_stride, dst.row_stride, dst.interior_off(), None, 0, 0, 0, st),
                                  "conv_stem7_fwd_f32")
                        elif codes is not None:
                            check(L_.yolo_conv_stem7_fwd(cur.p, ptr(wf), ptr(b), N, L.Hout, L.Wout, cur.img_stride, cur.row_stride,
                                                         self.SLOPE if L.lrelu else 1.0, 3, dst.p, dst.img_stride, dst.row_stride,
                                                         dst.interior_off(), ptr(codes), 0, 0, 0, st), "conv_stem7_fwd")
                        else:
                            check(L_.yolo_conv_stem7_fwd(cur.p, ptr(wf), ptr(b), N, L.Hout, L.Wout, cur.img_stride, cur.row_stride,
                                                         self.SLOPE if L.lrelu else 1.0, 1 if (fuse or dual) else 0, dst.p, dst.img_stride, dst.row_stride,
                                                         dst.interior_off(), full.p if dual else None, full.img_stride if dual else 0,
                                                         full.row_stride if dual else 0, full.interior_off() if dual else 0, st), "conv_stem7_fwd")
                    cur = dst
                    skip_pool = fuse or dual
                    continue
                dual = (train and self.c.FUSE_POOL and not fuse and li + 1 < len(self.layers) and self.layers[li + 1].kind == "pool"
                        and self._pool_fusable(L) and not L.first)
                if dual:
                    full, pooled = nxt, ws["acts"][li + 1]
                    d = self._conv_desc(L, cur, pooled)
                    codes = self._codes(ws, li, pooled) if codes_mode else None
                    if codes is not None:
                        d.pool2 = 3
                        auxp = ptr(codes)
                    else:
                        d.pool2 = 2
                        d.aux_img_stride, d.aux_row_stride, d.aux_px_stride, d.aux_off = full.img_stride, full.row_stride, full.px_stride, full.interior_off()
                        auxp = full.p
                    with _timed(f"conv{li}+pool", "igemm", 2.0 * N * L.Hout * L.Wout * L.Cout * L.Cin * L.K * L.K):
                        igemm_call(d, cur.p, ptr(wf), ptr(b), auxp, pooled.p, st, f"igemm conv{li}")
                    cur = pooled
                    skip_pool = True
                    continue
                with _timed(f"conv{li}" + ("+pool" if fuse else ""), "igemm", 2.0 * N * L.Hout * L.Wout * L.Cout * L.Cin * L.K * L.K):
                    igemm_call(d, cur.p, ptr(wf), ptr(b), None, nxt.p, st, f"igemm conv{li}")
                cur = nxt
                skip_pool = fuse
            elif L.kind == "pool" and skip_pool:
                skip_pool = False
            elif L.kind == "pool":
                pd = PoolDesc(N, cur.H, cur.W, cur.C, cur.halo, nxt.halo)
                with _timed(f"pool{li}", "maxpool2_fwd"):
                    check(L_.yolo_maxpool2_fwd(ctypes.byref(pd), cur.p, nxt.p, st), "maxpool")
                cur = nxt
            elif L.kind == "flatten":
                if not train and isinstance(cur, Act) and cur.halo == 0 and cur.halo_hi == 0 and self.c.FLATTEN_FREE:
                    hwc = (cur.C, cur.H * cur.W)
                    cur = cur.t.view(N, -1)
                    continue
                check(L_.yolo_nhwc_bf16_to_nchw_bf16(cur.p, N, cur.C, cur.H, cur.W, cur.halo, ptr(nxt), st), "flatten")
                cur = nxt
            elif L.kind == "fc":
                self.params_ready.wait(dev)
                if train:
                    wf, _ = self._pack(li, False)
                else:
                    wf = self._pack_fc_blocked(li, hwc)
                    hwc = None
                xin = cur
                K = L.Cin
                d = IgemmDesc()
                d.N, d.Ho, d.Wo = N, 1, 1
                d.in_img_stride, d.in_row_stride, d.in_px_stride, d.in_off = xin.shape[1], 0, xin.shape[1], 0
                d.stride, d.KH, d.KW, d.tap_len, d.Cout = 1, 1, 1, K, L.Cout
                d.out_img_stride, d.out_row_stride, d.out_px_stride, d.out_off = L.Cout, 0, L.Cout, 0
                d.slope = self.SLOPE
                d.out_fp32 = 1
                d.w_blocked = 0 if train else 1
                last = (li == len(self.layers) - 1)
                nk = K // 64
                splits = max(1, min(32 if d.w_blocked else 48, nk // 16)) if K >= 4096 else 1
                b = L.bias.detach()
                if splits > 1:
                    acc = RT._splitk_scratch(splits * N * L.Cout, zero=False)
                    d.epilogue, d.split_k, d.split_slabs = EPI_NONE, splits, 1
                    with _timed(f"fc{li}", "igemm", 2.0 * N * L.Cout * L.Cin):
                        _igemm(L_, d, ptr(xin), ptr(wf), None, None, ptr(acc), st, f"igemm fc{li}")
                    yb = torch.empty((N, L.Cout), dtype=torch.bfloat16, device=dev) if not last else None
                    yf = torch.empty((N, L.Cout), dtype=torch.float32, device=dev) if last else None
                    check(L_.yolo_bias_lrelu_rows_slabs(ptr(acc), splits, ptr(b), N, L.Cout, self.SLOPE if L.lrelu else 1.0, ptr(yb), ptr(yf), st),
                          "bias_lrelu_rows")
                else:
                    yf = torch.empty((N, L.Cout), dtype=torch.float32, device=dev)
                    d.epilogue, d.split_k = (EPI_BIAS_LRELU if L.lrelu else EPI_BIAS), 1
                    with _timed(f"fc{li}", "igemm", 2.0 * N * L.Cout * L.Cin):
                        _igemm(L_, d, ptr(xin), ptr(wf), ptr(b), None, ptr(yf), st, f"igemm fc{li}")
                    yb = None
                    if not last:
                        yb = torch.empty((N, L.Cout), dtype=torch.bfloat16, device=dev)
                        check(L_.yolo_cast_f32_to_bf16(ptr(yf), yf.numel(), ptr(yb), st), "cast")
                mask = None
                y_act = yb
                if L.drop_mod is not None:
                    L.dropout = float(L.drop_mod.p)
                if not last and L.dropout > 0 and drop_training:
                    mask = (torch.rand((N, L.Cout), device=dev) >= L.dropout).to(torch.uint8)
                    yd = torch.empty_like(yb)
                    check(L_.yolo_dropout_bf16(ptr(yb), ptr(mask), 1.0 / max(1.0 - L.dropout, 1e-12) if L.dropout < 1.0 else 0.0, yb.numel(), ptr(yd), st), "dropout")
                    cur = yd
                else:
                    cur = yb
                fc_saved[li] = (xin, y_act, mask)
                if last:
                    out = yf
        if out is None:
            out = torch.empty((N, cur.C, cur.H, cur.W), dtype=torch.float32, device=dev)
            check(L_.yolo_nhwc_bf16_to_nchw_f32(cur.p, N, cur.C, cur.H, cur.W, cur.halo, ptr(out), st), "nhwc->nchw")
        saved = (key, ws, fc_saved, N, dev) if train else None
        if not train:
            self._release(key, ws)
        return out, saved

    @staticmethod
    def _codes(ws, li: int, pooled: Act) -> torch.Tensor:
        c = ws["misc"].get(("codes", li))
        if c is None:
            c = torch.empty(pooled.t.numel() // 8, dtype=torch.int16, device=pooled.t.device)
            ws["misc"][("codes", li)] = c
        ws["codes"].add(li)
        return c

    def _grad_buf(self, ws, li: int, N, dev) -> Act:
        g = ws["grads"].get(li)
        if g is None:
            L = self.layers[li]
            if L.stride == 1 or L.first:
                g = Act(N, L.Hout, L.Wout, L.Cout, 1, dev)
            else:
                g = Act(N, L.Hin, L.Win, L.Cout, 1, dev)
            ws["grads"][li] = g
        return g

    def _grad_out_strides(self, L: Layer, g: Act):
        if L.stride == 1 or L.first:
            return g.img_stride, g.row_stride, g.px_stride, g.interior_off()
        return g.img_stride, 2 * g.row_stride, 2 * g.px_stride, g.interior_off()

    @staticmethod
    def _wgrad_desc(L: Layer, g: Act, xin: Act, N: int) -> WgradDesc:
        px = N * L.Hout * L.Wout
        deep = (L.Cout >= 512 and L.Cin >= 256 and px >= 40000) or (L.Cout >= 1024 and L.Cin >= 1024 and px >= 12000)
        variant = 5 if (CFG.WGRAD_PIPE and L.K == 3 and L.stride == 1 and deep) else 0
        flat = False
        if CFG.WGRAD_PIPE and CFG.WGRAD_WIDE and L.K == 3 and L.stride == 1:
            if (deep and L.Cin < 1024) or (L.Cin == 64 and L.Cout >= 192 and px >= 500000):
                variant = 6
                flat = L.Hout >= 56 and L.Wout >= 56
        geo_ok = L.Hout >= 2 and L.Wout >= 2
        geo = variant >= 5 or (geo_ok and (L.stride > 1 or g.Hp * g.Wp >= 1.12 * L.Hout * L.Wout))
        choice = CFG.WGRAD_CHOICE.get((N, L.Hout, L.Wout, L.Cout, L.Cin, L.K, L.stride)) if CFG.WGRAD_CHOICE else None
        if choice is not None and L.K == 3 and L.stride == 1 and CFG.WGRAD_PIPE and (int(choice[0]) != 6 or CFG.WGRAD_WIDE):
            variant, flat = int(choice[0]), bool(choice[1])
            geo = geo_ok and not flat
        if not flat and geo:
            return WgradDesc(N * L.Hout * L.Wout, g.px_stride, xin.px_stride, L.Cout, L.Cin, L.K, L.K, L.pad, xin.row_stride, 0, 0, variant,
                             L.Wout, L.Hout, g.Hp * g.Wp, g.Wp * L.stride, L.stride, g.halo * g.Wp + g.halo)
        return WgradDesc(N * g.Hp * g.Wp, g.px_stride, xin.px_stride, L.Cout, L.Cin, L.K, L.K, L.pad, xin.row_stride, 0, 0, variant)

    def backward(self, saved, gout: torch.Tensor, need_gx: bool):
        L_ = RT.lib()
        st = RT.stream()
        key, ws, fc_saved, N, dev = saved
        self._apply_geom(ws)
        if self.arena is not None:
            self.arena[self._arena_w_end:].zero_()
        grads: dict[int, tuple] = {}
        nl = len(self.layers)
        offs, tot = {}, 0
        for i, L in enumerate(self.layers):
            if L.kind == "conv":
                offs[("w", i)] = tot
                tot += _round_up(L.Cout * 7 * 8 * 4 if L.first else L.Cout * L.K * L.K * L.Cin, 64)
        btot = 0
        if self.arena is None:
            for i, L in enumerate(self.layers):
                if L.kind in ("conv", "fc"):
                    offs[("b", i)] = btot
                    btot += _round_up(L.Cout, 64)
        scratch = ws["misc"].get("wgrad_scratch")
        if scratch is None or scratch.numel() < tot:
            scratch = ws["misc"]["wgrad_scratch"] = torch.empty(max(tot, 1), dtype=torch.float32, device=dev)
        bscratch = torch.zeros(max(btot, 1), dtype=torch.float32, device=dev)

        def grad_tensors(i):
            L = self.layers[i]
            if self.arena is not None:
                dw, db, _, _ = self.arena_views[i]
                return dw, db
            o = offs[("b", i)]
            return torch.empty_like(L.weight, dtype=torch.float32), bscratch[o: o + L.Cout]

        pending: list[tuple] = []
        stem_dpool = None

        def flush():
            items = [ConvUnpackItem(dwp.data_ptr(), dw.data_ptr(), L.Cout, L.Cin, L.K, L.K) for (i, L, dwp, dw) in pending if self._multi_ok(L)]
            if items:
                check(L_.yolo_unpack_conv_wgrads_multi((ConvUnpackItem * len(items))(*items), len(items), RT.stream()), "unpack_conv_wgrads_multi")
            for (i, L, dwp, dw) in pending:
                if not self._multi_ok(L):
                    if L.first:
                        check(L_.yolo_unpack_conv_wgrad(ptr(dwp), L.Cout, 3, 7, 7, 4, 8, ptr(dw), 0, RT.stream()), "unpack")
                    else:
                        check(L_.yolo_unpack_conv_wgrad(ptr(dwp), L.Cout, L.Cin, L.K, L.K, L.Cin, L.K, ptr(dw), 0, RT.stream()), "unpack")
                self._layer_done(i)
            pending.clear()

        gout = gout.detach()
        if gout.dtype != torch.float32 or not gout.is_contiguous():
            gout = gout.float().contiguous()

        main_t = RT.STREAMS.current(dev)
        side_t = self._side_stream(dev) if self.c.WGRAD_STREAM else None
        det = bool(self.c.DETERMINISTIC)

        def _on_side():
            return _on_side_stream(main_t, side_t, self.on_stream_wait if self.arena is not None else None)

        with _on_side():
            scratch.zero_()
        fc_keep: list = []

        def input_of(li):
            return ws["in"] if li == 0 else ws["acts"][li - 1]

        g_flat = None
        g_act: Act | None = None
        li = nl - 1
        if self.layers[li].kind == "fc":
            g_flat = gout.reshape(N, -1)
        else:
            L = self.layers[li]
            y = ws["acts"][li]
            graw = Act(N, y.H, y.W, y.C, 1, dev)
            check(L_.yolo_nchw_f32_to_nhwc_bf16(ptr(gout), N, y.C, y.H, y.W, graw.p, y.C, 1, 1, st), "gout->nhwc")
            if L.kind == "conv":
                g = self._grad_buf(ws, li, N, dev)
                self._apply_dlrelu_into(graw, y, L, g, st)
                g_act = g
            else:
                assert L.kind == "pool", "plans end with fc, conv or pool"
                g_act = graw

        while li >= 0:
            L = self.layers[li]
            if L.kind == "fc":
                xin, y_act, mask = fc_saved[li]
                last = (li == nl - 1)
                ldg = _round_up(L.Cout, 32)
                gb = torch.empty((N, ldg), dtype=torch.bfloat16, device=dev)
                check(L_.yolo_scale_rows_to_bf16(ptr(g_flat), ptr(mask), ((1.0 / (1.0 - L.dropout)) if L.dropout < 1.0 else 0.0) if mask is not None else 1.0,
                                                 ptr(y_act) if (L.lrelu and not last) else None, self.SLOPE, N, L.Cout, ldg, ptr(gb), st), "scale_rows")
                dw, db = grad_tensors(li)
                wd = WgradDesc(N, ldg, L.Cin, L.Cout, L.Cin, 1, 1, 0, 0, 1, 0)
                nsq = None
                if det:
                    pass
                elif L.Cout * L.Cin >= self.c.FC_NORM_IN_WGRAD and L.Cin % 4 == 0:
                    nsq = torch.zeros((), dtype=torch.float64, device=dev)
                    wd.dw_sumsq = nsq.data_ptr()
                if self.c.FC_WGRAD_SIDE and side_t is not None:
                    fc_keep.append(gb)
                    with _on_side() as wst:
                        if det:
                            _attach_wgrad_slabs(L_, wd, dev, wst)
                        with _timed(f"fc{li}.wgrad", "wgrad", 2.0 * N * L.Cout * L.Cin):
                            check(L_.yolo_wgrad(ctypes.byref(wd), ptr(xin), ptr(gb), ptr(dw), ptr(db), wst), f"wgrad fc{li}")
                        self._layer_done(li)
                else:
                    if det:
                        _attach_wgrad_slabs(L_, wd, dev, st)
                    with _timed(f"fc{li}.wgrad", "wgrad", 2.0 * N * L.Cout * L.Cin):
                        check(L_.yolo_wgrad(ctypes.byref(wd), ptr(xin), ptr(gb), ptr(dw), ptr(db), st), f"wgrad fc{li}")
                    self._layer_done(li)
                if nsq is not None:
                    self.grad_norm_sq[id(L.weight)] = ((dw.data_ptr(), tuple(dw.shape)), dw._version, nsq)
                grads[li] = (dw, db)
                need_prev = li > 0 or need_gx
                behind_flatten = li >= 2 and self.layers[li - 1].kind == "flatten" and self.layers[li - 2].kind in ("conv", "pool")
                if need_prev and behind_flatten:
                    Lc = self.layers[li - 2]
                    y = ws["acts"][li - 2]
                    wf, _ = self._pack(li, False)
                    ldn = _round_up(N, 8)
                    gT = torch.zeros((L.Cout, ldn), dtype=torch.bfloat16, device=dev)
                    check(L_.yolo_transpose_bf16(ptr(gb), N, L.Cout, ldg, ptr(gT), ldn, st), "transpose g")
                    dxT = torch.zeros((L.Cin, N), dtype=torch.float32, device=dev)
                    wd = WgradDesc(L.Cout, L.Cin, ldn, L.Cin, N, 1, 1, 0, 0, 0, 1)
                    if det:
                        wd.accumulate = 0
                        _attach_wgrad_slabs(L_, wd, dev, st)
                    with _timed(f"fc{li}.dgrad", "wgrad", 2.0 * N * L.Cout * L.Cin):
                        check(L_.yolo_wgrad(ctypes.byref(wd), ptr(gT), ptr(wf), ptr(dxT), None, st), f"dgrad fc{li}")
                    if Lc.kind == "conv":
                        assert Lc.stride == 1, "nn.Flatten is expected after a stride-1 conv or a pool"
                        g = self._grad_buf(ws, li - 2, N, dev)
                        yact = y.p if Lc.lrelu else None
                    else:
                        g = ws["misc"].get("graw_flat")
                        if g is None:
                            g = Act(N, y.H, y.W, y.C, 1, dev)
                            ws["misc"]["graw_flat"] = g
                        yact = None
                    check(L_.yolo_fc_dgrad_to_nhwc(ptr(dxT), N, y.C, y.H, y.W, 1, yact, self.SLOPE, g.p, st), "fc_dgrad_to_nhwc")
                    g_act = g
                    g_flat = None
                    li -= 2
                    continue
                if need_prev:
                    _, wt = self._pack(li, True)
                    d = IgemmDesc()
                    d.N, d.Ho, d.Wo = N, 1, 1
                    d.in_img_stride, d.in_row_stride, d.in_px_stride, d.in_off = ldg, 0, ldg, 0
                    d.stride, d.KH, d.KW, d.tap_len, d.Cout = 1, 1, 1, ldg, L.Cin
                    d.out_img_stride, d.out_row_stride, d.out_px_stride, d.out_off = L.Cin, 0, L.Cin, 0
                    d.epilogue, d.slope, d.out_fp32, d.split_k = EPI_NONE, self.SLOPE, 1, 1
                    gprev = torch.empty((N, L.Cin), dtype=torch.float32, device=dev)
                    with _timed(f"fc{li}.dgrad", "igemm", 2.0 * N * L.Cout * L.Cin):
                        _igemm(L_, d, ptr(gb), ptr(wt), None, None, ptr(gprev), st, f"dgrad fc{li}")
                    g_flat = gprev
                li -= 1
            elif L.kind == "flatten":
                raise AssertionError("nn.Flatten is handled together with the Linear layer behind it")
            elif L.kind == "pool":
                lc = li - 1
                Lc = self.layers[lc]
                assert Lc.kind == "conv" and Lc.lrelu, "MaxPool2d is expected right after conv+LeakyReLU"
                yfull = ws["acts"][lc]
                if (lc == 0 and Lc.first and self.c.STEM_POOL_BWD_FUSED and Lc.Cout == 64 and Lc.Hout % 8 == 0 and Lc.Wout % 16 == 0 and g_act.halo == 1
                        and not need_gx):
                    stem_dpool = g_act
                    li -= 1
                    continue
                g = self._grad_buf(ws, lc, N, dev)
                pd = PoolDesc(N, yfull.H, yfull.W, yfull.C, 1, 1)
                with _timed(f"pool{li}.bwd", "maxpool2_bwd"):
                    if lc in ws.get("codes", ()):
                        ypool = ws["acts"][li]
                        assert (ypool.Hp, ypool.Wp, ypool.C, ypool.halo) == (g_act.Hp, g_act.Wp, g_act.C, g_act.halo)
                        check(L_.yolo_maxpool2_bwd_codes(ctypes.byref(pd), ypool.p, ptr(ws["misc"][("codes", lc)]), g_act.p, self.SLOPE, g.p, st), "maxpool_bwd_codes")
                    else:
                        check(L_.yolo_maxpool2_bwd_lrelu(ctypes.byref(pd), yfull.p, g_act.p, self.SLOPE, g.p, st), "maxpool_bwd")
                g_act = g
                li -= 1
            elif L.kind == "conv":
                g = g_act
                xin = input_of(li)
                dw, db = grad_tensors(li)
                with _on_side() as wst:
                    o = offs[("w", li)]
                    stem_direct = L.first and L.Cout == 64 and L.Hout % 8 == 0 and L.Wout % 16 == 0
                    if stem_direct:
                        part = ws["misc"].get("stem_part")
                        if part is None:
                            part = torch.empty((768 * 14400,), dtype=torch.float32, device=dev)
                            ws["misc"]["stem_part"] = part
                        with _timed(f"conv{li}.wgrad", "wgrad", 2.0 * N * L.Hout * L.Wout * L.Cout * 147):
                            if stem_dpool is not None and 0 in ws.get("codes", ()):
                                yp = ws["acts"][1]
                                assert (yp.Hp, yp.Wp, yp.C, yp.halo) == (stem_dpool.Hp, stem_dpool.Wp, stem_dpool.C, stem_dpool.halo)
                                check(L_.yolo_wgrad_stem7_codes(xin.p, yp.p, ptr(ws["misc"][("codes", 0)]), N, L.Hout, L.Wout, xin.img_stride, xin.row_stride,
                                                                stem_dpool.p, stem_dpool.img_stride, stem_dpool.row_stride, stem_dpool.interior_off(),
                                                                self.SLOPE if L.lrelu else 1.0, ptr(dw), ptr(db), ptr(part), part.numel(), wst), "wgrad_stem7_codes")
                            elif stem_dpool is not None:
                                yf = ws["acts"][0]
                                check(L_.yolo_wgrad_stem7_pooled(xin.p, yf.p, N, L.Hout, L.Wout, xin.img_stride, xin.row_stride, yf.img_stride, yf.row_stride,
                                                                 yf.interior_off(), stem_dpool.p, stem_dpool.img_stride, stem_dpool.row_stride,
                                                                 stem_dpool.interior_off(), self.SLOPE if L.lrelu else 1.0, ptr(dw), ptr(db), ptr(part),
                                                                 part.numel(), wst), "wgrad_stem7_pooled")
                            else:
                                check(L_.yolo_wgrad_stem7(xin.p, g.p, N, L.Hout, L.Wout, xin.img_stride, xin.row_stride, g.img_stride, g.row_stride,
                                                          g.interior_off(), ptr(dw), ptr(db), ptr(part), part.numel(), wst), "wgrad_stem7")
                        grads[li] = (dw, db)
                        flush()
                        self._layer_done(li)
                    elif L.first:
                        xcol = ws["misc"].get("xcol")
                        if xcol is None:
                            xcol = Act(N, L.Hout, L.Wout, 7 * 32, 1, dev)
                            ws["misc"]["xcol"] = xcol
                        check(L_.yolo_im2col_rows(xin.p, xin.img_stride, xin.row_stride, xin.px_stride, 2, 7, 32, N, L.Hout, L.Wout, 1, xcol.p, wst), "im2col_rows")
                        dwp = scratch[o: o + L.Cout * 7 * 8 * 4]
                        split = max(1, min(1024, g.slots // 4096))
                        wd = WgradDesc(g.slots, g.px_stride, xcol.px_stride, L.Cout, 7 * 32, 1, 1, 0, xcol.row_stride, split, 0)
# ... 148 lines not shown
```

### yolo-v1_amd/yolo/plans.py

```python

from __future__ import annotations

import ctypes
import os

import torch

from . import _hip
from ._hip import EPI_BIAS, EPI_BIAS_ADD_LRELU, EPI_BIAS_LRELU, EPI_MUL_DLRELU, EPI_NONE, IgemmDesc, check, ptr
from .config import CONFIG as CFG
from .runtime import RT, _igemm

_TUNE_CANDIDATES = (5, 11, 12, 3, 4)
_TUNED: dict = {}
_FLUSH = None
PLAN_FILE = os.path.join(os.path.dirname(os.path.abspath(__file__)), "plans", "gfx950.json")


def _key_str(key) -> str:
    return ",".join(str(int(v)) for v in key)


def load_plans(path: str = PLAN_FILE) -> int:
    import json
    if not os.path.exists(path):
        return 0
    with open(path) as f:
        data = json.load(f)
    for k, v in data.get("plans", {}).items():
        _TUNED[tuple(int(t) for t in k.split(","))] = tuple(v)
    if data.get("wgrad"):
        CFG.WGRAD_CHOICE = dict(CFG.WGRAD_CHOICE or {})
        CFG.WGRAD_CHOICE.update({tuple(int(t) for t in k.split(",")): tuple(int(t) for t in v) for k, v in data["wgrad"].items()})
    return len(data.get("plans", {}))


def save_plans(path: str = PLAN_FILE, note: str = "") -> None:
    import json
    os.makedirs(os.path.dirname(path), exist_ok=True)
    body = {"arch": "gfx950", "key": "N,Ho,Wo,KH,KW,tap_len,Cout,stride,epilogue,pool2,out_px_stride,in_px_stride", "note": note,
            "plans": {_key_str(k): list(v) for k, v in sorted(_TUNED.items())}}
    if CFG.WGRAD_CHOICE:
        body["wgrad"] = {_key_str(k): list(v) for k, v in sorted(CFG.WGRAD_CHOICE.items())}
    with open(path, "w") as f:
        json.dump(body, f, indent=0, separators=(",", ":"))
        f.write("\n")


def _flush_caches(dev):
    global _FLUSH
    if _FLUSH is None or _FLUSH.device != dev:
        _FLUSH = torch.empty(512 << 20, dtype=torch.uint8, device=dev)
    _FLUSH.fill_(1)


_TILE = {1: (128, 128), 3: (128, 64), 4: (64, 128), 5: (128, 128), 10: (64, 128), 11: (256, 128), 12: (256, 256), 13: (256, 128), 14: (256, 208),
         15: (256, 208), 16: (256, 224), 17: (128, 208), 18: (128, 224), 19: (64, 16),
         20: (256, 208), 21: (256, 224),
         22: (64, 256)}
_TAIL_CANDIDATES = (5, 3, 4)
_TILE_COST = {12: (256, 1.00), 14: (256, 0.80), 11: (256, 0.54), 5: (512, 0.36), 3: (512, 0.20), 4: (512, 0.20)}

def _pipe_ok(d: IgemmDesc) -> bool:
    nk = d.KH * d.KW * d.tap_len // 32
    return d.tap_len % 32 == 0 and nk % 2 == 0 and nk >= 4 and not d.bn_stats and not d.w_blocked


def _persist_ok(d: IgemmDesc) -> bool:
    nk = d.KH * d.KW * d.tap_len // 32
    return (d.tap_len % 32 == 0 and nk % 2 == 0 and nk >= 6 and not d.bn_stats and not d.w_blocked and not d.out_fp32 and d.split_k <= 1
            and (d.Cout <= 256 or d.Cout % 256 == 0) and d.Cout % 16 == 0 and d.epilogue in (EPI_NONE, EPI_BIAS, EPI_BIAS_LRELU, EPI_MUL_DLRELU, EPI_BIAS_ADD_LRELU))


def _pipe_pool_ok(d: IgemmDesc) -> bool:
    return _pipe_ok(d) and d.Wo in (112, 56, 28) and d.Ho % 2 == 0 and (d.Ho * d.Wo) % 112 == 0 and d.Cout % 8 == 0


def _default_plan(d: IgemmDesc):
    M = d.N * d.Ho * d.Wo
    if d.pool2:
        if d.Ho % 8 == 0 and d.Wo % 16 == 0 and not (_pipe_pool_ok(d) and d.Cout >= 192):
            return (0, 0)
        if _persist_ok(d) and d.pool2 in (1, 3) and M % 224 == 0 and d.Cout > 128:
            return ("tile", 21, 1, 0)
        return ("tile", 16 if d.Cout > 128 else 18, 1, 0)
    if M < 2048 or (M < 8192 and ((d.Cout + 63) // 64) * ((M + 127) // 128) < 256):
        ktot = d.KH * d.KW * d.tap_len
        if (CFG.SMALL_SPLIT and ktot >= 2304 and d.tap_len % 64 == 0 and d.Cout % 8 == 0 and not d.out_fp32 and not d.bn_stats and d.split_k <= 1
                and d.epilogue in (EPI_NONE, EPI_BIAS, EPI_BIAS_LRELU, EPI_MUL_DLRELU)):
            hint = 3 if (M + 63) // 64 * 64 < (M + 127) // 128 * 128 else 4
            tco, tpx = _TILE[hint]
            tiles = ((d.Cout + tco - 1) // tco) * ((M + tpx - 1) // tpx)
            S = 2
            while S < 32 and tiles * S < 512 and (ktot // 64) // (2 * S) >= 8:
                S *= 2
            return ("slabs", hint, S, 0)
        if M < 2048:
            return (0, 0)
    if _persist_ok(d) and d.Cout >= 192 and M * ((d.Cout + 255) // 256) >= 96 * 208:
        return ("tile", 20, 1, 196 if M % 196 == 0 else 208)
    best, best_t = (0, 0), None
    for hint, (slots, cost) in _TILE_COST.items():
        tco, tpx = _TILE[hint]
        forms = [((hint, 1), tpx)]
        if hint == 14:
            h = 15 if _pipe_ok(d) else 14
            forms = [(("tile", h, 1, 196), 196)] if M % 196 == 0 else [(("tile", h, 1, 208), 208)]
        for plan, px in forms:
            tiles = ((d.Cout + tco - 1) // tco) * ((M + px - 1) // px)
            t = ((tiles + slots - 1) // slots) * cost
            if best_t is None or t < best_t - 1e-9:
                best, best_t = plan, t
    return best


_BORROWED = set()


def _borrowed_plan(key):
    n = key[0]
    if not (CFG.BORROW_PLANS and CFG.PLAN_TABLE) or n < 8:
        return None
    sizes = sorted({k[0] for k in _TUNED if k[1:] == key[1:] and k not in _BORROWED and k[0] != n})
    if not sizes:
        return None
    nb = min(sizes, key=lambda b: (max(b, n) / min(b, n), -b))
    plan = _TUNED[(nb,) + tuple(key[1:])]
    if isinstance(plan[0], int) and len(plan) == 4:
        return None
    return plan


def _run_plan_igemm(L_, d: IgemmDesc, plan, inp, w, bias, aux, out, st, what):
    if d.bn_stats and (plan[0] in ("splitk", "slabs") or (isinstance(plan[0], int) and len(plan) == 4)):
        plan = ((14 if plan[1] in (15, 16, 17, 18, 20, 21) else plan[1]), 1) if plan[0] in ("splitk", "slabs") else (plan[0], plan[1])
    if plan[0] == "tile" and plan[1] in (20, 21) and (d.pool2 == 2 or not CFG.PERSIST or not _persist_ok(d)):
        plan = ("tile", 16 if (d.pool2 or plan[1] == 21) else 15, plan[2], 0 if d.pool2 else plan[3]) + tuple(plan[4:])
    if d.bn_stats:
        if plan[0] == "tile" and plan[1] in (15, 16, 17, 18):
            plan = ("tile", 14, plan[2], min(plan[3], 208)) + tuple(plan[4:])
        elif plan[0] == "skew" and plan[1] in (15, 16, 17, 18):
            plan = ("skew", 14) + tuple(plan[2:])
        elif isinstance(plan[0], int) and plan[0] in (15, 16, 17, 18):
            plan = (14, plan[1])
        elif isinstance(plan[0], int) and plan[0] == 19 and d.epilogue != EPI_NONE:
            plan = (10, plan[1])
    d.tile_px, d.px_begin, d.px_end, d.skew_phases, d.skew_step = 0, 0, 0, 0, 0
    if plan[0] == "splitk" and CFG.DETERMINISTIC:
        plan = ("slabs", plan[1], plan[2], 0)
    if plan[0] in ("splitk", "slabs"):
        slabs = plan[0] == "slabs"
        S = plan[2]
        M = d.N * d.Ho * d.Wo
        acc = RT._splitk_scratch(M * d.Cout * (S if slabs else 1), zero=not slabs)
        d2 = IgemmDesc.from_buffer_copy(d)
        d2.out_fp32, d2.epilogue, d2.split_k, d2.tile_hint, d2.tile_order = 1, EPI_NONE, S, plan[1], 1
        d2.out_img_stride, d2.out_row_stride, d2.out_px_stride, d2.out_off = d.Ho * d.Wo * d.Cout, d.Wo * d.Cout, d.Cout, 0
        d2.split_slabs, d2.tile_px = (1, plan[3]) if slabs else (0, 0)
        _igemm(L_, d2, inp, w, None, None, ptr(acc), st, what)
        d.split_k, d.split_slabs = (S, 1) if slabs else (1, 0)
        try:
            check(L_.yolo_igemm_finish(ctypes.byref(d), ptr(acc), bias, aux, out, st), what + " (finish)")
        finally:
            d.split_k, d.split_slabs = 1, 0
        return
    if plan[0] in ("skew", "tile"):
        if plan[0] == "skew":
            d.tile_hint, d.tile_order, d.skew_phases, d.skew_step = plan[1], plan[2], plan[3], plan[4]
        else:
            d.tile_hint, d.tile_order, d.tile_px = plan[1], plan[2], plan[3]
            if len(plan) > 4:
                d.skew_phases, d.skew_step = plan[4], plan[5]
        try:
            _igemm(L_, d, inp, w, bias, aux, out, st, what)
        finally:
            d.skew_phases, d.skew_step, d.tile_px = 0, 0, 0
        return
    d.tile_hint, d.tile_order = plan[0], plan[1]
    if len(plan) == 2:
        _igemm(L_, d, inp, w, bias, aux, out, st, what)
        return
    d.px_begin, d.px_end = 0, plan[2]
    _igemm(L_, d, inp, w, bias, aux, out, st, what)
    d.tile_hint, d.px_begin, d.px_end = plan[3], plan[2], 0
    _igemm(L_, d, inp, w, bias, aux, out, st, what)
    d.px_begin, d.px_end = 0, 0


class _RawDevice:

    def __init__(self, ptr_, n, fp32):
        self.__cuda_array_interface__ = {"shape": (n,), "typestr": "<f4" if fp32 else "<i2", "data": (int(ptr_), False), "version": 2}


def _output_snapshot(L_, d: IgemmDesc, plan, inp, w, bias, aux, out, st, what):
    _run_plan_igemm(L_, d, plan, inp, w, bias, aux, out, st, what)
    torch.cuda.synchronize()
    addr = out.value if hasattr(out, "value") else int(out)
    t = torch.as_tensor(_RawDevice(addr, d.N * d.out_img_stride, bool(d.out_fp32)), device="cuda")
    t = t if d.out_fp32 else t.view(torch.bfloat16)
    return torch.nan_to_num(t.float(), nan=0.0, posinf=0.0, neginf=0.0).clone()


def _tune(L_, d: IgemmDesc, inp, w, bias, aux, out, st, what):
    dev = torch.device("cuda", torch.cuda.current_device())
    stats_ptr, d.bn_stats = d.bn_stats, None
    M = d.N * d.Ho * d.Wo

    def timed(plan):
        try:
            _run_plan_igemm(L_, d, plan, inp, w, bias, aux, out, st, what)
        except _hip.HipUnsupported:
            return None
        ts = []
        reps = CFG.TUNE_REPS
        for _ in range(3):
            if reps <= 1:
                _flush_caches(dev)
            e0, e1 = torch.cuda.Event(enable_timing=True), torch.cuda.Event(enable_timing=True)
            e0.record()
            for _r in range(max(1, reps)):
                _run_plan_igemm(L_, d, plan, inp, w, bias, aux, out, st, what)
            e1.record()
            e1.synchronize()
            ts.append(e0.elapsed_time(e1) / max(1, reps))
        return min(ts)

    times = {}

    def consider(plan):
        t = timed(plan)
        if t is not None:
            times[plan] = t

    cands = [c for c in _TUNE_CANDIDATES if not (d.pool2 and c in (3, 12))]
    if d.pool2 and not (d.Ho % 8 == 0 and d.Wo % 16 == 0):
        cands = []
    if d.KH == 1 and d.KW == 1 and d.tap_len <= 256 and not d.pool2:
        cands.append(10)
    if d.KH == 1 and d.KW == 1 and not d.pool2:
        if d.tap_len in (64, 128, 192, 256, 512) and d.Cout % 64 == 0 and (d.N * d.Ho * d.Wo) % 16 == 0 and not d.out_fp32 and d.split_k <= 1:
            cands.append(19)
    if (d.KH == 3 and d.KW == 3 and d.tap_len == 64 and d.Cout == 64 and d.stride == 1 and d.Ho % 16 == 0 and d.Wo % 16 == 0 and not d.pool2 and not d.out_fp32
            and d.epilogue in (EPI_NONE, EPI_BIAS, EPI_BIAS_LRELU)):
        cands.append(22)
    orders = (1, 2) if (d.Cout * d.KH * d.KW * d.tap_len * 2 > (4 << 20) and d.Cout >= 1024) else (1,)
    for c in cands:
        for o in orders:
            consider((c, o))
    tile_px = 196 if M % 196 == 0 else 208
    if not d.pool2:
        for o in orders:
            consider(("tile", 14, o, tile_px))
            if _pipe_ok(d):
                consider(("tile", 15, o, tile_px))
                consider(("tile", 17, o, tile_px))
                if (d.Ho * d.Wo) % 112 == 0:
                    consider(("tile", 16, o, 0))
                    consider(("tile", 18, o, 0))
            if _persist_ok(d):
                for tp in sorted({tile_px, 208, 0 if M % 224 else 224} - {0}):
                    consider(("tile", 21 if tp == 224 else 20, o, tp))
    elif _pipe_pool_ok(d):
        consider(("tile", 16, 1, 0))
        consider(("tile", 18, 1, 0))
        if _persist_ok(d) and d.pool2 in (1, 3) and M % 224 == 0:
            consider(("tile", 21, 1, 0))
    if times and not d.pool2:
        singles = sorted((pl for pl in times if isinstance(pl[0], int)), key=times.get)
        for (c, o) in [pl for pl in singles if _TILE[pl[0]][0] * _TILE[pl[0]][1] >= 128 * 128][:2]:
            tco, tpx = _TILE[c]
            n_co = (d.Cout + tco - 1) // tco
            tiles = n_co * ((M + tpx - 1) // tpx)
            cuts = set()
            for slots in (256, 512):
                full = tiles // slots * slots
                cut = full // n_co * tpx
                if 0 < cut < M and tiles - full < 0.9 * slots:
                    cuts.add(cut)
            for cut in sorted(cuts):
                for tc in _TAIL_CANDIDATES:
                    consider((c, o, cut, tc))
    if times and not d.pool2:
        eight = [pl for pl in sorted(times, key=times.get) if (len(pl) == 2 and pl[0] in (11, 12)) or pl[0] == "tile"][:2]
        for pl in eight:
            c, o, tpv = (pl[0], pl[1], 0) if isinstance(pl[0], int) else (pl[1], pl[2], pl[3])
            tco, tpx = _TILE[c]
            tiles = ((d.Cout + tco - 1) // tco) * ((M + (tpv or tpx) - 1) // (tpv or tpx))
            if tiles < 400:
                continue
            tile_cycles = times[pl] * 1e-3 / ((tiles + 255) // 256) * 2.1e9
            for ph, frac in ((3, 0.3), (5, 0.2), (3, 0.2), (5, 0.3)):
                consider(("tile", c, o, tpv, ph, int(frac * tile_cycles)) if tpv else ("skew", c, o, ph, int(frac * tile_cycles)))
    if (times and not d.pool2 and not d.out_fp32 and M <= 8192 and d.KH * d.KW * d.tap_len >= 2304 and d.Cout % 8 == 0
            and d.epilogue in (EPI_NONE, EPI_BIAS, EPI_BIAS_LRELU, EPI_MUL_DLRELU)):
        for c, S, tpv in ((11, 2, 0), (5, 2, 0), (3, 2, 0), (14, 4, tile_px), (15, 4, tile_px), (15, 2, tile_px), (12, 4, 0), (11, 4, 0)):
            consider(("slabs", c, S, tpv))
        if M < 2048 or ((d.Cout + 63) // 64) * ((M + 127) // 128) < 256:
            nks = d.KH * d.KW * d.tap_len // 64
            for c in (5, 3, 4):
                for S in (4, 8, 16, 32):
                    if nks // S >= 2:
                        consider(("slabs", c, S, 0))
        if d.Cout % 256 == 0 and d.tap_len % 32 == 0:
            for S in (2, 4, 8):
                nks = d.KH * d.KW * d.tap_len // 32
                if nks % S == 0 and (nks // S) % 2 == 0 and nks // S >= 6:
                    consider(("slabs", 20, S, tile_px))
    if not times:
        d.bn_stats = stats_ptr
        return (0, 0)
    best = None
    want = _output_snapshot(L_, d, _default_plan(d), inp, w, bias, aux, out, st, what)
    for cand in sorted(times, key=times.get):
        got = _output_snapshot(L_, d, cand, inp, w, bias, aux, out, st, what)
        err = float((got - want).norm() / (want.norm() + 1e-30))
        if err < 0.02:
            best = cand
            break
        print(f"tune: {what} {_tune_key(d)}: plan {cand} differs from the default plan's output by {err:.3g} -- dropped", flush=True)
        del times[cand]
    d.bn_stats = stats_ptr
    if best is None:
        return _default_plan(d)
    if CFG.TUNE_LOG is not None:
        CFG.TUNE_LOG.append((_tune_key(d), best, sorted(times.items(), key=lambda kv: kv[1])[:6]))
    return best




def igemm_call(d: IgemmDesc, inp, w, bias, aux, out, st, what: str):
    L_ = RT.lib()
    plain = CFG.TILE_HINT == 0 and d.split_k <= 1 and not d.w_blocked and d.tap_len % 64 == 0
    if not plain:
        d.tile_hint, d.tile_px = CFG.TILE_HINT, CFG.TILE_PX
        _igemm(L_, d, inp, w, bias, aux, out, st, what)
        return
    key = _tune_key(d)
    best = _TUNED.get(key)
    if best is None:
        if CFG.AUTOTUNE and CFG.TIMERS is None and (d.N * d.Ho * d.Wo >= 2048 or d.KH * d.KW * d.tap_len * d.Cout >= (1 << 20)):
            best = _tune(L_, d, inp, w, bias, aux, out, st, what)
        else:
            best = _borrowed_plan(key)
            if best is not None:
                _BORROWED.add(key)
            else:
                best = _default_plan(d)
        _TUNED[key] = best
    if key in _BORROWED:
        _BORROWED.discard(key)
        try:
            _run_plan_igemm(L_, d, best, inp, w, bias, aux, out, st, what)
            return
        except _hip.HipUnsupported:
            best = _TUNED[key] = _default_plan(d)
    rec = CFG.PLAN_TIMES
    if rec is None:
        _run_plan_igemm(L_, d, best, inp, w, bias, aux, out, st, what)
        return
    e0, e1 = torch.cuda.Event(enable_timing=True), torch.cuda.Event(enable_timing=True)
    e0.record()
    _run_plan_igemm(L_, d, best, inp, w, bias, aux, out, st, what)
    e1.record()
    rec.setdefault(key, []).append((e0, e1))


def _tune_key(d: IgemmDesc):
    return (d.N, d.Ho, d.Wo, d.KH, d.KW, d.tap_len, d.Cout, d.stride, d.epilogue, 1 if d.pool2 == 3 else d.pool2, d.out_px_stride, d.in_px_stride)


if CFG.PLAN_TABLE:
    load_plans()
```

Measured before the change: 24290 images/s.

## Fuse split-K slab reduction and epilogue into the GEMM via last-arriver counters

Split-K convolutions and FC layers now reduce their fp32 slabs and apply bias/LReLU/dLReLU inside the same kernel. The last workgroup to arrive on an output tile, tracked by per-tile atomic counters, does the reduction and then resets the counter. This removes the separate finish or bias_lrelu_rows launch and its extra pass over the scratch. In exchange the slab sums run as a serialized tail in the last-arriving block, the code needs release/acquire fences and a counter ring, and the persistent kernel uses extra LDS.

```diff
diff --git a/include/yolo_hip.h b/include/yolo_hip.h
--- a/include/yolo_hip.h
+++ b/include/yolo_hip.h
@@ -71,6 +71,8 @@
     void *bn_stats;
     int32_t tile_px;
     int32_t split_slabs;
+    void *finish_slabs;
+    int32_t finish_in_kernel;
 } yolo_igemm_desc;
 
 #define YOLO_EPI_NONE 0
diff --git a/yolo-v1_amd/csrc/igemm.hip b/yolo-v1_amd/csrc/igemm.hip
--- a/yolo-v1_amd/csrc/igemm.hip
+++ b/yolo-v1_amd/csrc/igemm.hip
@@ -35,7 +35,7 @@
 __global__ void __launch_bounds__(WCO * WPX * 64, (TCO == 64 && TPX == 128 && BK == 32 && VAR == 0 ? 5 : 2)) igemm_kernel(const IgemmParams p)
 {
     using Cfg = IgemmCfg<TCO, TPX, BK, WCO, WPX, NST, MF>;
-    constexpr bool STATS = VAR == 1, CODES = VAR == 2;
+    constexpr bool STATS = VAR == 1, CODES = VAR == 2, FIN = VAR == 3;
     constexpr bool M16 = MF != MFMA_32x32x16;
     constexpr bool UNEVEN = Cfg::UNEVEN;
     constexpr bool STG = MF == MFMA_16x16x32_STAGGER || UNEVEN;
@@ -581,6 +581,23 @@
             }
         }
     }
+    if constexpr (FIN) {
+        asm volatile("s_waitcnt vmcnt(0)" ::: "memory");
+        __syncthreads();
+        int *lst = reinterpret_cast<int *>(stage_base);
+        if (tid == 0) lst[0] = bid;
+        const int S = (int)gridDim.y;
+        finish_arrive(p.fin_ctr, lst, 1, (unsigned)S);
+        if (lst[0] >= 0) {
+            long npx = p.M - px0;
+            if (npx > tpv) npx = tpv;
+            for (int e = tid; e < (int)npx * CCH; e += NTHR) {
+                const int c = co0 + (e % CCH) * 8;
+                if (c < p.Cout) finish_px8(p, S, px0 + e / CCH, c);
+            }
+            if (tid == 0) __hip_atomic_store(p.fin_ctr + bid, 0u, __ATOMIC_RELAXED, __HIP_MEMORY_SCOPE_AGENT);
+        }
+    }
 }
 
 template <int TCO, int TPX, int BK, int WCO, int WPX, int NST, int MF, int VAR>
@@ -610,6 +627,10 @@
     if (p.px_fastest < 0) q.px_fastest = 0;
     q.nk_per_split = (q.nk + splits - 1) / splits;
     const int real_splits = p.slab_stride ? splits : (q.nk + q.nk_per_split - 1) / q.nk_per_split;
+    if (VAR == 3) {
+        q.fin_ctr = finish_counters(dev, (long)q.n_co_tiles * q.n_px_tiles);
+        if (!q.fin_ctr) return fail(YOLO_E_UNSUPPORTED, "yolo_igemm: finish_in_kernel: no arrival counters for %ld output tiles", (long)q.n_co_tiles * q.n_px_tiles);
+    }
     hipLaunchKernelGGL((igemm_kernel<TCO, TPX, BK, WCO, WPX, NST, MF, VAR>), dim3(q.n_co_tiles * q.n_px_tiles, real_splits), dim3(Cfg::NTHR), Cfg::LDS_BYTES, s, q);
     return check_launch("yolo_igemm");
 }
@@ -617,6 +638,7 @@
 template <int TCO, int TPX, int BK, int WCO, int WPX, int NST, int MF = MFMA_32x32x16>
 static int launch(const IgemmParams &p, int splits, hipStream_t s)
 {
+    if (p.fin_out) return launch_impl<TCO, TPX, BK, WCO, WPX, NST, MF, 3>(p, splits, s);
     return p.stats ? launch_impl<TCO, TPX, BK, WCO, WPX, NST, MF, 1>(p, splits, s) : launch_impl<TCO, TPX, BK, WCO, WPX, NST, MF, 0>(p, splits, s);
 }
 
@@ -699,12 +721,23 @@
     if ((d->epilogue == YOLO_EPI_MUL_DLRELU || d->epilogue == YOLO_EPI_BIAS_ADD_LRELU) && !aux) return fail(YOLO_E_ARG, "yolo_igemm: epilogue needs aux");
     if (d->epilogue < 0 || d->epilogue > YOLO_EPI_BIAS_ADD_LRELU) return fail(YOLO_E_ARG, "yolo_igemm: epilogue %d", d->epilogue);
     const int splits = d->split_k > 1 ? d->split_k : 1;
-    if (splits > 1 && (!d->out_fp32 || d->epilogue != YOLO_EPI_NONE)) return fail(YOLO_E_ARG, "yolo_igemm: split_k needs fp32 output and EPI_NONE");
-    if (d->split_slabs && splits > 1 && (d->out_off != 0 || (d->Wo > 1 && d->out_px_stride != d->Cout) || (d->Ho > 1 && d->out_row_stride != d->Wo * d->Cout)
+    const bool fin = d->finish_in_kernel != 0;
+    if (fin) {
+        if (splits < 2 || !d->split_slabs || !d->finish_slabs) return fail(YOLO_E_ARG, "yolo_igemm: finish_in_kernel needs split_k > 1, split_slabs = 1 and the slab scratch (finish_slabs)");
+        if (d->epilogue != YOLO_EPI_NONE && d->epilogue != YOLO_EPI_BIAS && d->epilogue != YOLO_EPI_BIAS_LRELU && d->epilogue != YOLO_EPI_MUL_DLRELU)
+            return fail(YOLO_E_UNSUPPORTED, "yolo_igemm: finish_in_kernel has no epilogue %d", d->epilogue);
+        if (d->pool2 || d->bn_stats || d->px_begin || d->px_end) return fail(YOLO_E_UNSUPPORTED, "yolo_igemm: finish_in_kernel takes no pool2, bn_stats or pixel range");
+        if (d->epilogue == YOLO_EPI_MUL_DLRELU && ((d->Cout & 7) || (d->aux_off & 7) || (d->aux_px_stride & 7) || (d->aux_row_stride & 7) || (d->aux_img_stride & 7)))
+            return fail(YOLO_E_UNSUPPORTED, "yolo_igemm: finish_in_kernel reads aux in 16-byte pieces: Cout and aux strides in multiples of 8");
+        if ((d->tile_hint >= 15 && d->tile_hint <= 19) || d->tile_hint == 22 || d->tile_hint == 12 || d->tile_hint == 14)
+            return fail(YOLO_E_UNSUPPORTED, "yolo_igemm: tile_hint %d has no in-kernel finish (two passes: yolo_igemm_finish)", d->tile_hint);
+    }
+    if (!fin && splits > 1 && (!d->out_fp32 || d->epilogue != YOLO_EPI_NONE)) return fail(YOLO_E_ARG, "yolo_igemm: split_k needs fp32 output and EPI_NONE");
+    if (!fin && d->split_slabs && splits > 1 && (d->out_off != 0 || (d->Wo > 1 && d->out_px_stride != d->Cout) || (d->Ho > 1 && d->out_row_stride != d->Wo * d->Cout)
                                          || (d->N > 1 && d->out_img_stride != (int64_t)d->Ho * d->Wo * d->Cout)))
         return fail(YOLO_E_ARG, "yolo_igemm: split_slabs needs the dense [N*Ho*Wo][Cout] output addressing");
     if (d->tile_px < 0) return fail(YOLO_E_ARG, "yolo_igemm: tile_px %d", d->tile_px);
-    if (!d->out_fp32 && ((d->Cout & 7) || (d->out_off & 7) || (d->out_px_stride & 7) || (d->out_row_stride & 7) || (d->out_img_stride & 7)))
+    if (!fin && !d->out_fp32 && ((d->Cout & 7) || (d->out_off & 7) || (d->out_px_stride & 7) || (d->out_row_stride & 7) || (d->out_img_stride & 7)))
         return fail(YOLO_E_UNSUPPORTED, "yolo_igemm: bf16 output needs Cout and output strides in multiples of 8");
     if ((d->tap_len & 31) || (d->in_off & 7) || (d->in_px_stride & 3) || (d->in_row_stride & 7) || (d->in_img_stride & 7))
         return fail(YOLO_E_UNSUPPORTED, "yolo_igemm: tap_len=%d must be a multiple of 32 and input strides 16-B aligned", d->tap_len);
@@ -725,6 +758,14 @@
     p.out_img_stride = d->out_img_stride; p.out_row_stride = d->out_row_stride; p.out_px_stride = d->out_px_stride; p.out_off = d->out_off;
     p.aux_img_stride = d->aux_img_stride; p.aux_row_stride = d->aux_row_stride; p.aux_px_stride = d->aux_px_stride; p.aux_off = d->aux_off;
     p.epilogue = d->epilogue; p.slope = d->slope; p.out_fp32 = d->out_fp32;
+    if (fin) {
+        p.out = d->finish_slabs;
+        p.out_img_stride = (long)d->Ho * d->Wo * d->Cout; p.out_row_stride = d->Wo * d->Cout; p.out_px_stride = d->Cout; p.out_off = 0;
+        p.epilogue = YOLO_EPI_NONE; p.out_fp32 = 1;
+        p.fin_out = out;
+        p.fin_img_stride = d->out_img_stride; p.fin_row_stride = d->out_row_stride; p.fin_px_stride = d->out_px_stride; p.fin_off = d->out_off;
+        p.fin_epilogue = d->epilogue; p.fin_out_fp32 = d->out_fp32;
+    }
     hipStream_t s = STRM(stream);
 
     const bool bk64 = (d->tap_len % 64) == 0;
diff --git a/yolo-v1_amd/csrc/igemm_common.h b/yolo-v1_amd/csrc/igemm_common.h
--- a/yolo-v1_amd/csrc/igemm_common.h
+++ b/yolo-v1_amd/csrc/igemm_common.h
@@ -45,7 +45,106 @@
     double *stats;
     unsigned div_hw_magic, div_hw_shift, div_w_magic, div_w_shift, div_hw2_magic, div_hw2_shift;
     unsigned *tile_ctr;
+    unsigned *fin_ctr;
+    void *fin_out;
+    long fin_img_stride;
+    int fin_row_stride, fin_px_stride, fin_off;
+    int fin_epilogue, fin_out_fp32;
 };
+
+unsigned *finish_counters(int dev, long n);
+
+__device__ __forceinline__ void finish_px8(const IgemmParams &p, int S, long m, int c)
+{
+    const float *a0 = reinterpret_cast<const float *>(p.out) + m * p.Cout + c;
+    const int nv = p.Cout - c < 8 ? p.Cout - c : 8;
+    const bool vec = nv == 8 && ((m * p.Cout + c) & 3) == 0;
+    float v[8];
+    if (vec) {
+        const f32x4 a = *reinterpret_cast<const f32x4 *>(a0), b = *reinterpret_cast<const f32x4 *>(a0 + 4);
+        v[0] = a[0]; v[1] = a[1]; v[2] = a[2]; v[3] = a[3]; v[4] = b[0]; v[5] = b[1]; v[6] = b[2]; v[7] = b[3];
+        for (int sl = 1; sl < S; ++sl) {
+            const float *as = a0 + (long)sl * p.slab_stride;
+            const f32x4 a2 = *reinterpret_cast<const f32x4 *>(as), b2 = *reinterpret_cast<const f32x4 *>(as + 4);
+            v[0] += a2[0]; v[1] += a2[1]; v[2] += a2[2]; v[3] += a2[3]; v[4] += b2[0]; v[5] += b2[1]; v[6] += b2[2]; v[7] += b2[3];
+        }
+    } else {
+#pragma unroll
+        for (int k = 0; k < 8; ++k) v[k] = k < nv ? a0[k] : 0.0f;
+        for (int sl = 1; sl < S; ++sl) {
+            const float *as = a0 + (long)sl * p.slab_stride;
+#pragma unroll
+            for (int k = 0; k < 8; ++k) v[k] += k < nv ? as[k] : 0.0f;
+        }
+    }
+    const int n = (int)(m / p.HoWo);
+    const int rem = (int)(m - (long)n * p.HoWo);
+    const int oy = rem / p.Wo, ox = rem - oy * p.Wo;
+    if (p.fin_epilogue == YOLO_EPI_BIAS || p.fin_epilogue == YOLO_EPI_BIAS_LRELU) {
+#pragma unroll
+        for (int k = 0; k < 8; ++k) v[k] += k < nv ? p.bias[c + k] : 0.0f;
+    }
+    if (p.fin_epilogue == YOLO_EPI_BIAS_LRELU) {
+#pragma unroll
+        for (int k = 0; k < 8; ++k) v[k] = v[k] > 0.0f ? v[k] : v[k] * p.slope;
+    } else if (p.fin_epilogue == YOLO_EPI_MUL_DLRELU) {
+        const uint4 y = *reinterpret_cast<const uint4 *>(p.aux + (long)n * p.aux_img_stride + (long)oy * p.aux_row_stride + (long)ox * p.aux_px_stride + p.aux_off + c);
+        const unsigned yy[4] = {y.x, y.y, y.z, y.w};
+#pragma unroll
+        for (int k = 0; k < 8; ++k) {
+            const float t = __uint_as_float((k & 1) ? (yy[k >> 1] & 0xffff0000u) : (yy[k >> 1] << 16));
+            v[k] = t > 0.0f ? v[k] : v[k] * p.slope;
+        }
+    }
+    const long oe = (long)n * p.fin_img_stride + (long)oy * p.fin_row_stride + (long)ox * p.fin_px_stride + p.fin_off + c;
+    if (p.fin_out_fp32) {
+        float *o = reinterpret_cast<float *>(p.fin_out) + oe;
+        if (nv == 8 && (oe & 3) == 0) {
+            *reinterpret_cast<f32x4 *>(o) = f32x4{v[0], v[1], v[2], v[3]};
+            *reinterpret_cast<f32x4 *>(o + 4) = f32x4{v[4], v[5], v[6], v[7]};
+        } else {
+#pragma unroll
+            for (int k = 0; k < 8; ++k)
+                if (k < nv) o[k] = v[k];
+        }
+    } else {
+        bf16_t *o = reinterpret_cast<bf16_t *>(p.fin_out) + oe;
+        if (nv == 8 && (oe & 7) == 0) {
+            uint4 pk;
+            pk.x = (unsigned)f32_to_bf16(v[0]) | ((unsigned)f32_to_bf16(v[1]) << 16);
+            pk.y = (unsigned)f32_to_bf16(v[2]) | ((unsigned)f32_to_bf16(v[3]) << 16);
+            pk.z = (unsigned)f32_to_bf16(v[4]) | ((unsigned)f32_to_bf16(v[5]) << 16);
+            pk.w = (unsigned)f32_to_bf16(v[6]) | ((unsigned)f32_to_bf16(v[7]) << 16);
+            *reinterpret_cast<uint4 *>(o) = pk;
+        } else {
+#pragma unroll
+            for (int k = 0; k < 8; ++k)
+                if (k < nv) o[k] = f32_to_bf16(v[k]);
+        }
+    }
+}
+
+__device__ __forceinline__ void finish_arrive(unsigned *ctr, int *lst, int n, unsigned S)
+{
+    __syncthreads();
+    if (threadIdx.x == 0) {
+        __builtin_amdgcn_fence(__ATOMIC_RELEASE, "agent");
+        asm volatile("s_waitcnt vmcnt(0)" ::: "memory");
+        bool any = false;
+        for (int i = 0; i < n; ++i) {
+            const int t = lst[i];
+            const unsigned old = __hip_atomic_fetch_add(ctr + t, 1u, __ATOMIC_RELAXED, __HIP_MEMORY_SCOPE_AGENT);
+            const bool last = old == S - 1u;
+            lst[i] = last ? t : -1;
+            any |= last;
+        }
+        if (any) {
+            __builtin_amdgcn_fence(__ATOMIC_ACQUIRE, "agent");
+            asm volatile("s_waitcnt vmcnt(0)" ::: "memory");
+        }
+    }
+    __syncthreads();
+}
 
 #define GLDS16(gptr, lptr) \
     __builtin_amdgcn_global_load_lds((const __attribute__((address_space(1))) void *)(gptr), (__attribute__((address_space(3))) void *)(lptr), 16, 0, 0)
diff --git a/yolo-v1_amd/csrc/igemm_persist.hip b/yolo-v1_amd/csrc/igemm_persist.hip
--- a/yolo-v1_amd/csrc/igemm_persist.hip
+++ b/yolo-v1_amd/csrc/igemm_persist.hip
@@ -20,6 +20,7 @@
     static constexpr int MAIL_BYTES = 64;
     static constexpr int LDS_BYTES = 2 * TABLE_BYTES + STASH_BYTES + MAIL_BYTES + NST * STAGE_BYTES;
     static constexpr int D = NST - 1;
+    static constexpr int FIN_LIST = 1024;
     static_assert(NT1 >= 1 && NT1 <= NT0, "pixel group B holds 1 .. 7 columns");
 };
 
@@ -108,7 +109,7 @@
     y = f32x4{y0, y1, y2, y3};
 }
 
-template <int NTILES, bool POOL, int DGRAD, bool CODES = false, bool SLAB = false, int MT = 4>
+template <int NTILES, bool POOL, int DGRAD, bool CODES = false, bool SLAB = false, int MT = 4, bool FIN = false>
 __global__ void __launch_bounds__(512, 2) igemm_persist_kernel(const IgemmParams p)
 {
     using C = PersistCfg<NTILES>;
@@ -255,6 +256,7 @@
     const int a_rd0 = lds_off<BK, true>(wco * WCH + (lane & 15), lane >> 4);
     const int b_rd0 = A_BYTES + lds_off<BK, true>(px_lo + (lane & 15), lane >> 4);
 
+    int n_done = 0;
     f32x4 acc[MT][NT0];
 
     unsigned drawn = 0;
@@ -560,6 +562,9 @@
 #endif
             nst = __builtin_amdgcn_readfirstlane(min(MT, max(0, (p.Cout - co0_cur - wco * WCH) >> 4)));
             epilogue(ti & 1, co0_cur, nst, ks_cur);
+            if constexpr (FIN) {
+                if (wave == 0 && fresh_lane() == 0) reinterpret_cast<int *>(smem + C::LDS_BYTES)[ti] = j_cur;
+            }
             ks_cur = ks_next;
 #ifdef IGEMM_STAMPS
             if (ti == 0) PSTAMP(3);
@@ -574,6 +579,7 @@
             if (!has_next) n_lim = ti;
         }
         wait_vmcnt<0>();
+        n_done = n_lim;
         if (threadIdx.x == 0) {
             const unsigned gone = atomicAdd(p.tile_ctr + 8 + xl, 1u);
             if (gone == (unsigned)nwg_x - 1u) {
@@ -584,6 +590,26 @@
     };
     if (grp == 0) run(std::integral_constant<int, NT0>{});
     else run(std::integral_constant<int, NT1>{});
+    if constexpr (FIN) {
+        int *lst = reinterpret_cast<int *>(smem + C::LDS_BYTES);
+        if (threadIdx.x == 0) {
+            const int q = T >> 3, r = T & 7;
+            const int base = xl < r ? xl * (q + 1) : r * (q + 1) + (xl - r) * q;
+            for (int i = 0; i < n_done; ++i) lst[i] = (base + lst[i]) / S;
+        }
+        finish_arrive(p.fin_ctr, lst, n_done, (unsigned)S);
+        for (int i = 0; i < n_done; ++i) {
+            const int ot = lst[i];
+            if (ot < 0) continue;
+            const int co_tile = p.px_fastest ? ot / p.n_px_tiles : ot % p.n_co_tiles;
+            const int px_tile = p.px_fastest ? ot % p.n_px_tiles : ot / p.n_co_tiles;
+            const long px0 = (long)px_tile * tpv;
+            const int npx = (int)(p.M - px0 < tpv ? p.M - px0 : tpv);
+            constexpr int CCH = TCO / 8;
+            for (int e = threadIdx.x; e < npx * CCH; e += C::NTHR) finish_px8(p, S, px0 + e / CCH, co_tile * TCO + (e % CCH) * 8);
+            if (threadIdx.x == 0) __hip_atomic_store(p.fin_ctr + ot, 0u, __ATOMIC_RELAXED, __HIP_MEMORY_SCOPE_AGENT);
+        }
+    }
 #ifdef IGEMM_STAMPS
     if (p.dbg && lane == 0 && blockIdx.x < 512) {
         tstamp[7] = __builtin_amdgcn_s_memtime();
@@ -622,17 +648,38 @@
     return ring[dev] + 16u * (next[dev].fetch_add(1u, std::memory_order_relaxed) % RING);
 }
 
-template <int NTILES, bool POOL, int DGRAD, bool CODES = false, bool SLAB = false, int MT = 4>
+unsigned *finish_counters(int dev, long n)
+{
+    constexpr long RING = 1L << 20;
+    static unsigned *ring[64] = {};
+    static long next[64] = {};
+    static std::mutex mu;
+    if (dev < 0 || dev >= 64 || n <= 0 || n > RING / 16) return nullptr;
+    std::lock_guard<std::mutex> g(mu);
+    if (!ring[dev]) {
+        unsigned *r = nullptr;
+        if (hipMalloc(&r, RING * sizeof(unsigned)) != hipSuccess) return nullptr;
+        if (hipMemset(r, 0, RING * sizeof(unsigned)) != hipSuccess || hipDeviceSynchronize() != hipSuccess) return nullptr;
+        ring[dev] = r;
+    }
+    if (next[dev] + n > RING) next[dev] = 0;
+    unsigned *c = ring[dev] + next[dev];
+    next[dev] += n;
+    return c;
+}
+
+template <int NTILES, bool POOL, int DGRAD, bool CODES = false, bool SLAB = false, int MT = 4, bool FIN = false>
 static int persist_launch(const IgemmParams &p, int splits, hipStream_t s)
 {
     using C = PersistCfg<NTILES>;
+    constexpr int LDS = C::LDS_BYTES + (FIN ? C::FIN_LIST * 4 : 0);
     static bool attr_done[64] = {};
     static int cus[64] = {};
     int dev = 0;
     if (hipGetDevice(&dev) != hipSuccess || dev < 0 || dev >= 64) dev = 0;
     if (!attr_done[dev]) {
-        hipError_t e = hipFuncSetAttribute(reinterpret_cast<const void *>(&igemm_persist_kernel<NTILES, POOL, DGRAD, CODES, SLAB, MT>), hipFuncAttributeMaxDynamicSharedMemorySize, C::LDS_BYTES);
-        if (e != hipSuccess) return fail((int)e, "yolo_igemm: hipFuncSetAttribute(%d B LDS): %s", C::LDS_BYTES, hipGetErrorString(e));
+        hipError_t e = hipFuncSetAttribute(reinterpret_cast<const void *>(&igemm_persist_kernel<NTILES, POOL, DGRAD, CODES, SLAB, MT, FIN>), hipFuncAttributeMaxDynamicSharedMemorySize, LDS);
+        if (e != hipSuccess) return fail((int)e, "yolo_igemm: hipFuncSetAttribute(%d B LDS): %s", LDS, hipGetErrorString(e));
         int n = 0;
         if (hipDeviceGetAttribute(&n, hipDeviceAttributeMultiprocessorCount, dev) != hipSuccess || n <= 0) n = 256;
         cus[dev] = n;
@@ -654,7 +701,12 @@
     q.pool_tiles_x = SLAB ? splits : 1;
     q.tile_ctr = persist_counters(dev);
     if (!q.tile_ctr) return fail(2, "yolo_igemm: cannot allocate the tile counters");
-    hipLaunchKernelGGL((igemm_persist_kernel<NTILES, POOL, DGRAD, CODES, SLAB, MT>), dim3(G), dim3(C::NTHR), C::LDS_BYTES, s, q);
+    if (FIN) {
+        if ((tiles + 7) / 8 > C::FIN_LIST) return fail(YOLO_E_UNSUPPORTED, "yolo_igemm: finish_in_kernel holds at most %d tiles per XCD label", C::FIN_LIST);
+        q.fin_ctr = finish_counters(dev, (long)q.n_co_tiles * q.n_px_tiles);
+        if (!q.fin_ctr) return fail(YOLO_E_UNSUPPORTED, "yolo_igemm: finish_in_kernel: no arrival counters for %ld output tiles", (long)q.n_co_tiles * q.n_px_tiles);
+    }
+    hipLaunchKernelGGL((igemm_persist_kernel<NTILES, POOL, DGRAD, CODES, SLAB, MT, FIN>), dim3(G), dim3(C::NTHR), LDS, s, q);
     return check_launch("yolo_igemm (persistent)");
 }
 
@@ -693,6 +745,7 @@
         return p.pool == 3 ? persist_launch<14, true, 0, true>(p, 1, s) : persist_launch<14, true, 0>(p, 1, s);
     }
     if (slab && p.Cout % 256) return fail(YOLO_E_UNSUPPORTED, "yolo_igemm: tile_hint %d splits K only for Cout %% 256 == 0", hint);
+    if (slab && p.fin_out) return hint == 20 ? persist_launch<13, false, 0, false, true, 4, true>(p, splits, s) : persist_launch<14, false, 0, false, true, 4, true>(p, splits, s);
     if (slab) return hint == 20 ? persist_launch<13, false, 0, false, true>(p, splits, s) : persist_launch<14, false, 0, false, true>(p, splits, s);
     const int dg = p.epilogue == YOLO_EPI_MUL_DLRELU ? 1 : (p.epilogue == YOLO_EPI_BIAS_ADD_LRELU ? 2 : 0);
     switch (hint) {
diff --git a/yolo-v1_amd/yolo/_hip.py b/yolo-v1_amd/yolo/_hip.py
--- a/yolo-v1_amd/yolo/_hip.py
+++ b/yolo-v1_amd/yolo/_hip.py
@@ -36,6 +36,7 @@
         ("skew_phases", ctypes.c_int32), ("skew_step", ctypes.c_int32),
         ("bn_stats", ctypes.c_void_p),
         ("tile_px", ctypes.c_int32), ("split_slabs", ctypes.c_int32),
+        ("finish_slabs", ctypes.c_void_p), ("finish_in_kernel", ctypes.c_int32),
     ]
 
 
diff --git a/yolo-v1_amd/yolo/config.py b/yolo-v1_amd/yolo/config.py
--- a/yolo-v1_amd/yolo/config.py
+++ b/yolo-v1_amd/yolo/config.py
@@ -15,6 +15,8 @@
     PLAN_TABLE: bool = True
     BORROW_PLANS: bool = True
     SMALL_SPLIT: bool = True
+    FINISH_IN_KERNEL: bool = True
+    FINISH_IN_KERNEL_MAX_KB: int = 0
     PERSIST: bool = True
     BN_STATS_IN_CONV: bool = True
     STEM_KERNEL: bool = True
diff --git a/yolo-v1_amd/yolo/executor.py b/yolo-v1_amd/yolo/executor.py
--- a/yolo-v1_amd/yolo/executor.py
+++ b/yolo-v1_amd/yolo/executor.py
@@ -10,7 +10,7 @@
 from . import _hip
 from ._hip import (EPI_BIAS, EPI_BIAS_LRELU, EPI_MUL_DLRELU, EPI_NONE, ConvPackItem, ConvUnpackItem, IgemmDesc, PoolDesc, WgradDesc, check, ptr)
 from .config import CONFIG as CFG
-from .plans import igemm_call
+from .plans import finish_in_kernel_ok, igemm_call
 from .runtime import RT, Act, _attach_wgrad_slabs, _EventSlot, _igemm, _on_side_stream, _round_up, _timed
 
 @dataclass
@@ -501,13 +501,19 @@
                 b = L.bias.detach()
                 if splits > 1:
                     acc = RT._splitk_scratch(splits * N * L.Cout, zero=False)
-                    d.epilogue, d.split_k, d.split_slabs = EPI_NONE, splits, 1
-                    with _timed(f"fc{li}", "igemm", 2.0 * N * L.Cout * L.Cin):
-                        _igemm(L_, d, ptr(xin), ptr(wf), None, None, ptr(acc), st, f"igemm fc{li}")
                     yb = torch.empty((N, L.Cout), dtype=torch.bfloat16, device=dev) if not last else None
                     yf = torch.empty((N, L.Cout), dtype=torch.float32, device=dev) if last else None
-                    check(L_.yolo_bias_lrelu_rows_slabs(ptr(acc), splits, ptr(b), N, L.Cout, self.SLOPE if L.lrelu else 1.0, ptr(yb), ptr(yf), st),
-                          "bias_lrelu_rows")
+                    d.epilogue, d.split_k, d.split_slabs = (EPI_BIAS_LRELU if L.lrelu else EPI_BIAS), splits, 1
+                    if finish_in_kernel_ok(d, 0, splits, 128, 64 if N <= 64 else 128, self.c):
+                        d.out_fp32, d.finish_slabs, d.finish_in_kernel = (1 if last else 0), ptr(acc), 1
+                        with _timed(f"fc{li}", "igemm", 2.0 * N * L.Cout * L.Cin):
+                            _igemm(L_, d, ptr(xin), ptr(wf), ptr(b), None, ptr(yf if last else yb), st, f"igemm fc{li}")
+                    else:
+                        d.epilogue = EPI_NONE
+                        with _timed(f"fc{li}", "igemm", 2.0 * N * L.Cout * L.Cin):
+                            _igemm(L_, d, ptr(xin), ptr(wf), None, None, ptr(acc), st, f"igemm fc{li}")
+                        check(L_.yolo_bias_lrelu_rows_slabs(ptr(acc), splits, ptr(b), N, L.Cout, self.SLOPE if L.lrelu else 1.0, ptr(yb), ptr(yf), st),
+                              "bias_lrelu_rows")
                 else:
                     yf = torch.empty((N, L.Cout), dtype=torch.float32, device=dev)
                     d.epilogue, d.split_k = (EPI_BIAS_LRELU if L.lrelu else EPI_BIAS), 1
diff --git a/yolo-v1_amd/yolo/plans.py b/yolo-v1_amd/yolo/plans.py
--- a/yolo-v1_amd/yolo/plans.py
+++ b/yolo-v1_amd/yolo/plans.py
@@ -131,6 +131,22 @@
     return plan
 
 
+_FINISH_HINTS = frozenset((0, 1, 2, 3, 4, 5, 6, 7, 8, 9, 10, 11, 13, 20, 21))
+
+
+def finish_in_kernel_ok(d: IgemmDesc, hint: int, S: int, tile_co: int, tile_px: int, cfg=None) -> bool:
+    cfg = cfg or CFG
+    if not cfg.FINISH_IN_KERNEL or hint not in _FINISH_HINTS or S < 2:
+        return False
+    if d.pool2 or d.bn_stats or d.px_begin or d.px_end or d.epilogue not in (EPI_NONE, EPI_BIAS, EPI_BIAS_LRELU, EPI_MUL_DLRELU):
+        return False
+    if d.epilogue == EPI_MUL_DLRELU and (d.Cout % 8 or d.aux_off % 8 or d.aux_px_stride % 8 or d.aux_row_stride % 8 or d.aux_img_stride % 8):
+        return False
+    M = d.N * d.Ho * d.Wo
+    kb = S * min(tile_co, d.Cout) * min(tile_px, M) * 4 / 1024.0
+    return not cfg.FINISH_IN_KERNEL_MAX_KB or kb <= cfg.FINISH_IN_KERNEL_MAX_KB
+
+
 def _run_plan_igemm(L_, d: IgemmDesc, plan, inp, w, bias, aux, out, st, what):
     if d.bn_stats and (plan[0] in ("splitk", "slabs") or (isinstance(plan[0], int) and len(plan) == 4)):
         plan = ((14 if plan[1] in (15, 16, 17, 18, 20, 21) else plan[1]), 1) if plan[0] in ("splitk", "slabs") else (plan[0], plan[1])
@@ -153,6 +169,17 @@
         S = plan[2]
         M = d.N * d.Ho * d.Wo
         acc = RT._splitk_scratch(M * d.Cout * (S if slabs else 1), zero=not slabs)
+        tco, tpx = _TILE.get(plan[1], (0, 0))
+        if slabs and tco and not d.out_fp32 and finish_in_kernel_ok(d, plan[1], S, tco, plan[3] or tpx):
+            keep = (d.tile_hint, d.tile_order)
+            d.split_k, d.split_slabs, d.tile_hint, d.tile_order, d.tile_px = S, 1, plan[1], 1, plan[3]
+            d.finish_slabs, d.finish_in_kernel = ptr(acc), 1
+            try:
+                _igemm(L_, d, inp, w, bias, aux, out, st, what)
+            finally:
+                d.split_k, d.split_slabs, d.tile_px, d.finish_slabs, d.finish_in_kernel = 1, 0, 0, None, 0
+                d.tile_hint, d.tile_order = keep
+            return
         d2 = IgemmDesc.from_buffer_copy(d)
         d2.out_fp32, d2.epilogue, d2.split_k, d2.tile_hint, d2.tile_order = 1, EPI_NONE, S, plan[1], 1
         d2.out_img_stride, d2.out_row_stride, d2.out_px_stride, d2.out_off = d.Ho * d.Wo * d.Cout, d.Wo * d.Cout, d.Cout, 0
```

Result: slower. 22700 images/s (-6.5%).
